# burchim/AVEC

Measured on AMD Instinct MI355X. Metric: AV utterances/sec fwd+bwd (audio T=400, video 100x88x88), higher is better.
Workload: dtype bf16

## Files before the change

### avec_amd/csrc/attention.h

```cpp
#pragma once
#include "common.h"
#include "avec_hip.h"

struct AttnArgs {
  const void *q, *k, *v; long long ld;
  const void* e; long long lde;
  const long long* lens; int len_div;
  int q_full;
  const float* mask; long long mask_bstride;
  void* o; long long ldo;
  float* lse;
  const void* dout;
  void *dq, *dk, *dv; long long lddq, ldd;
  float* de; long long ldde;
  void *pbuf, *dsbuf; long long ldt;
  void* dsrel; long long ldr;
  int B, H, T, d; float scale;
  int Tk;
};

template <typename T>
__device__ __forceinline__ bool key_keep(const AttnArgs& a, int b, int i, int j) {
  if (a.mask) return a.mask[(long long)b * a.mask_bstride + (long long)i * a.Tk + j] != 0.f;
  if (i >= a.q_full) return false;
  if (a.lens) return j < (int)(a.lens[b] / a.len_div);
  return true;
}


int attn_mfma_fwd(const AttnArgs& a, hipStream_t st);
int attn_mfma_bwd_rows(const AttnArgs& a, hipStream_t st);
```

### avec_amd/csrc/attention.hip

```cpp
#include "attention.h"
#include <stdio.h>

static constexpr int TQ = 32;
static constexpr int RPW = TQ / 4;
static constexpr int TK = 64;
static constexpr int QC = 32;
static constexpr int NCS = 3;

template <typename T, int VW>
__device__ __forceinline__ void load_vec(const T* p, float* v) {
  constexpr int NB = VW * (int)sizeof(T);
  if constexpr (NB < 4) { v[0] = ldf(p); }
  else {
    uint32_t w[NB / 4];
    if constexpr (NB == 16) { const chunk16 c = ldg16(p); w[0] = c.w[0]; w[1] = c.w[1]; w[2] = c.w[2]; w[3] = c.w[3]; }
    else {
#pragma unroll
      for (int k = 0; k < NB / 4; ++k) w[k] = ((const uint32_t*)p)[k];
    }
    if constexpr (sizeof(T) == 4) {
#pragma unroll
      for (int k = 0; k < NB / 4; ++k) v[k] = __uint_as_float(w[k]);
    } else {
#pragma unroll
// ... 94 lines not shown
        float p = (iv && jv) ? __expf(s - Li[rr]) * Il[rr] : 0.f;
        pval = p * (dp - dl[rr]) * a.scale;
        if (iv && jv) {
          const long long o = ((long long)bh * Tn + i) * a.ldt + j; stf((T*)a.pbuf + o, p); stf((T*)a.dsbuf + o, pval);
          if (a.dsrel) stf((T*)a.dsrel + ((long long)h * a.B * Tn + (long long)b * Tn + i) * a.ldr + (j + Tn - 1 - i), pval);
        }
      }
      Ps[w * 64 + lane] = pval;
      __syncthreads();
      if (!BWD) {
        for (int jj = 0; jj < TK; ++jj) {
          const float pj = Ps[w * 64 + jj];
#pragma unroll
          for (int u = 0; u < NCS; ++u) if (lane + 64 * u < d) acc[rr][u] += pj * Vs[jj * DP + lane + 64 * u];
        }
      } else {
        const float* ebase = Es + (TQ - 1 - ri) * DP;
        for (int jj = 0; jj < TK; ++jj) {
          const float dsj = Ps[w * 64 + jj];
#pragma unroll
          for (int u = 0; u < NCS; ++u) if (lane + 64 * u < d) acc[rr][u] += dsj * (Ks[jj * DP + lane + 64 * u] + ebase[jj * DP + lane + 64 * u]);
        }
      }
      __syncthreads();
    }
  }
#pragma unroll
  for (int rr = 0; rr < RPW; ++rr) {
    const int i = i0 + w * RPW + rr;
    if (i >= Tn) continue;
    if (!BWD) {
      const float inv = 1.f / l_run[rr];
      T* op = (T*)a.o + ((long long)b * Tn + i) * a.ldo + h * d;
#pragma unroll
      for (int u = 0; u < NCS; ++u) if (lane + 64 * u < d) stf(op + lane + 64 * u, acc[rr][u] * inv);
      if (lane == 0) { a.lse[((long long)bh * Tn + i) * 2] = m_run[rr]; a.lse[((long long)bh * Tn + i) * 2 + 1] = l_run[rr]; }
    } else {
      T* op = (T*)a.dq + ((long long)b * Tn + i) * a.lddq + h * d;
#pragma unroll
      for (int u = 0; u < NCS; ++u) if (lane + 64 * u < d) stf(op + lane + 64 * u, acc[rr][u]);
    }
  }
}

template <typename T, int DPAD>
__global__ __launch_bounds__(256) void attn_bwd_cols_kernel(AttnArgs a, int ktiles) {
  extern __shared__ __attribute__((aligned(16))) float sm[];
  const int d = a.d, DP = d | 1, Tn = a.T;
  float* Qs = sm; float* Gs = Qs + QC * DP; float* R0 = Gs + QC * DP; float* R1 = R0 + 64 * DP;
  const int lane = threadIdx.x & 63, w = threadIdx.x >> 6;
  const int bh = blockIdx.y, b = bh / a.H, h = bh % a.H;
  const bool rel = (int)blockIdx.x >= ktiles;
  const int c0 = (rel ? (int)blockIdx.x - ktiles : (int)blockIdx.x) * 64;
  const int col = c0 + lane;
  const T* qp = (const T*)a.q + (long long)b * Tn * a.ld + h * d;
  const T* gp = (const T*)a.dout + (long long)b * Tn * a.ldo + h * d;
  const T* P = (const T*)a.pbuf + (long long)bh * Tn * a.ldt; const T* S = (const T*)a.dsbuf + (long long)bh * Tn * a.ldt;
  float acc0[DPAD], acc1[DPAD];
#pragma unroll
  for (int c = 0; c < DPAD; ++c) { acc0[c] = 0.f; acc1[c] = 0.f; }
  for (int ic = 0; ic < Tn; ic += QC) {
    __syncthreads();
    load_rows<T>(Qs, DP, qp, a.ld, ic, QC, Tn, d);
    if (!rel) load_rows<T>(Gs, DP, gp, a.ldo, ic, QC, Tn, d);
    __syncthreads();
    for (int qi = w; qi < QC; qi += 4) {
      const int i = ic + qi;
      if (i >= Tn) break;
      const float* qrow = Qs + qi * DP;
      if (!rel) {
        float ds = 0.f, p = 0.f;
        if (col < Tn) { ds = ldf(S + (long long)i * a.ldt + col); p = ldf(P + (long long)i * a.ldt + col); }
        const float* grow = Gs + qi * DP;
#pragma unroll
        for (int c = 0; c < DPAD; ++c) if (c < d) { acc0[c] += ds * qrow[c]; acc1[c] += p * grow[c]; }
      } else {
        const int j = i - (Tn - 1) + col;
        const float ds = (col < 2 * Tn - 1 && j >= 0 && j < Tn) ? ldf(S + (long long)i * a.ldt + j) : 0.f;
#pragma unroll
        for (int c = 0; c < DPAD; ++c) if (c < d) acc0[c] += ds * qrow[c];
      }
    }
  }
  __syncthreads();
  for (int ww = 0; ww < 4; ++ww) {
    if (w == ww) {
#pragma unroll
      for (int c = 0; c < DPAD; ++c) if (c < d) {
        if (ww == 0) { R0[lane * DP + c] = acc0[c]; R1[lane * DP + c] = acc1[c]; }
        else { R0[lane * DP + c] += acc0[c]; R1[lane * DP + c] += acc1[c]; }
      }
    }
    __syncthreads();
  }
  for (int idx = threadIdx.x; idx < 64 * d; idx += 256) {
    const int r = idx / d, c = idx - r * d; const int cc = c0 + r;
    if (!rel) {
      if (cc < Tn) { stf((T*)a.dk + ((long long)b * Tn + cc) * a.ldd + h * d + c, R0[r * DP + c]); stf((T*)a.dv + ((long long)b * Tn + cc) * a.ldd + h * d + c, R1[r * DP + c]); }
    } else if (cc < 2 * Tn - 1) {
      atomicAdd(a.de + (long long)cc * a.ldde + h * d + c, R0[r * DP + c]);
    }
  }
}

static int fill_args(AttnArgs& a, const avec_attn_t* p) {
  a.q = p->q; a.k = p->k; a.v = p->v; a.ld = p->ld; a.e = p->e; a.lde = p->lde; a.lens = p->lens; a.len_div = p->len_div > 0 ? p->len_div : 1; a.q_full = p->q_full > 0 ? p->q_full : p->T;
  a.mask = p->mask; a.mask_bstride = p->mask_bstride; a.o = p->o; a.ldo = p->ldo; a.lse = p->lse; a.dout = p->dout;
  a.dq = p->dq; a.dk = p->dk; a.dv = p->dv; a.lddq = p->lddq; a.ldd = p->ldd; a.de = p->de; a.ldde = p->ldde; a.pbuf = p->pbuf; a.dsbuf = p->dsbuf; a.ldt = p->ldt; a.dsrel = p->dsrel; a.ldr = p->ldr;
  a.B = p->B; a.H = p->H; a.T = p->T; a.d = p->d; a.scale = p->scale; a.Tk = p->Tk > 0 ? p->Tk : p->T;
  AVEC_CHECK_ARG(a.q && a.k && a.v && a.e && a.o && a.lse, "attention: null pointer");
  AVEC_CHECK_ARG(a.B > 0 && a.H > 0 && a.T > 0 && a.d > 0 && a.d <= 64 * NCS && a.Tk >= a.T, "attention: bad dims B=%d H=%d T=%d Tk=%d d=%d (d <= %d, Tk >= T)", a.B, a.H, a.T, a.Tk, a.d, 64 * NCS);
  return 0;
}

extern "C" int avec_relpos_attention_fwd(int dtype, const avec_attn_t* p, hipStream_t st) {
  AttnArgs a; AVEC_CHECK_ARG(p, "attention_fwd: null args"); if (int r = fill_args(a, p)) return r;
  if (dtype == AVEC_BF16) { const int r = attn_mfma_fwd(a, st); if (r != 1) return r; }
  const int DP = a.d | 1; size_t lds = (size_t)(2 * TK + (TQ + TK - 1) + TQ) * DP * 4 + 4 * 64 * 4;
  dim3 grid((a.T + TQ - 1) / TQ, a.B * a.H);
  avec_note_kernel("attn_rows<%s,fwd>", dtype == AVEC_BF16 ? "bf16" : "f32");
  if (dtype == AVEC_BF16) { if (int r = avec_lds_optin(attn_rows_kernel<bf16, false>, lds)) return r; hipLaunchKernelGGL((attn_rows_kernel<bf16, false>), grid, dim3(256), lds, st, a); }
  else { if (int r = avec_lds_optin(attn_rows_kernel<float, false>, lds)) return r; hipLaunchKernelGGL((attn_rows_kernel<float, false>), grid, dim3(256), lds, st, a); }
  AVEC_LAUNCH_CHECK(); return 0;
}

template <typename T> static int launch_bwd(AttnArgs& a, hipStream_t st) {
  const int DP = a.d | 1;
  size_t lds1 = (size_t)(2 * TK + (TQ + TK - 1) + 2 * TQ) * DP * 4 + 4 * 64 * 4;
  dim3 grid1((a.T + TQ - 1) / TQ, a.B * a.H);
  bool rows_done = false;
  const bool cols = !(a.dsrel || a.Tk != a.T);
  AVEC_CHECK_ARG(!cols || a.d <= 96, "attention_bwd: the register-accumulating column pass serves d <= 96 (d=%d): pass dsrel and use avec_gemm_tn_batched", a.d);
  if (sizeof(T) == 2) { const int r = attn_mfma_bwd_rows(a, st); if (r == 0) rows_done = true; else if (r != 1) return r; }
  if (!rows_done) {
    if (int r = avec_lds_optin(attn_rows_kernel<T, true>, lds1)) return r;
    avec_note_kernel("attn_rows<%s,bwd>", sizeof(T) == 2 ? "bf16" : "f32");
    hipLaunchKernelGGL((attn_rows_kernel<T, true>), grid1, dim3(256), lds1, st, a);
  }
  if (!cols) return 0;
  size_t lds2 = (size_t)(2 * QC + 2 * 64) * DP * 4;
  const int ktiles = (a.T + 63) / 64, rtiles = (2 * a.T - 1 + 63) / 64;
  dim3 grid2(ktiles + rtiles, a.B * a.H);
#define LB(DPAD) do { char rows_[96]; snprintf(rows_, sizeof(rows_), "%s", avec_last_kernel()); avec_note_kernel("%s+cols<%d>", rows_, DPAD); \
    if (int r = avec_lds_optin(attn_bwd_cols_kernel<T, DPAD>, lds2)) return r; hipLaunchKernelGGL((attn_bwd_cols_kernel<T, DPAD>), grid2, dim3(256), lds2, st, a, ktiles); } while (0)
  if (a.d <= 48) LB(48); else if (a.d <= 64) LB(64); else LB(96);
#undef LB
  return 0;
}

extern "C" int avec_relpos_attention_bwd(int dtype, const avec_attn_t* p, hipStream_t st) {
  AttnArgs a; AVEC_CHECK_ARG(p, "attention_bwd: null args"); if (int r = fill_args(a, p)) return r;
  AVEC_CHECK_ARG(a.dout && a.dq && a.pbuf && a.dsbuf && a.ldt >= a.Tk && (a.dsrel ? a.ldr >= a.Tk + a.T - 1 : (a.Tk != a.T || (a.dk && a.dv && a.de))), "attention_bwd: null gradient / scratch pointer");
  int r = (dtype == AVEC_BF16) ? launch_bwd<bf16>(a, st) : launch_bwd<float>(a, st);
  if (r) return r;
  AVEC_LAUNCH_CHECK(); return 0;
}

struct AttnStream {
  const void *q, *k, *v; long long ld; const void* e; long long lde; void *kc, *vc;
  const long long* pos; const unsigned char* reset; const long long* clen; int div;
  void* o; long long ldo; int B, H, Tq, d, L; float scale;
};
template <typename T>
__global__ __launch_bounds__(256) void attn_stream_kernel(AttnStream a) {
  extern __shared__ __attribute__((aligned(16))) float sm[];
  const int d = a.d, DP = d | 1, Tq = a.Tq, L = a.L, cap = L + Tq;
  float* Ks = sm; float* Vs = Ks + TK * DP; float* Es = Vs + TK * DP; float* Qs = Es + (TQ + TK - 1) * DP; float* Ps = Qs + TQ * DP;
  const int lane = threadIdx.x & 63, w = threadIdx.x >> 6;
  const int bh = blockIdx.y, b = bh / a.H, h = bh % a.H;
  const int i0 = blockIdx.x * TQ;
  long long p0 = (a.reset && a.reset[b]) ? 0 : a.pos[b] / a.div; if (p0 < 0) p0 = 0;
  int n = Tq;
  if (a.clen) { const long long c = (a.clen[b] + a.div - 1) / a.div; n = c < 0 ? 0 : (c > Tq ? Tq : (int)c); }
  const long long ldc = (long long)a.H * d;
  const T* qp = (const T*)a.q + (long long)b * Tq * a.ld + h * d;
  const T* kp = (const T*)a.k + (long long)b * Tq * a.ld + h * d;
  const T* vp = (const T*)a.v + (long long)b * Tq * a.ld + h * d;
  T* kcb = (T*)a.kc + (long long)b * cap * ldc + h * d;
  T* vcb = (T*)a.vc + (long long)b * cap * ldc + h * d;
  const T* ep = (const T*)a.e + h * d;
  for (int r = w; r < TQ; r += 4) {
    const int i = i0 + r; const bool ok = i < Tq;
    for (int c = lane; c < d; c += 64) Qs[r * DP + c] = ok ? ldf(qp + (long long)i * a.ld + c) : 0.f;
    if (ok && i < n) {
      const long long crow = (p0 + i) % cap;
      for (int c = lane; c < d; c += 64) { kcb[crow * ldc + c] = kp[(long long)i * a.ld + c]; vcb[crow * ldc + c] = vp[(long long)i * a.ld + c]; }
    }
  }
  float m_run[RPW], l_run[RPW], acc[RPW][NCS];
#pragma unroll
  for (int rr = 0; rr < RPW; ++rr) { m_run[rr] = -INFINITY; l_run[rr] = 0.f; for (int u = 0; u < NCS; ++u) acc[rr][u] = 0.f; }
  const int i_last = min(i0 + TQ, Tq) - 1;
  const bool wave_live = i0 + w * RPW < Tq;
  for (int c0 = i0; c0 <= i_last + L; c0 += TK) {
    __syncthreads();
    for (int r = w; r < TK; r += 4) {
      const int c = c0 + r; bool ok = c <= i_last + L; const T *kr = kp, *vr = vp;
      if (c < L) { const long long p = p0 - L + c; ok = ok && p >= 0; const long long row = ok ? p % cap : 0; kr = kcb + row * ldc; vr = vcb + row * ldc; }
      else { const int ci = c - L; ok = ok && ci < Tq; const long long row = ok ? ci : 0; kr = kp + row * a.ld; vr = vp + row * a.ld; }
      for (int ch = lane; ch < d; ch += 64) { Ks[r * DP + ch] = ok ? ldf(kr + ch) : 0.f; Vs[r * DP + ch] = ok ? ldf(vr + ch) : 0.f; }
    }
    const int dmin = i0 + L - c0 - (TK - 1);
    for (int r = w; r < TQ + TK - 1; r += 4) {
      const int dl = dmin + r; const bool ok = dl >= 0 && dl <= L; const T* er = ep + (long long)(ok ? dl : 0) * a.lde;
      for (int ch = lane; ch < d; ch += 64) Es[r * DP + ch] = ok ? ldf(er + ch) : 0.f;
    }
    __syncthreads();
    if (wave_live) {
      const int c = c0 + lane;
#pragma unroll
      for (int rr = 0; rr < RPW; ++rr) {
        const int ri = w * RPW + rr, i = i0 + ri; const int dl = i + L - c;
        const bool keep = i < Tq && dl >= 0 && dl <= L && (c >= L || p0 - L + c >= 0);
        const float* qrow = Qs + ri * DP; const float* krow = Ks + lane * DP; const float* erow = Es + (ri + TK - 1 - lane) * DP;
        float s = 0.f;
        for (int ch = 0; ch < d; ++ch) s += qrow[ch] * (krow[ch] + erow[ch]);
        s *= a.scale;
        const float tmax = wave_max(keep ? s : -INFINITY);
        const float m_new = fmaxf(m_run[rr], tmax);
        float pval = 0.f;
        if (m_new != -INFINITY) {
          const float alpha = (m_run[rr] == -INFINITY) ? 0.f : __expf(m_run[rr] - m_new);
          pval = keep ? __expf(s - m_new) : 0.f;
          l_run[rr] = l_run[rr] * alpha + wave_sum(pval);
          for (int u = 0; u < NCS; ++u) acc[rr][u] *= alpha;
          m_run[rr] = m_new;
        }
        Ps[ri * 64 + lane] = pval;
      }
    }
    __syncthreads();
    if (wave_live) {
#pragma unroll
      for (int rr = 0; rr < RPW; ++rr) {
        const float* prow = Ps + (w * RPW + rr) * 64;
        for (int jj = 0; jj < TK; ++jj) {
          const float pj = prow[jj];
#pragma unroll
          for (int u = 0; u < NCS; ++u) if (lane + 64 * u < d) acc[rr][u] += pj * Vs[jj * DP + lane + 64 * u];
        }
      }
    }
  }
#pragma unroll
  for (int rr = 0; rr < RPW; ++rr) {
    const int i = i0 + w * RPW + rr;
    if (i >= Tq) continue;
    const float inv = 1.f / l_run[rr];
    T* op = (T*)a.o + ((long long)b * Tq + i) * a.ldo + h * d;
#pragma unroll
    for (int u = 0; u < NCS; ++u) if (lane + 64 * u < d) stf(op + lane + 64 * u, acc[rr][u] * inv);
  }
}

extern "C" long long avec_relpos_attention_stream_state_bytes(int dtype, int B, int H, int d, int L, int Tq) {
  if (B <= 0 || H <= 0 || d <= 0 || L < 0 || Tq <= 0) return 0;
  return (long long)B * (L + Tq) * H * d * (dtype == AVEC_BF16 ? 2 : 4);
}
extern "C" int avec_relpos_attention_stream(int dtype, const void* q, const void* k, const void* v, long long ld, const void* e, long long lde, void* kcache, void* vcache,
                                            long long cache_bytes, const long long* pos, const unsigned char* reset, const long long* chunk_len, int div, void* o, long long ldo,
                                            int B, int H, int Tq, int d, int L, float scale, hipStream_t st) {
  AVEC_CHECK_ARG(q && k && v && e && kcache && vcache && pos && o, "relpos_attention_stream: null pointer (q, k, v, e, kcache, vcache, pos and o are required)");
  AVEC_CHECK_ARG(B > 0 && H > 0 && Tq > 0 && L >= 0 && div > 0 && d > 0 && d <= 64 * NCS, "relpos_attention_stream: bad dims B=%d H=%d Tq=%d d=%d L=%d div=%d (d <= %d)", B, H, Tq, d, L, div, 64 * NCS);
  AVEC_CHECK_ARG(ld >= (long long)H * d && ldo >= (long long)H * d && lde >= (long long)H * d, "relpos_attention_stream: row strides ld=%lld ldo=%lld lde=%lld below H * d = %d", ld, ldo, lde, H * d);
  const long long need = avec_relpos_attention_stream_state_bytes(dtype, B, H, d, L, Tq);
  AVEC_CHECK_ARG(cache_bytes >= need, "relpos_attention_stream: key / value rings of %lld bytes each, %lld needed (avec_relpos_attention_stream_state_bytes)", cache_bytes, need);
  const uintptr_t em = dtype == AVEC_BF16 ? 1 : 3;
  AVEC_CHECK_ARG(!(((uintptr_t)q | (uintptr_t)k | (uintptr_t)v | (uintptr_t)e | (uintptr_t)kcache | (uintptr_t)vcache | (uintptr_t)o) & em) && !(((uintptr_t)pos | (uintptr_t)chunk_len) & 7),
                 "relpos_attention_stream: misaligned pointer (tensors: element size, pos / chunk_len: 8 bytes)");
  AVEC_CHECK_ARG(kcache != vcache, "relpos_attention_stream: kcache and vcache must be two buffers");
  AttnStream a{q, k, v, ld, e, lde, kcache, vcache, pos, reset, chunk_len, div, o, ldo, B, H, Tq, d, L, scale};
  const int DP = d | 1; const size_t lds = (size_t)(2 * TK + (TQ + TK - 1) + TQ) * DP * 4 + (size_t)TQ * 64 * 4;
  dim3 grid((Tq + TQ - 1) / TQ, B * H);
  avec_note_kernel("attn_stream<%s>", dtype == AVEC_BF16 ? "bf16" : "f32");
  if (dtype == AVEC_BF16) { if (int r = avec_lds_optin(attn_stream_kernel<bf16>, lds)) return r; hipLaunchKernelGGL((attn_stream_kernel<bf16>), grid, dim3(256), lds, st, a); }
  else { if (int r = avec_lds_optin(attn_stream_kernel<float>, lds)) return r; hipLaunchKernelGGL((attn_stream_kernel<float>), grid, dim3(256), lds, st, a); }
  AVEC_LAUNCH_CHECK(); return 0;
}
```

### avec_amd/csrc/attention_mfma.hip

```cpp
#include "attention.h"
#ifndef AVEC_ATTN_ABL
#define AVEC_ATTN_ABL 0
#endif

typedef __attribute__((ext_vector_type(8))) __bf16 bf16x8_t;
typedef __attribute__((ext_vector_type(16))) float f32x16;
typedef short v4s_t __attribute__((ext_vector_type(4)));

static constexpr int NTMAX = 12;
static constexpr int CTMAX = 3;

template <int PITCH> __device__ __forceinline__ int aswz(int row) {
  return PITCH == 128 ? ((((row >> 1) & 1) << 2) | ((row >> 2) & 3)) : (((row & 3) << 2) | ((row >> 2) & 3));
}
__device__ __forceinline__ f32x16 mma(const chunk16& a, const chunk16& b, f32x16 c) {
  return __builtin_amdgcn_mfma_f32_32x32x16_bf16(__builtin_bit_cast(bf16x8_t, a), __builtin_bit_cast(bf16x8_t, b), c, 0, 0, 0);
}
__device__ __forceinline__ chunk16 tr8(const char* p0, const char* p1) {
  typedef __attribute__((address_space(3))) v4s_t* lp_t;
  const v4s_t a = __builtin_amdgcn_ds_read_tr16_b64_v4i16((lp_t)p0), b = __builtin_amdgcn_ds_read_tr16_b64_v4i16((lp_t)p1);
  const uint2 ua = __builtin_bit_cast(uint2, a), ub = __builtin_bit_cast(uint2, b);
  chunk16 f; f.w[0] = ua.x; f.w[1] = ua.y; f.w[2] = ub.x; f.w[3] = ub.y; return f;
}
__device__ __forceinline__ uint32_t pack2(float lo, float hi) { return f32x2_to_bf16x2(lo, hi); }

template <int PITCH, int NTHR>
__device__ __forceinline__ void stage_rows(char* dst, const bf16* src, long long ld, int row0, int nrows, int limit, int d, int dpad) {
  const int CH = dpad >> 3;
  for (int idx = threadIdx.x; idx < nrows * CH; idx += NTHR) {
    const int r = idx / CH, c = idx - r * CH; const int gr = row0 + r;
    chunk16 v; v.w[0] = v.w[1] = v.w[2] = v.w[3] = 0u;
    if (gr >= 0 && gr < limit) {
      const bf16* p = src + (long long)gr * ld + c * 8;
      if (c * 8 + 8 <= d) v = ldg16(p);
      else {
        uint32_t h[8];
#pragma unroll
        for (int e = 0; e < 8; ++e) h[e] = (c * 8 + e < d) ? (uint32_t)p[e].v : 0u;
#pragma unroll
        for (int e = 0; e < 4; ++e) v.w[e] = h[2 * e] | (h[2 * e + 1] << 16);
      }
    }
    *(chunk16*)(dst + r * PITCH + ((c ^ aswz<PITCH>(r)) << 4)) = v;
  }
}

__device__ __forceinline__ void attn_glds16(const void* gsrc, unsigned lds_dst_uniform) {
  unsigned keep;
  asm volatile("s_mov_b32 %0, m0\n\ts_mov_b32 m0, %2\n\ts_nop 0\n\tglobal_load_lds_dwordx4 %1, off\n\ts_mov_b32 m0, %0" : "=&s"(keep) : "v"(gsrc), "s"(lds_dst_uniform) : "memory");
}
__device__ __attribute__((aligned(64))) unsigned char attn_zero16[64];

template <int PITCH, int NW>
__device__ __forceinline__ void stage_rows_dma(unsigned lds_img, char* img, const bf16* src, long long ld, int row0, int nrows, int limit, int d, int dpad,
                                               long long last_row, int rowbytes, int wave, int lane) {
  constexpr int SLOTS = PITCH / 16, RPI = 64 / SLOTS;
  constexpr int NV = PITCH == 128 ? 2 : 4;
  const int CH = dpad >> 3;
  const int rg = lane / SLOTS, pos = lane % SLOTS;
  const int ninstr = nrows / RPI;
  const unsigned ldb = (unsigned)ld * 2u;
  const bool can_past = dpad * 2 > rowbytes && last_row <= (long long)limit - 1;
  const int lastr = can_past ? (int)last_row : -1;
  unsigned short pe[8]; int pk = -1, pn = 0; unsigned pc = 0;
  if (can_past) {
    const int rt = lastr - row0;
    if (rt >= 0 && rt < nrows && (rt / RPI) % NW == wave && rt % RPI == rg) {
      int c = pos ^ aswz<PITCH>(rt);
      if (c < CH && c * 16 + 16 > rowbytes) {
        pk = rt / RPI; pc = (unsigned)c * 16u; pn = (rowbytes - c * 16) >> 1; pn = pn < 0 ? 0 : pn;
        const unsigned short* q = (const unsigned short*)((const char*)src + ((unsigned)lastr * ldb + pc));
#pragma unroll
        for (int e = 0; e < 8; ++e) pe[e] = e < pn ? q[e] : (unsigned short)0;
      }
    }
  }
  unsigned coff[NV]; bool cpast[NV];
#pragma unroll
  for (int v = 0; v < NV; ++v) {
    int c = pos ^ aswz<PITCH>(RPI * (wave + v * NW) + rg); c = c < CH ? c : 0;
    coff[v] = (unsigned)c * 16u; cpast[v] = c * 16 + 16 > rowbytes;
  }
  for (int k0 = wave; k0 < ninstr; k0 += NW * NV) {
#pragma unroll
    for (int v = 0; v < NV; ++v) {
      const int k = k0 + v * NW;
      if (k < ninstr) {
        int gr = row0 + k * RPI + rg; gr = gr < 0 ? 0 : (gr >= limit ? limit - 1 : gr);
        const char* p = (const char*)src + ((unsigned)gr * ldb + coff[v]);
        const bool past = gr == lastr && cpast[v];
        attn_glds16(past ? (const void*)attn_zero16 : (const void*)p, (unsigned)__builtin_amdgcn_readfirstlane((int)(lds_img + k * 1024)));
      }
    }
  }
  if (can_past && __builtin_amdgcn_readfirstlane(__any(pk >= 0) ? 1 : 0)) {
    asm volatile("s_waitcnt vmcnt(0)" ::: "memory");
    if (pk >= 0) {
      unsigned short* dst = (unsigned short*)(img + pk * 1024 + lane * 16);
#pragma unroll
      for (int e = 0; e < 8; ++e) if (e < pn) dst[e] = pe[e];
    }
  }
}
template <int PITCH, int NW>
__device__ __forceinline__ void zero_pad_channels(char* img, int nrows, int d, int dpad, int wave, int lane) {
  if (d == dpad) return;
  constexpr int SLOTS = PITCH / 16, RPI = 64 / SLOTS;
  const int rg = lane / SLOTS, pos = lane % SLOTS;
  const int ninstr = nrows / RPI;
  for (int k = wave; k < ninstr; k += NW) {
    const int r = k * RPI + rg;
    const int c = pos ^ aswz<PITCH>(r);
    unsigned short* dst = (unsigned short*)(img + k * 1024 + lane * 16);
#pragma unroll
    for (int e = 0; e < 8; ++e) if (c * 8 + e >= d && c * 8 + e < dpad) dst[e] = 0;
  }
}

struct MfmaGeom { int Tp, NT, NE, dpad, DKS, CT, alias; size_t offK, offV, offE, offQ, offS, total; };
static MfmaGeom mfma_geom(int T, int d, int pitch, bool bwd) {
  MfmaGeom g; g.Tp = (T + 31) / 32 * 32; g.NT = g.Tp / 32; g.NE = g.Tp + 64; g.dpad = (d + 15) / 16 * 16; g.DKS = g.dpad / 16; g.CT = (d + 31) / 32;
  for (g.alias = 0; g.alias < 2; ++g.alias) {
    g.offK = 0; g.offV = g.alias ? g.offK : g.offK + (size_t)g.Tp * pitch; g.offE = g.offV + (size_t)g.Tp * pitch; g.offQ = g.offE + (size_t)g.NE * pitch;
    g.offS = g.offQ + (size_t)64 * pitch * (bwd ? 2 : 1);
    g.total = g.offS + (size_t)2 * 8192;
    if (g.total <= 160 * 1024) break;
  }
  if (g.alias > 1) g.alias = 1;
  return g;
}

template <int PITCH, int NTM, int DKS>
__device__ __forceinline__ float scores(f32x16 (&S)[NTM], const char* Ks, const char* Es, const char* qrow, float* ring, const MfmaGeom& G, float scale,
                                        int w, int il, int hf, int Tn, int klen, bool row_masked) {
  const int dks = DKS ? DKS : G.DKS;
  const int swr = aswz<PITCH>(il);
#pragma unroll
  for (int jt = 0; jt < NTM; ++jt)
#pragma unroll
    for (int r = 0; r < 16; ++r) S[jt][r] = 0.f;
  auto rel_tile = [&](int et) {
    f32x16 R;
#pragma unroll
    for (int r = 0; r < 16; ++r) R[r] = 0.f;
    const char* erow = Es + (32 * et + 32 * (1 - w) + il) * PITCH;
#pragma unroll
    for (int kk = 0; kk < dks; ++kk) {
      const chunk16 fa = *(const chunk16*)(erow + (((2 * kk + hf) ^ swr) << 4));
      const chunk16 fb = *(const chunk16*)(qrow + (((2 * kk + hf) ^ swr) << 4));
      R = mma(fa, fb, R);
    }
    float* slot = ring + (et & 1) * 1024;
#pragma unroll
    for (int r = 0; r < 16; ++r) slot[((r & 3) + 8 * (r >> 2) + 4 * hf) * 32 + il] = R[r];
  };
  rel_tile(0);
#pragma unroll
  for (int jt = 0; jt < NTM; ++jt) {
    if (jt < G.NT) {
      const char* krow = Ks + (32 * jt + il) * PITCH;
#pragma unroll
      for (int kk = 0; kk < dks; ++kk) {
        const chunk16 fa = *(const chunk16*)(krow + (((2 * kk + hf) ^ swr) << 4));
        const chunk16 fb = *(const chunk16*)(qrow + (((2 * kk + hf) ^ swr) << 4));
        S[jt] = mma(fa, fb, S[jt]);
      }
      rel_tile(jt + 1);
      asm volatile("s_waitcnt lgkmcnt(0)" ::: "memory");
#pragma unroll
      for (int r = 0; r < 16; ++r) {
        const int jl = (r & 3) + 8 * (r >> 2) + 4 * hf;
        const int el = 32 * jt + jl + 31 - il;
        S[jt][r] += ring[(el & 63) * 32 + il];
      }
      asm volatile("" ::: "memory");
    }
  }
  float mx = -INFINITY;
#pragma unroll
  for (int jt = 0; jt < NTM; ++jt) {
    if (jt < G.NT) {
#pragma unroll
      for (int r = 0; r < 16; ++r) {
        const int j = 32 * jt + (r & 3) + 8 * (r >> 2) + 4 * hf;
        float v = S[jt][r] * scale;
        if (row_masked || j >= klen) v += -1e9f;
        v = j < Tn ? v : -INFINITY;
        S[jt][r] = v; mx = fmaxf(mx, v);
      }
    }
  }
  return mx;
}

template <int PITCH>
__device__ __forceinline__ void tr_offsets(int (&off)[CTMAX][2], int lane) {
  const int g4 = lane >> 4, t = lane & 15;
#pragma unroll
  for (int hh = 0; hh < 2; ++hh) {
    const int key = 8 * hh + 4 * (g4 >> 1) + (t >> 2);
#pragma unroll
    for (int ct = 0; ct < CTMAX; ++ct) {
      const int cb = 32 * ct + 16 * (g4 & 1);
      off[ct][hh] = key * PITCH + ((((cb >> 3) + ((t & 3) >> 1)) ^ aswz<PITCH>(key)) << 4) + (t & 1) * 8;
    }
  }
}

__device__ __forceinline__ void store_rows_T(const f32x16 (&O)[CTMAX], float mul, float* ring, const MfmaGeom& G, bf16* op, long long ldo, int nrow, int d, int lane) {
  const int hf = lane >> 5, il = lane & 31;
  bf16* ost = (bf16*)ring; const int OP = G.dpad + 4;
  asm volatile("s_waitcnt lgkmcnt(0)" ::: "memory");
#pragma unroll
  for (int ct = 0; ct < CTMAX; ++ct) {
    if (ct < G.CT) {
#pragma unroll
      for (int q = 0; q < 4; ++q) {
        const int c0 = 32 * ct + 8 * q + 4 * hf;
        uint2 u; u.x = pack2(O[ct][4 * q] * mul, O[ct][4 * q + 1] * mul); u.y = pack2(O[ct][4 * q + 2] * mul, O[ct][4 * q + 3] * mul);
        if (c0 < G.dpad) *(uint2*)(ost + il * OP + c0) = u;
      }
    }
  }
  asm volatile("s_waitcnt lgkmcnt(0)" ::: "memory");
  typedef uint32_t __attribute__((aligned(2))) u32_u;
  const int dh = d >> 1;
  for (int idx = lane; idx < nrow * dh; idx += 64) { const int r = idx / dh, c = (idx - r * dh) * 2; *(u32_u*)(op + (long long)r * ldo + c) = *(const uint32_t*)(ost + r * OP + c); }
  if (d & 1) for (int r = lane; r < nrow; r += 64) op[(long long)r * ldo + d - 1] = ost[r * OP + d - 1];
}

template <int PITCH, int NTM, bool ALIAS, int DKS>
__global__ __launch_bounds__(ALIAS ? 128 : 256) void attn_mfma_fwd_kernel(AttnArgs a, MfmaGeom G) {
  constexpr int NWS = ALIAS ? 2 : 4;
  extern __shared__ __attribute__((aligned(16))) char sm[];
  char* Ks = sm + G.offK; char* Vs = sm + G.offV; char* Es = sm + G.offE; char* Qs = sm + G.offQ;
  const int tid = threadIdx.x, lane = tid & 63, w = tid >> 6, hf = lane >> 5, il = lane & 31;
  float* ring = (float*)(sm + G.offS + w * 8192);
  const int bh = blockIdx.y, b = bh / a.H, h = bh - b * a.H;
  const int Tn = a.T, d = a.d, i0 = blockIdx.x * 64;
  const bf16* qp = (const bf16*)a.q + (long long)b * Tn * a.ld + h * d;
  const bf16* kp = (const bf16*)a.k + (long long)b * Tn * a.ld + h * d;
  const bf16* vp = (const bf16*)a.v + (long long)b * Tn * a.ld + h * d;
  const bf16* ep = (const bf16*)a.e + h * d;
  {
    typedef __attribute__((address_space(3))) void* lptr_t;
    const unsigned lds0 = (unsigned)(uintptr_t)(lptr_t)sm;
    const int wv = __builtin_amdgcn_readfirstlane(w);
    const long long lastq = (long long)(a.B - 1 - b) * Tn + Tn - 1;
    const int rb = (a.H - h) * d * 2;
    stage_rows_dma<PITCH, NWS>(lds0 + (unsigned)G.offK, Ks, kp, a.ld, 0, G.Tp, Tn, d, G.dpad, lastq, rb, wv, lane);
    if (!ALIAS) stage_rows_dma<PITCH, NWS>(lds0 + (unsigned)G.offV, Vs, vp, a.ld, 0, G.Tp, Tn, d, G.dpad, lastq, rb, wv, lane);
    stage_rows_dma<PITCH, NWS>(lds0 + (unsigned)G.offQ, Qs, qp, a.ld, i0, 64, Tn, d, G.dpad, lastq, rb, wv, lane);
    stage_rows_dma<PITCH, NWS>(lds0 + (unsigned)G.offE, Es, ep, a.lde, (Tn - 1) - (i0 + 63), G.NE, 2 * Tn - 1, d, G.dpad, 2 * Tn - 2, rb, wv, lane);
    asm volatile("s_waitcnt vmcnt(0)" ::: "memory");
    zero_pad_channels<PITCH, NWS>(Qs, 64, d, G.dpad, wv, lane);
  }
  __syncthreads();
  if (NWS > 2 && w >= 2) return;
#if AVEC_ATTN_ABL == 1
  if (sm[tid * 16] == 123) a.lse[0] = 1.f;
  return;
#endif

  const int i = i0 + 32 * w + il;
  const char* qrow = Qs + (32 * w + il) * PITCH;
  const int klen = a.lens ? (int)(a.lens[b] / a.len_div) : Tn;
  const bool row_masked = i >= a.q_full;

  f32x16 S[NTM];
  float mx = scores<PITCH, NTM, DKS>(S, Ks, Es, qrow, ring, G, a.scale, w, il, hf, Tn, klen, row_masked);
  mx = fmaxf(mx, __shfl_xor(mx, 32, 64));
  float lsum = 0.f;
#pragma unroll
  for (int jt = 0; jt < NTM; ++jt) {
    if (jt < G.NT) {
#pragma unroll
      for (int r = 0; r < 16; ++r) { const float p = __expf(S[jt][r] - mx); S[jt][r] = p; lsum += p; }
    }
  }
  lsum += __shfl_xor(lsum, 32, 64);
  if (hf == 0 && i < Tn) { a.lse[((long long)bh * Tn + i) * 2] = mx; a.lse[((long long)bh * Tn + i) * 2 + 1] = lsum; }
#if AVEC_ATTN_ABL == 2
  return;
#endif

  if (ALIAS) { __syncthreads(); stage_rows<PITCH, 128>(Vs, vp, a.ld, 0, G.Tp, Tn, d, G.dpad); __syncthreads(); }
  f32x16 O[CTMAX];
#pragma unroll
  for (int ct = 0; ct < CTMAX; ++ct)
#pragma unroll
    for (int r = 0; r < 16; ++r) O[ct][r] = 0.f;
  int offv[CTMAX][2]; tr_offsets<PITCH>(offv, lane);
#pragma unroll
  for (int jt = 0; jt < NTM; ++jt) {
    if (jt < G.NT) {
#pragma unroll
      for (int s = 0; s < 2; ++s) {
        chunk16 pb;
#pragma unroll
        for (int e = 0; e < 4; ++e) pb.w[e] = pack2(S[jt][8 * s + 2 * e], S[jt][8 * s + 2 * e + 1]);
        const char* vb = Vs + (32 * jt + 16 * s) * PITCH;
#pragma unroll
        for (int ct = 0; ct < CTMAX; ++ct) if (ct < G.CT) O[ct] = mma(tr8(vb + offv[ct][0], vb + offv[ct][1]), pb, O[ct]);
      }
    }
  }
  bf16* op = (bf16*)a.o + ((long long)b * Tn + i0 + 32 * w) * a.ldo + h * d;
  store_rows_T(O, 1.f / lsum, ring, G, op, a.ldo, min(32, Tn - (i0 + 32 * w)), d, lane);
}

template <int PITCH, int NTM, bool ALIAS, int DKS>
__global__ __launch_bounds__(ALIAS ? 128 : 256) void attn_mfma_bwd_kernel(AttnArgs a, MfmaGeom G) {
  constexpr int NWS = ALIAS ? 2 : 4;
  extern __shared__ __attribute__((aligned(16))) char sm[];
  char* Ks = sm + G.offK; char* Vs = sm + G.offV; char* Es = sm + G.offE; char* Qs = sm + G.offQ; char* Gs = Qs + 64 * PITCH;
  const int tid = threadIdx.x, lane = tid & 63, w = tid >> 6, hf = lane >> 5, il = lane & 31;
  float* ring = (float*)(sm + G.offS + w * 8192);
  const int bh = blockIdx.y, b = bh / a.H, h = bh - b * a.H;
  const int Tn = a.T, d = a.d, i0 = blockIdx.x * 64;
  const bf16* qp = (const bf16*)a.q + (long long)b * Tn * a.ld + h * d;
  const bf16* kp = (const bf16*)a.k + (long long)b * Tn * a.ld + h * d;
  const bf16* vp = (const bf16*)a.v + (long long)b * Tn * a.ld + h * d;
  const bf16* ep = (const bf16*)a.e + h * d;
  const bf16* gp = (const bf16*)a.dout + (long long)b * Tn * a.ldo + h * d;
  {
    typedef __attribute__((address_space(3))) void* lptr_t;
    const unsigned lds0 = (unsigned)(uintptr_t)(lptr_t)sm;
    const int wv = __builtin_amdgcn_readfirstlane(w);
    const long long lastq = (long long)(a.B - 1 - b) * Tn + Tn - 1;
    const int rb = (a.H - h) * d * 2;
    stage_rows_dma<PITCH, NWS>(lds0 + (unsigned)G.offK, Ks, kp, a.ld, 0, G.Tp, Tn, d, G.dpad, lastq, rb, wv, lane);
    if (!ALIAS) stage_rows_dma<PITCH, NWS>(lds0 + (unsigned)G.offV, Vs, vp, a.ld, 0, G.Tp, Tn, d, G.dpad, lastq, rb, wv, lane);
    stage_rows_dma<PITCH, NWS>(lds0 + (unsigned)G.offQ, Qs, qp, a.ld, i0, 64, Tn, d, G.dpad, lastq, rb, wv, lane);
    stage_rows_dma<PITCH, NWS>(lds0 + (unsigned)G.offQ + 64 * PITCH, Gs, gp, a.ldo, i0, 64, Tn, d, G.dpad, lastq, rb, wv, lane);
    stage_rows_dma<PITCH, NWS>(lds0 + (unsigned)G.offE, Es, ep, a.lde, (Tn - 1) - (i0 + 63), G.NE, 2 * Tn - 1, d, G.dpad, 2 * Tn - 2, rb, wv, lane);
    asm volatile("s_waitcnt vmcnt(0)" ::: "memory");
    zero_pad_channels<PITCH, NWS>(Qs, 64, d, G.dpad, wv, lane);
    zero_pad_channels<PITCH, NWS>(Gs, 64, d, G.dpad, wv, lane);
  }
  __syncthreads();
  if (NWS > 2 && w >= 2) return;
#if AVEC_ATTN_ABL == 1
  if (sm[tid * 16] == 123) a.lse[0] = 1.f;
  return;
#endif

  const int i = i0 + 32 * w + il;
  const int swr = aswz<PITCH>(il);
  const char* qrow = Qs + (32 * w + il) * PITCH; const char* grow = Gs + (32 * w + il) * PITCH;
  const int klen = a.lens ? (int)(a.lens[b] / a.len_div) : Tn;
  const bool row_masked = i >= a.q_full, iv = i < Tn;
  float delta = 0.f, m_i = 0.f, il_i = 0.f;
  if (iv) {
    const bf16* orow = (const bf16*)a.o + ((long long)b * Tn + i) * a.ldo + h * d;
    const int c0 = hf * ((d + 1) >> 1), c1 = hf ? d : ((d + 1) >> 1);
    for (int c = c0; c < c1; ++c) {
      const int ch = c >> 3; const bf16* gq = (const bf16*)(grow + ((ch ^ swr) << 4)) + (c & 7);
      delta += bf16_to_f32(gq->v) * bf16_to_f32(orow[c].v);
    }
    m_i = a.lse[((long long)bh * Tn + i) * 2]; il_i = 1.f / a.lse[((long long)bh * Tn + i) * 2 + 1];
  }
  delta += __shfl_xor(delta, 32, 64);

  f32x16 S[NTM];
  scores<PITCH, NTM, DKS>(S, Ks, Es, qrow, ring, G, a.scale, w, il, hf, Tn, klen, row_masked);
#if AVEC_ATTN_ABL == 2
  if (S[0][0] + S[1][3] + delta == 1234.5f) a.lse[0] = 1.f;
  return;
#endif
  if (ALIAS) { __syncthreads(); stage_rows<PITCH, 128>(Vs, vp, a.ld, 0, G.Tp, Tn, d, G.dpad); __syncthreads(); }
  bf16* prow = (bf16*)a.pbuf + ((long long)bh * Tn + i) * a.ldt;
  bf16* srow = (bf16*)a.dsbuf + ((long long)bh * Tn + i) * a.ldt;
  bf16* rrow = a.dsrel ? (bf16*)a.dsrel + ((long long)h * a.B * Tn + (long long)b * Tn + i) * a.ldr + (Tn - 1 - i) : nullptr;
  const bool st8 = (a.ldt & 3) == 0 && ((((size_t)a.pbuf) | ((size_t)a.dsbuf)) & 7) == 0;
#pragma unroll
  for (int jt = 0; jt < NTM; ++jt) {
    if (jt < G.NT) {
      f32x16 dP;
#pragma unroll
      for (int r = 0; r < 16; ++r) dP[r] = 0.f;
      const char* vrow = Vs + (32 * jt + il) * PITCH;
#pragma unroll
      for (int kk = 0; kk < (DKS ? DKS : G.DKS); ++kk) {
        const chunk16 fa = *(const chunk16*)(vrow + (((2 * kk + hf) ^ swr) << 4));
        const chunk16 fb = *(const chunk16*)(grow + (((2 * kk + hf) ^ swr) << 4));
        dP = mma(fa, fb, dP);
      }
#pragma unroll
      for (int q = 0; q < 4; ++q) {
        const int j0 = 32 * jt + 8 * q + 4 * hf;
        float pv[4], dv[4];
#pragma unroll
        for (int e = 0; e < 4; ++e) {
          const int r = 4 * q + e; const bool ok = iv && (j0 + e) < Tn;
          const float p = ok ? __expf(S[jt][r] - m_i) * il_i : 0.f;
          pv[e] = p; dv[e] = p * (dP[r] - delta) * a.scale; S[jt][r] = dv[e];
        }
        if (iv && j0 < Tn) {
          if (st8 && j0 + 3 < Tn) {
            uint2 up, ud; up.x = pack2(pv[0], pv[1]); up.y = pack2(pv[2], pv[3]); ud.x = pack2(dv[0], dv[1]); ud.y = pack2(dv[2], dv[3]);
            *(uint2*)(prow + j0) = up; *(uint2*)(srow + j0) = ud;
          } else {
#pragma unroll
            for (int e = 0; e < 4; ++e) if (j0 + e < Tn) { prow[j0 + e].v = f32_to_bf16(pv[e]); srow[j0 + e].v = f32_to_bf16(dv[e]); }
          }
          if (rrow) {
            typedef uint2 __attribute__((aligned(2))) u64_u;
            if (j0 + 3 < Tn) { uint2 ud; ud.x = pack2(dv[0], dv[1]); ud.y = pack2(dv[2], dv[3]); *(u64_u*)(rrow + j0) = ud; }
            else {
#pragma unroll
              for (int e = 0; e < 4; ++e) if (j0 + e < Tn) rrow[j0 + e].v = f32_to_bf16(dv[e]);
            }
          }
        }
      }
    }
  }
#if AVEC_ATTN_ABL == 3
  return;
#endif
  if (ALIAS) { __syncthreads(); stage_rows<PITCH, 128>(Ks, kp, a.ld, 0, G.Tp, Tn, d, G.dpad); __syncthreads(); }
  f32x16 DQ[CTMAX];
#pragma unroll
  for (int ct = 0; ct < CTMAX; ++ct)
#pragma unroll
    for (int r = 0; r < 16; ++r) DQ[ct][r] = 0.f;
  int offt[CTMAX][2]; tr_offsets<PITCH>(offt, lane);
#pragma unroll
  for (int jt = 0; jt < NTM; ++jt) {
    if (jt < G.NT) {
#pragma unroll
      for (int s = 0; s < 2; ++s) {
        chunk16 pb;
#pragma unroll
        for (int e = 0; e < 4; ++e) pb.w[e] = pack2(S[jt][8 * s + 2 * e], S[jt][8 * s + 2 * e + 1]);
        const char* kb = Ks + (32 * jt + 16 * s) * PITCH;
#pragma unroll
        for (int ct = 0; ct < CTMAX; ++ct) if (ct < G.CT) DQ[ct] = mma(tr8(kb + offt[ct][0], kb + offt[ct][1]), pb, DQ[ct]);
      }
    }
  }
  asm volatile("s_waitcnt lgkmcnt(0)" ::: "memory");
#pragma unroll
  for (int r = 0; r < 16; ++r) ring[1024 + ((r & 3) + 8 * (r >> 2) + 4 * hf) * 32 + il] = 0.f;
#pragma unroll
  for (int et = 0; et <= NTM; ++et) {
    if (et <= G.NT) {
      float* slot = ring + (et & 1) * 1024;
#pragma unroll
      for (int r = 0; r < 16; ++r) {
        float v = 0.f;
        if (et < NTM) v = (et < G.NT) ? S[et < NTM ? et : 0][r] : 0.f;
        slot[((r & 3) + 8 * (r >> 2) + 4 * hf) * 32 + il] = v;
      }
      asm volatile("s_waitcnt lgkmcnt(0)" ::: "memory");
      float rs[16];
#pragma unroll
      for (int r = 0; r < 16; ++r) {
        const int j = 32 * et + (r & 3) + 8 * (r >> 2) + 4 * hf - 31 + il;
        rs[r] = ring[(j & 63) * 32 + il];
      }
      asm volatile("" ::: "memory");
#pragma unroll
      for (int s = 0; s < 2; ++s) {
        chunk16 pb;
#pragma unroll
        for (int e = 0; e < 4; ++e) pb.w[e] = pack2(rs[8 * s + 2 * e], rs[8 * s + 2 * e + 1]);
        const char* eb = Es + (32 * et + 32 * (1 - w) + 16 * s) * PITCH;
#pragma unroll
        for (int ct = 0; ct < CTMAX; ++ct) if (ct < G.CT) DQ[ct] = mma(tr8(eb + offt[ct][0], eb + offt[ct][1]), pb, DQ[ct]);
      }
    }
  }
  bf16* dqp = (bf16*)a.dq + ((long long)b * Tn + i0 + 32 * w) * a.lddq + h * d;
  store_rows_T(DQ, 1.f, ring, G, dqp, a.lddq, min(32, Tn - (i0 + 32 * w)), d, lane);
}

static const bool g_mfma_off = getenv("AVEC_NO_MFMA_ATTN") != nullptr;
static bool rows_too_short(long long ld, int d) { return ld + d < (d + 15) / 16 * 16; }

int attn_mfma_fwd(const AttnArgs& a, hipStream_t st) {
  if (g_mfma_off || a.mask || a.d > 96 || a.T > 32 * NTMAX || a.Tk != a.T || rows_too_short(a.ld, a.d) || rows_too_short(a.lde, a.d)) return 1;
  const int pitch = a.d <= 64 ? 128 : 256;
  const MfmaGeom G = mfma_geom(a.T, a.d, pitch, false);
  if (G.total > 160 * 1024) return 1;
  dim3 grid((a.T + 63) / 64, a.B * a.H);
#define AVEC_LAUNCH_ATTN(TAG, NAME, P, N, A, K) do { avec_note_kernel(TAG "<%d,%d,%d,%d>", P, N, (int)A, K); if (int r = avec_lds_optin(NAME<P, N, A, K>, G.total)) return r; \
    hipLaunchKernelGGL((NAME<P, N, A, K>), grid, dim3(G.alias ? 128 : 256), G.total, st, a, G); } while (0)
#define AVEC_PICK_DKS(TAG, NAME, N, A) do { \
    if (pitch == 128) { if (G.DKS == 4) AVEC_LAUNCH_ATTN(TAG, NAME, 128, N, A, 4); else if (G.DKS == 3) AVEC_LAUNCH_ATTN(TAG, NAME, 128, N, A, 3); else AVEC_LAUNCH_ATTN(TAG, NAME, 128, N, A, 0); } \
    else { if (G.DKS == 6) AVEC_LAUNCH_ATTN(TAG, NAME, 256, N, A, 6); else AVEC_LAUNCH_ATTN(TAG, NAME, 256, N, A, 0); } } while (0)
#define AVEC_PICK_ATTN(TAG, NAME) do { \
    if (a.T <= 224 && !G.alias) AVEC_PICK_DKS(TAG, NAME, 7, false); \
    else if (!G.alias) AVEC_PICK_DKS(TAG, NAME, 12, false); \
    else AVEC_PICK_DKS(TAG, NAME, 12, true); } while (0)
  AVEC_PICK_ATTN("attn_mfma_fwd", attn_mfma_fwd_kernel);
  AVEC_LAUNCH_CHECK(); return 0;
}

int attn_mfma_bwd_rows(const AttnArgs& a, hipStream_t st) {
  if (g_mfma_off || a.mask || a.d > 96 || a.T > 32 * NTMAX || a.Tk != a.T || !a.pbuf || !a.dsbuf || !a.dq || !a.dout || rows_too_short(a.ld, a.d) || rows_too_short(a.lde, a.d) ||
      rows_too_short(a.ldo, a.d)) return 1;
  const int pitch = a.d <= 64 ? 128 : 256;
  const MfmaGeom G = mfma_geom(a.T, a.d, pitch, true);
  if (G.total > 160 * 1024) return 1;
  dim3 grid((a.T + 63) / 64, a.B * a.H);
  AVEC_PICK_ATTN("attn_mfma_bwd", attn_mfma_bwd_kernel);
#undef AVEC_PICK_ATTN
#undef AVEC_PICK_DKS
#undef AVEC_LAUNCH_ATTN
  AVEC_LAUNCH_CHECK(); return 0;
}
```

### avec_amd/csrc/gemm.hip

```cpp
#include "gemm_dev.h"

template <typename T, int BM, int BN, int MODE, bool SRC_F32, bool A16>
__global__ __launch_bounds__(256, 2) void gemm_nt_kernel(GemmArgs g) {
  constexpr int VEC = Elt<T>::VEC;
  constexpr int KE = BKB / (int)sizeof(T);
  constexpr int NCA = BM * 8 / 256, NCB = BN * 8 / 256;
  constexpr int MT = BM / 64, NT = BN / 64;
  constexpr int TILE = (BM + BN) * LDS_ROW;
  extern __shared__ __attribute__((aligned(16))) char smem[];
  const int tid = threadIdx.x, lane = tid & 63, wave = tid >> 6;
  const int wm = wave >> 1, wn = wave & 1;
  const long long m0 = (long long)blockIdx.x * BM; const int n0 = blockIdx.y * BN;
  const int kc = (tid & 7) * VEC;
  const int r0 = tid >> 3;

  RowInfo ra[NCA]; RowInfo rb[NCB];
  RowSrc ws; ws.ptr = g.W; ws.ld = g.ldw; ws.step = 0; ws.rows_out = ws.rows_in = 1;
#pragma unroll
  for (int i = 0; i < NCA; ++i) ra[i] = row_info<MODE>(g.a, m0 + r0 + i * 32, g.M);
#pragma unroll
  for (int i = 0; i < NCB; ++i) rb[i] = row_info<MODE_PLAIN>(ws, n0 + r0 + i * 32, g.N);

  f32x16 acc[MT][NT];
#pragma unroll
// ... 678 lines not shown
    long long row[MT], rrow[MT]; bool valid[MT];
    const long long Mc = perm ? pMc : g.M;
    const bool use_res = g.e.res != nullptr && (!g.e.res_cls0 || cls == 0);
#pragma unroll
    for (int i = 0; i < MT; ++i) {
      long long mc = m0 + wm * (BM / 2) + i * 32 + (lane & 31);
      valid[i] = mc < Mc; if (!valid[i]) mc = Mc - 1;
      row[i] = mc;
      if (perm) { long long img; int ih, iw; perm2_pixel(g.a, cls, mc, img, ih, iw); row[i] = (img * g.a.H + ih) * (long long)g.a.W + iw; }
      rrow[i] = g.e.res_cls0 ? mc : row[i];
    }
    conv_epilogue_tr<BM, BN, MT, NT>(g, acc, smem, row, valid, use_res ? (const bf16*)g.e.res : nullptr, rrow, m0 + BM <= Mc, n0, tid, lane, wm, wn);
  } else nt_epilogue<T, BM, BN, MT, NT>(g, acc, smem, m0, n0, tid, lane, wm, wn, cls);
}

typedef __attribute__((ext_vector_type(8))) int i32x8;

template <int BM, int BN, int STAGES>
__global__ __launch_bounds__(256, 2) void gemm_nt_fp8_kernel(GemmArgs g, const float* __restrict__ amax_a, const float* __restrict__ amax_w) {
  typedef bf16 T;
  constexpr int RB = 128, KE = 128;
  constexpr int NCA = BM * 8 / 256, NCB = BN * 8 / 256;
  constexpr int MT = BM / 64, NT = BN / 64;
  constexpr int TILE = (BM + BN) * RB;
  extern __shared__ __attribute__((aligned(16))) char smem[];
  const int tid = threadIdx.x, lane = tid & 63, wave = tid >> 6;
  const int wm = wave >> 1, wn = wave & 1;
  const long long m0 = (long long)blockIdx.x * BM; const int n0 = blockIdx.y * BN;
  typedef __attribute__((address_space(1))) const void* gptr_t;
  typedef __attribute__((address_space(3))) void* lptr_t;
  long long aoff[NCA], boff[NCB]; int ka[NCA], kb[NCB];
#pragma unroll
  for (int i = 0; i < NCA; ++i) { const int row = (tid >> 3) + i * 32; aoff[i] = (m0 + row < g.M) ? (m0 + row) * g.a.ld : -1; ka[i] = ((tid & 7) ^ glds_swz<RB>(row)) * 16; }
#pragma unroll
  for (int i = 0; i < NCB; ++i) { const int row = (tid >> 3) + i * 32; boff[i] = (n0 + row < g.N) ? (long long)(n0 + row) * g.ldw : -1; kb[i] = ((tid & 7) ^ glds_swz<RB>(row)) * 16; }
  auto issue = [&](int kt, int buf) {
    char* As = smem + buf * TILE; char* Bs = As + BM * RB;
#pragma unroll
    for (int i = 0; i < NCA; ++i) {
      const int k = kt * KE + ka[i];
      const void* src = (aoff[i] >= 0 && k < g.K) ? (const void*)((const char*)g.a.ptr + aoff[i] + k) : (const void*)avec_zero16;
      __builtin_amdgcn_global_load_lds((gptr_t)src, (lptr_t)(As + (i * 256 + wave * 64) * 16), 16, 0, 0);
    }
#pragma unroll
    for (int i = 0; i < NCB; ++i) {
      const int k = kt * KE + kb[i];
      const void* src = (boff[i] >= 0 && k < g.K) ? (const void*)((const char*)g.W + boff[i] + k) : (const void*)avec_zero16;
      __builtin_amdgcn_global_load_lds((gptr_t)src, (lptr_t)(Bs + (i * 256 + wave * 64) * 16), 16, 0, 0);
    }
  };
  int offa[MT], swa[MT], offb[NT], swb[NT];
#pragma unroll
  for (int i = 0; i < MT; ++i) { const int row = wm * (BM / 2) + i * 32 + (lane & 31); offa[i] = row * RB; swa[i] = glds_swz<RB>(row); }
#pragma unroll
  for (int j = 0; j < NT; ++j) { const int row = wn * (BN / 2) + j * 32 + (lane & 31); offb[j] = row * RB; swb[j] = glds_swz<RB>(row); }
  const int gsel = lane >> 5;
  f32x16 acc[MT][NT];
#pragma unroll
  for (int i = 0; i < MT; ++i)
#pragma unroll
    for (int j = 0; j < NT; ++j)
#pragma unroll
      for (int r = 0; r < 16; ++r) acc[i][j][r] = 0.f;
  const int KT = (g.K + KE - 1) / KE;
  constexpr int LPT = NCA + NCB;
#define AVEC_WAIT_VM(n) asm volatile("s_waitcnt vmcnt(%0)" ::"n"(n) : "memory")
#pragma unroll
  for (int st = 0; st < STAGES - 1; ++st) if (st < KT) issue(st, st);
  for (int kt = 0; kt < KT; ++kt) {
    const int newer = min(STAGES - 2, KT - 1 - kt);
    if (STAGES <= 2 || newer <= 0) AVEC_WAIT_VM(0);
    else if (newer == 1) AVEC_WAIT_VM(LPT);
    else AVEC_WAIT_VM(2 * LPT);
    __builtin_amdgcn_s_barrier();
    asm volatile("" ::: "memory");
    if (kt + STAGES - 1 < KT) issue(kt + STAGES - 1, (kt + STAGES - 1) % STAGES);
    const char* As = smem + (kt % STAGES) * TILE; const char* Bs = As + BM * RB;
#pragma unroll
    for (int s2 = 0; s2 < 2; ++s2) {
      chunk16 fa[MT][2], fb[NT][2];
#pragma unroll
      for (int i = 0; i < MT; ++i)
#pragma unroll
        for (int h = 0; h < 2; ++h) fa[i][h] = *(const chunk16*)(As + offa[i] + (((4 * s2 + 2 * gsel + h) ^ swa[i]) << 4));
#pragma unroll
      for (int j = 0; j < NT; ++j)
#pragma unroll
        for (int h = 0; h < 2; ++h) fb[j][h] = *(const chunk16*)(Bs + offb[j] + (((4 * s2 + 2 * gsel + h) ^ swb[j]) << 4));
      asm volatile("" ::: "memory");
#pragma unroll
      for (int i = 0; i < MT; ++i) {
        const i32x8 a = {(int)fa[i][0].w[0], (int)fa[i][0].w[1], (int)fa[i][0].w[2], (int)fa[i][0].w[3], (int)fa[i][1].w[0], (int)fa[i][1].w[1], (int)fa[i][1].w[2], (int)fa[i][1].w[3]};
#pragma unroll
        for (int j = 0; j < NT; ++j) {
          const i32x8 b = {(int)fb[j][0].w[0], (int)fb[j][0].w[1], (int)fb[j][0].w[2], (int)fb[j][0].w[3], (int)fb[j][1].w[0], (int)fb[j][1].w[1], (int)fb[j][1].w[2], (int)fb[j][1].w[3]};
          acc[i][j] = __builtin_amdgcn_mfma_scale_f32_32x32x64_f8f6f4(a, b, acc[i][j], 0, 0, 0, 127, 0, 127);
        }
      }
    }
  }
#undef AVEC_WAIT_VM
  const float sc = (fmaxf(*amax_a, 1e-20f) * (1.0f / 448.0f)) * (fmaxf(*amax_w, 1e-20f) * (1.0f / 448.0f));
#pragma unroll
  for (int i = 0; i < MT; ++i)
#pragma unroll
    for (int j = 0; j < NT; ++j)
#pragma unroll
      for (int r = 0; r < 16; ++r) acc[i][j][r] *= sc;
  __syncthreads();
  nt_epilogue<T, BM, BN, MT, NT>(g, acc, smem, m0, n0, tid, lane, wm, wn);
}

struct TnArgs { const void* P; long long ldp; RowSrc q; float* O; void* Oact; long long ldo; long long M; int I, J, Iq, Jq; int m_per_block; float* pcs;
                int split, nb_inner, xcd_map, q_ohw, q_mg, q_nwrap; long long sPo, sPi, sQo, sQi, sOo, sOi; };

__device__ __forceinline__ int tn_swz(int col) { return (((col >> 2) ^ (col >> 3) ^ (col >> 4)) & 1) << 4; }

template <typename T>
__device__ __forceinline__ void store_transposed(char* S, int col0, int p, const chunk16& c0, const chunk16& c1) {
  constexpr int VEC = Elt<T>::VEC;
  if (sizeof(T) == 4) {
#pragma unroll
    for (int e = 0; e < VEC; ++e) *(uint32_t*)(S + (col0 + e) * LDS_ROW + ((p ^ tn_swz(col0 + e)) << 2)) = c0.w[e];
  } else {
#pragma unroll
    for (int e = 0; e < VEC; ++e) {
      const uint32_t w = (e & 1) ? __builtin_amdgcn_perm(c1.w[e >> 1], c0.w[e >> 1], 0x07060302u) : __builtin_amdgcn_perm(c1.w[e >> 1], c0.w[e >> 1], 0x05040100u);
      *(uint32_t*)(S + (col0 + e) * LDS_ROW + ((p ^ tn_swz(col0 + e)) << 2)) = w;
    }
  }
}

template <typename T, int BM, int BN, int MT, int NT>
__device__ __forceinline__ void mma_tile_swz(const char* As, const char* Bs, int wm, int wn, int lane, f32x16 (&acc)[MT][NT]) {
  int offa[MT], offb[NT], lowa[MT], lowb[NT];
#pragma unroll
  for (int i = 0; i < MT; ++i) { const int row = wm * (BM / 2) + i * 32 + (lane & 31); offa[i] = row * LDS_ROW; lowa[i] = ((lane >> 5) * 16) ^ (tn_swz(row) << 2); }
#pragma unroll
  for (int j = 0; j < NT; ++j) { const int row = wn * (BN / 2) + j * 32 + (lane & 31); offb[j] = row * LDS_ROW; lowb[j] = ((lane >> 5) * 16) ^ (tn_swz(row) << 2); }
#pragma unroll
  for (int kk = 0; kk < 4; ++kk) {
    chunk16 fa[MT], fb[NT];
#pragma unroll
    for (int i = 0; i < MT; ++i) fa[i] = *(const chunk16*)(As + offa[i] + (lowa[i] ^ (kk * 32)));
#pragma unroll
    for (int j = 0; j < NT; ++j) fb[j] = *(const chunk16*)(Bs + offb[j] + (lowb[j] ^ (kk * 32)));
#pragma unroll
    for (int i = 0; i < MT; ++i)
#pragma unroll
      for (int j = 0; j < NT; ++j) Mma<T>::run(fa[i], fb[j], acc[i][j]);
  }
}

template <typename T, int BI, int BJ, int MODE, bool Q_F32, bool A16>
__device__ __forceinline__ void gemm_tn_body(TnArgs g, const int bx, const int by, const int bz) {
  constexpr int VEC = Elt<T>::VEC;
  constexpr int RPT = sizeof(T) == 2 ? 2 : 1;
  constexpr int KE = 32 * RPT;
  constexpr int CPR_I = BI / VEC, CPR_J = BJ / VEC;
  constexpr int NTI = 32 * CPR_I / 256, NTJ = 32 * CPR_J / 256;
  constexpr int MT = BI / 64, NT = BJ / 64;
  constexpr int TILE = (BI + BJ) * LDS_ROW;
  constexpr bool Q_CONV = (MODE == MODE_CONV_FWD);
  extern __shared__ __attribute__((aligned(16))) char smem[];
  const int tid = threadIdx.x, lane = tid & 63, wave = tid >> 6;
  const int wm = wave >> 1, wn = wave & 1;
  const int i0 = bx * BI, j0 = by * BJ;
  const int zb = bz / g.split, zs = bz - zb * g.split;
  const long long bo = zb / g.nb_inner, bi = zb - bo * g.nb_inner;
  g.P = (const T*)g.P + bo * g.sPo + bi * g.sPi;
  g.q.ptr = (Q_F32 && sizeof(T) == 2) ? (const void*)((const float*)g.q.ptr + bo * g.sQo + bi * g.sQi) : (const void*)((const T*)g.q.ptr + bo * g.sQo + bi * g.sQi);
  g.O += bo * g.sOo + bi * g.sOi;
  T* Oact = g.Oact ? (T*)g.Oact + bo * g.sOo + bi * g.sOi : nullptr;
  const long long mb = (long long)zs * g.m_per_block;
  long long me = mb + g.m_per_block; if (me > g.M) me = g.M;

  f32x16 acc[MT][NT];
#pragma unroll
  for (int i = 0; i < MT; ++i)
#pragma unroll
    for (int j = 0; j < NT; ++j)
#pragma unroll
      for (int r = 0; r < 16; ++r) acc[i][j][r] = 0.f;

  auto task_p = [&](int u) { const int hi = (tid >> 6) + 4 * u; return (tid & 15) + 16 * (hi & 1); };
  auto task_c = [&](int u) { const int hi = (tid >> 6) + 4 * u; return ((tid >> 4) & 3) + 4 * (hi >> 1); };
  int qkh[NTJ], qkw[NTJ], qc[NTJ], qoh[NTJ][RPT], qow[NTJ][RPT]; long long qimg[NTJ][RPT];
  if (Q_CONV) {
#pragma unroll
    for (int u = 0; u < NTJ; ++u) {
      const int j = j0 + task_c(u) * VEC; const int tap = j / g.q.C; qc[u] = j - tap * g.q.C; qkh[u] = tap / g.q.KW; qkw[u] = tap - qkh[u] * g.q.KW;
#pragma unroll
      for (int r = 0; r < RPT; ++r) {
        const long long m = mb + task_p(u) * RPT + r; qow[u][r] = (int)(m % g.q.OW); const long long t = m / g.q.OW; qoh[u][r] = (int)(t % g.q.OH); qimg[u][r] = t / g.q.OH;
      }
    }
  }
  Pend pp[NTI][RPT], pq[NTJ][RPT];
  auto issue = [&](long long mt0) {
#pragma unroll
    for (int u = 0; u < NTI; ++u) {
      const int col = i0 + task_c(u) * VEC;
#pragma unroll
      for (int r = 0; r < RPT; ++r) { const long long m = mt0 + task_p(u) * RPT + r; pp[u][r] = issue_load<T, false, A16>(g.P, m < me ? m * g.ldp + col : -1, col, g.Iq); }
    }
#pragma unroll
    for (int u = 0; u < NTJ; ++u) {
      const int col = j0 + task_c(u) * VEC;
#pragma unroll
      for (int r = 0; r < RPT; ++r) {
        const long long m = mt0 + task_p(u) * RPT + r;
        if (Q_CONV) {
          RowInfo ri; ri.valid = m < me; ri.base = qimg[u][r] * (long long)g.q.H * g.q.W * g.q.C;
          ri.a = qoh[u][r] * g.q.stride - g.q.pad; ri.b = qow[u][r] * g.q.stride - g.q.pad;
          pq[u][r] = issue_load<T, false, A16>(g.q.ptr, conv_offset<MODE_CONV_FWD>(g.q, ri, qkh[u], qkw[u], qc[u]), col, g.J);
          qow[u][r] += KE;
          while (qow[u][r] >= g.q.OW) { qow[u][r] -= g.q.OW; if (++qoh[u][r] >= g.q.OH) { qoh[u][r] = 0; ++qimg[u][r]; } }
        } else {
          long long row = m;
          if (g.q.step > 1) row = (m / g.q.rows_out) * (long long)g.q.rows_in + (m % g.q.rows_out) * (long long)g.q.step;
          pq[u][r] = issue_load<T, Q_F32, A16>(g.q.ptr, m < me ? row * g.q.ld + col : -1, col, g.Jq);
        }
      }
    }
  };
  auto stage = [&](int buf) {
    char* Ps = smem + buf * TILE; char* Qs = Ps + BI * LDS_ROW;
#pragma unroll
    for (int u = 0; u < NTI; ++u) store_transposed<T>(Ps, task_c(u) * VEC, task_p(u), finish_load<T, false>(pp[u][0]), finish_load<T, false>(pp[u][RPT - 1]));
#pragma unroll
    for (int u = 0; u < NTJ; ++u) store_transposed<T>(Qs, task_c(u) * VEC, task_p(u), finish_load<T, Q_F32 && !Q_CONV>(pq[u][0]), finish_load<T, Q_F32 && !Q_CONV>(pq[u][RPT - 1]));
  };
  if (mb < me) {
    issue(mb);
    stage(0);
    __syncthreads();
    int cur = 0;
    for (long long mt0 = mb; mt0 < me; mt0 += KE, cur ^= 1) {
      const bool more = mt0 + KE < me;
      if (more) issue(mt0 + KE);
      mma_tile_swz<T, BI, BJ, MT, NT>(smem + cur * TILE, smem + cur * TILE + BI * LDS_ROW, wm, wn, lane, acc);
      if (more) stage(cur ^ 1);
      __syncthreads();
    }
  }
#pragma unroll
  for (int j = 0; j < NT; ++j) {
    const int col = j0 + wn * (BJ / 2) + j * 32 + (lane & 31);
    if (col >= g.J) continue;
#pragma unroll
    for (int i = 0; i < MT; ++i)
#pragma unroll
      for (int r = 0; r < 16; ++r) {
        const int row = i0 + wm * (BI / 2) + i * 32 + (r & 3) + 8 * (r >> 2) + 4 * (lane >> 5);
        if (row < g.I) { if (Oact) stf(Oact + (long long)row * g.ldo + col, acc[i][j][r]); else atomicAdd(g.O + (long long)row * g.ldo + col, acc[i][j][r]); }
      }
  }
}

template <typename T, int BI, int BJ, int MODE, bool Q_F32, bool A16>
__global__ __launch_bounds__(256, 2) void gemm_tn_kernel(TnArgs g) { gemm_tn_body<T, BI, BJ, MODE, Q_F32, A16>(g, blockIdx.x, blockIdx.y, blockIdx.z); }

#define AVEC_TN_MULTI_MAX 3
struct TnMulti { TnArgs g[AVEC_TN_MULTI_MAX]; int first[AVEC_TN_MULTI_MAX + 1], gx[AVEC_TN_MULTI_MAX], gy[AVEC_TN_MULTI_MAX], n; };
__global__ __launch_bounds__(256, 2) void gemm_tn_multi_kernel(TnMulti m) {
  const int w = blockIdx.x;
  int p = 0; if (m.n > 1 && w >= m.first[1]) p = 1; if (m.n > 2 && w >= m.first[2]) p = 2;
  int l = w - m.first[p]; const int bx = l % m.gx[p]; l /= m.gx[p];
  gemm_tn_body<bf16, 64, 64, MODE_PLAIN, false, false>(m.g[p], bx, l % m.gy[p], l / m.gy[p]);
}

typedef short v4s_t __attribute__((ext_vector_type(4)));
__device__ __forceinline__ chunk16 tr_read8(const char* p0, const char* p1) {
  typedef __attribute__((address_space(3))) v4s_t* lp_t;
  const v4s_t a = __builtin_amdgcn_ds_read_tr16_b64_v4i16((lp_t)p0), b = __builtin_amdgcn_ds_read_tr16_b64_v4i16((lp_t)p1);
  const uint2 ua = __builtin_bit_cast(uint2, a), ub = __builtin_bit_cast(uint2, b);
  chunk16 f; f.w[0] = ua.x; f.w[1] = ua.y; f.w[2] = ub.x; f.w[3] = ub.y; return f;
}
template <int BC> __device__ __forceinline__ int tr_swz(int row) { return BC == 128 ? 4 * (row & 3) : 4 * ((row >> 1) & 1); }

template <int BI, int BJ, int MODE, int STAGES, bool Q32 = false, int KT = 64>
__device__ __forceinline__ void tn_tr_body(const TnArgs& g, const int bx, const int by, const int bz) {
  typedef bf16 T;
  constexpr int CPI = BI / 8, CPJ = BJ / 8;
  constexpr int RI = 256 / CPI, RJ = 256 / CPJ;
  constexpr int NLI = KT / RI, NLJ = KT / RJ;
  constexpr int MTI = BI / 64, MTJ = BJ / 64;
  constexpr int PBYTES = KT * BI * 2, QBYTES = KT * BJ * 2, TILE = PBYTES + QBYTES;
  constexpr bool Q_CONV = (MODE == MODE_CONV_FWD);
  extern __shared__ __attribute__((aligned(16))) char smem[];
  const int tid = threadIdx.x, lane = tid & 63, wave = tid >> 6;
  const int wi = wave >> 1, wj = wave & 1;
  const int i0 = bx * BI, j0 = by * BJ;
  const int zb = bz / g.split, zs = bz - zb * g.split;
  const long long bo = zb / g.nb_inner, bi = zb - bo * g.nb_inner;
  const T* Pp = (const T*)g.P + bo * g.sPo + bi * g.sPi;
  const T* Qp = (const T*)g.q.ptr + bo * g.sQo + bi * g.sQi;
  float* Op = g.O + bo * g.sOo + bi * g.sOi;
  const long long mb = (long long)zs * g.m_per_block;
  long long me = mb + g.m_per_block; if (me > g.M) me = g.M;

  f32x16 acc[MTI][MTJ];
#pragma unroll
  for (int i = 0; i < MTI; ++i)
#pragma unroll
    for (int j = 0; j < MTJ; ++j)
#pragma unroll
      for (int r = 0; r < 16; ++r) acc[i][j][r] = 0.f;

  const int prow0 = tid / CPI, pcol = i0 + (((tid % CPI) ^ tr_swz<BI>(prow0)) << 3);
  const int qrow0 = tid / CPJ, qcol = j0 + (((tid % CPJ) ^ tr_swz<BJ>(qrow0)) << 3);
  const bool pok = pcol < g.Iq, qok = qcol < (Q_CONV ? g.J : g.Jq);
  int qkh = 0, qkw = 0, qc = 0, qpx[NLJ]; long long qimg[NLJ];
  const int q_hwc = Q_CONV ? g.q.H * g.q.W * g.q.C : 0;
  if (Q_CONV) {
    const int tap = qcol / g.q.C; qc = qcol - tap * g.q.C; qkh = tap / g.q.KW; qkw = tap - qkh * g.q.KW;
#pragma unroll
    for (int u = 0; u < NLJ; ++u) {
      const long long m = mb + qrow0 + u * RJ; const long long im = m / g.q_ohw; qpx[u] = (int)(m - im * g.q_ohw); qimg[u] = im * (long long)q_hwc;
    }
  }
  typedef __attribute__((address_space(1))) const void* gptr_t;
  typedef __attribute__((address_space(3))) void* lptr_t;
  const unsigned lds0 = (unsigned)(uintptr_t)(lptr_t)smem;
  auto tn_dma = [&](const void* src, unsigned off) {
    if ((!Q_CONV || AVEC_TN_CONV_ASM) && !(AVEC_TN_BUILTIN_DMA)) glds16_v64(src, (unsigned)__builtin_amdgcn_readfirstlane((int)(lds0 + off)));
    else __builtin_amdgcn_global_load_lds((gptr_t)src, (lptr_t)(smem + off), 16, 0, 0);
  };
  unsigned poff[NLI], qoff[NLJ];
  bool lean = false;
  if constexpr (!Q_CONV) {
    lean = g.q.step <= 1 && !(AVEC_TN_BUILTIN_DMA);
#pragma unroll
    for (int u = 0; u < NLI; ++u) poff[u] = (unsigned)(((long long)(prow0 + u * RI) * g.ldp + (pok ? pcol : i0)) * 2);
#pragma unroll
    for (int u = 0; u < NLJ; ++u) qoff[u] = (unsigned)(((long long)(qrow0 + u * RJ) * g.q.ld + (qok ? qcol : j0)) * 2);
  }
  const int wave_u = __builtin_amdgcn_readfirstlane(wave);
  auto issue = [&](long long mt0, int buf) {
    if constexpr (!Q_CONV) {
      if (lean && mt0 + KT <= me) {
        const unsigned l0 = lds0 + (unsigned)(buf * TILE) + (unsigned)wave_u * 1024u;
        glds16_group<NLI>(poff, (const char*)Pp + mt0 * g.ldp * 2, l0);
        glds16_group<NLJ>(qoff, (const char*)Qp + mt0 * g.q.ld * 2, l0 + PBYTES);
        return;
      }
    }
#pragma unroll
    for (int u = 0; u < NLI; ++u) {
      const long long m = mt0 + prow0 + u * RI;
      const void* src = (pok && m < me) ? (const void*)(Pp + m * g.ldp + pcol) : (const void*)avec_zero16;
      tn_dma(src, (unsigned)(buf * TILE + (u * 256 + wave * 64) * 16));
    }
#pragma unroll
    for (int u = 0; u < NLJ; ++u) {
      const long long m = mt0 + qrow0 + u * RJ;
      const void* src = (const void*)avec_zero16;
      if (Q_CONV) {
        const int oh = (int)(((unsigned)qpx[u] * (unsigned)g.q_mg) >> 20), ow = qpx[u] - oh * g.q.OW;
        const int ih = oh * g.q.stride - g.q.pad + qkh, iw = ow * g.q.stride - g.q.pad + qkw;
        const bool ok = qok && m < me && (unsigned)ih < (unsigned)g.q.H && (unsigned)iw < (unsigned)g.q.W;
        const T* sp = Q32 ? Qp + ((int)qimg[u] + (ih * g.q.W + iw) * g.q.C + qc) : Qp + qimg[u] + (ih * g.q.W + iw) * g.q.C + qc;
        src = ok ? (const void*)sp : src;
        qpx[u] += KT;
        for (int r = 0; r < g.q_nwrap; ++r) { const bool w = qpx[u] >= g.q_ohw; qpx[u] -= w ? g.q_ohw : 0; qimg[u] += w ? q_hwc : 0; }
      } else {
        long long row = m;
        if (g.q.step > 1) row = (m / g.q.rows_out) * (long long)g.q.rows_in + (m % g.q.rows_out) * (long long)g.q.step;
        src = (qok && m < me) ? (const void*)(Qp + row * g.q.ld + qcol) : src;
      }
      tn_dma(src, (unsigned)(buf * TILE + PBYTES + (u * 256 + wave * 64) * 16));
    }
  };
  const int g4 = lane >> 4, t = lane & 15;
  int offa[MTI][2], offb[MTJ][2];
#pragma unroll
  for (int h = 0; h < 2; ++h) {
    const int row = 8 * (g4 >> 1) + 4 * h + (t >> 2);
#pragma unroll
    for (int i = 0; i < MTI; ++i) { const int cb = wi * (BI / 2) + i * 32 + 16 * (g4 & 1); offa[i][h] = row * (BI * 2) + ((((cb >> 3) + ((t & 3) >> 1)) ^ tr_swz<BI>(row)) << 4) + (t & 1) * 8; }
#pragma unroll
    for (int j = 0; j < MTJ; ++j) { const int cb = wj * (BJ / 2) + j * 32 + 16 * (g4 & 1); offb[j][h] = PBYTES + row * (BJ * 2) + ((((cb >> 3) + ((t & 3) >> 1)) ^ tr_swz<BJ>(row)) << 4) + (t & 1) * 8; }
  }
  constexpr int CS_RF = 64 / (CPI * 4), CS_N = (KT / 4) / (4 * CS_RF);
  const bool do_cs = g.pcs != nullptr && by == 0;
  const int cs_pc = lane % CPI, cs_r4 = (lane / CPI) & 3, cs_rs = lane / (CPI * 4);
  float cs[8] = {0.f, 0.f, 0.f, 0.f, 0.f, 0.f, 0.f, 0.f};
  constexpr int LPT = NLI + NLJ;
#define AVEC_WAIT_VM(n) asm volatile("s_waitcnt vmcnt(%0)" ::"n"(n) : "memory")
  const int KTN = (int)((me - mb + KT - 1) / KT);
#pragma unroll
  for (int st = 0; st < STAGES - 1; ++st) if (st < KTN) issue(mb + (long long)st * KT, st);
  for (int kt = 0; kt < KTN; ++kt) {
    const int newer = min(STAGES - 2, KTN - 1 - kt);
    if (STAGES <= 2 || newer <= 0) AVEC_WAIT_VM(0);
    else if (newer == 1) AVEC_WAIT_VM(LPT);
    else AVEC_WAIT_VM(2 * LPT);
    __builtin_amdgcn_s_barrier();
    asm volatile("" ::: "memory");
    if (kt + STAGES - 1 < KTN) issue(mb + (long long)(kt + STAGES - 1) * KT, (kt + STAGES - 1) % STAGES);
    const char* S = smem + (kt % STAGES) * TILE;
    if (do_cs) {
#pragma unroll
      for (int n = 0; n < CS_N; ++n) {
        const int m = cs_r4 + 4 * (wave * CS_RF + cs_rs + 4 * CS_RF * n);
        const chunk16 c = *(const chunk16*)(S + m * (BI * 2) + (cs_pc << 4));
#pragma unroll
        for (int e = 0; e < 4; ++e) { cs[2 * e] += __uint_as_float(c.w[e] << 16); cs[2 * e + 1] += __uint_as_float(c.w[e] & 0xffff0000u); }
      }
    }
#pragma unroll
    for (int kk = 0; kk < KT / 16; ++kk) {
      chunk16 fa[MTI], fb[MTJ];
#pragma unroll
      for (int i = 0; i < MTI; ++i) fa[i] = tr_read8(S + offa[i][0] + kk * 16 * BI * 2, S + offa[i][1] + kk * 16 * BI * 2);
#pragma unroll
      for (int j = 0; j < MTJ; ++j) fb[j] = tr_read8(S + offb[j][0] + kk * 16 * BJ * 2, S + offb[j][1] + kk * 16 * BJ * 2);
#pragma unroll
      for (int i = 0; i < MTI; ++i)
#pragma unroll
        for (int j = 0; j < MTJ; ++j) Mma<T>::run(fa[i], fb[j], acc[i][j]);
    }
  }
#undef AVEC_WAIT_VM
// ... 130 lines not shown
  if constexpr (sizeof(T) == 2 && MODE != MODE_PLAIN) { if (a16) return launch_nt_generic<T, BM, BN, MODE, false, true>(g, grid, st); }
  return launch_nt_generic<T, BM, BN, MODE, false, false>(g, grid, st);
}

template <typename T, int BM, int BN>
static int launch_nt_mode(const GemmArgs& g_in, int mode, int src_f32, hipStream_t st) {
  GemmArgs g = g_in;
  dim3 grid((unsigned)((g.M + BM - 1) / BM), (unsigned)((g.N + BN - 1) / BN));
  constexpr int VEC = Elt<T>::VEC;
  const bool f32src = src_f32 && sizeof(T) == 2;
  const bool a16 = avec_aligned16(g.a.ptr) && avec_aligned16(g.W) && g.K % VEC == 0 && g.ldw % VEC == 0 &&
                   (mode != MODE_PLAIN || (g.a.ld % (f32src ? 4 : VEC) == 0));
  const bool plain_any = sizeof(T) == 2 && mode == MODE_PLAIN && !f32src && (g.K % 8 == 0 || g.K % 8 == 4) && g.K >= 8 && g.ldw >= g.K && g.a.ld >= g.K && g.a.step <= 1;
  g.ktail = (plain_any && g.K % 8 == 4) ? 4 : 0;
  if (g.perm2 && mode == MODE_CONV_BWD && g.fast_conv && a16 && !f32src) {
    g.pTs[0] = 0; for (int c = 0; c < 4; ++c) g.pTs[c + 1] = g.pTs[c] + (int)((perm2_count(g.a, c, g.pImgs) + BM - 1) / BM);
    grid.x = (unsigned)g.pTs[4];
  } else {
    if (g.e.res_cls0) { avec_set_error("gemm_nt: res_cls0: this launch cannot run in parity-class order (alignment)"); return -1; }
    g.perm2 = 0;
  }
  if constexpr (sizeof(T) == 2 && BN == 64 && BM == 64) {
    const long long arows = g.a.step > 1 ? (g.M / (g.a.rows_out > 0 ? g.a.rows_out : 1) + 1) * (long long)g.a.rows_in : g.M;
    if (mode == MODE_PLAIN && !f32src && g.a.step <= 1 && (g.K % 8 == 0 || g.ktail) && g.K >= 8 && g.ldw >= g.K && g.a.ld >= g.K &&
        arows * g.a.ld * 2 < (1ll << 32) && (long long)g.N * g.ldw * 2 < (1ll << 32)) {
      const bool tr = plain_tr_ok(g);
      if ((long long)grid.x * grid.y > 512 && !g.ktail && g.K <= 384) return tr ? launch_nt_plain<BM, BN, 2, true>(g, grid, st) : launch_nt_plain<BM, BN, 2, false>(g, grid, st);
      return tr ? launch_nt_plain<BM, BN, 4, true>(g, grid, st) : launch_nt_plain<BM, BN, 4, false>(g, grid, st);
    }
  }
  if constexpr (sizeof(T) == 2 && BM == 128 && (BN == 128 || BN == 64)) {
    static const bool no_clean = getenv("AVEC_NO_LEAN_CONV") != nullptr;
    if (mode != MODE_PLAIN && g.fast_conv && a16 && !f32src && !no_clean && g.a.C % 32 == 0 && (long long)g.N * g.ldw * 2 < (1ll << 32)) {
      const bool fwd = mode == MODE_CONV_FWD;
      if (epi_tr_ok(g)) return fwd ? launch_nt_conv_lean<BN, MODE_CONV_FWD, true>(g, grid, st) : launch_nt_conv_lean<BN, MODE_CONV_BWD, true>(g, grid, st);
      if (g.e.res_mask) { avec_set_error("gemm_nt: res_mask needs the register-direct epilogue"); return -1; }
      return fwd ? launch_nt_conv_lean<BN, MODE_CONV_FWD, false>(g, grid, st) : launch_nt_conv_lean<BN, MODE_CONV_BWD, false>(g, grid, st);
    }
  }
  if (g.e.res_mask) { avec_set_error("gemm_nt: res_mask needs the register-direct epilogue (no kernel with it takes this product)"); return -1; }
  static const bool rb_env_set = getenv("AVEC_NT_RB") != nullptr;
  static const int rb_env = rb_env_set ? atoi(getenv("AVEC_NT_RB")) : 128;
  const long long ntiles = (long long)grid.x * grid.y;
  const bool rb64 = sizeof(T) == 2 && (rb_env_set ? rb_env == 64 : ntiles >= 1536);
  const bool dma = (a16 || plain_any) && !f32src;
  if (mode == MODE_PLAIN) return launch_nt_general<T, BM, BN, MODE_PLAIN>(g, grid, dma, rb64, f32src, a16, st);
  if (mode == MODE_CONV_FWD) return launch_nt_general<T, BM, BN, MODE_CONV_FWD>(g, grid, dma, rb64, f32src, a16, st);
  return launch_nt_general<T, BM, BN, MODE_CONV_BWD>(g, grid, dma, rb64, f32src, a16, st);
}

static int launch_conv_shift(const GemmArgs& g_in, int mode, hipStream_t st) {
  static const bool off = getenv("AVEC_NO_CONV_SHIFT") != nullptr;
  const RowSrc& a = g_in.a;
  if (off || mode == MODE_PLAIN || a.KH != 3 || a.KW != 3 || a.stride != 1 || a.pad != 1 || a.H != a.OH || a.W != a.OW || a.W > 31 || a.C % 32 != 0) return 1;
  if (!avec_aligned16(a.ptr) || !avec_aligned16(g_in.W) || g_in.ldw % 8 != 0 || g_in.M * a.C >= (1ll << 31) || (long long)g_in.N * g_in.ldw >= (1ll << 31) || g_in.N < 64) return 1;
  GemmArgs g = g_in; g.perm2 = 0; g.pTs[0] = 1;
  static const int bm_env = getenv("AVEC_SHIFT_BM") ? atoi(getenv("AVEC_SHIFT_BM")) : 0;
  const long long t128 = ((g.M + 127) / 128) * ((g.N + 127) / 128), t256 = ((g.M + 255) / 256) * ((g.N + 127) / 128);
  const double e128 = (double)t128 / (double)(((t128 + 767) / 768) * 768), e256 = 1.08 * (double)t256 / (double)(((t256 + 511) / 512) * 512);
  const bool tr_ok = epi_tr_ok(g) && !g.e.res_cls0;
  const bool fwd = mode == MODE_CONV_FWD;
  if (g.N >= 128 && (bm_env == 256 || (bm_env == 0 && e256 > e128) || (g.e.res_mask && tr_ok))) {
    if (tr_ok) return fwd ? launch_shift<256, 128, MODE_CONV_FWD, true>(g, st) : launch_shift<256, 128, MODE_CONV_BWD, true>(g, st);
    return fwd ? launch_shift<256, 128, MODE_CONV_FWD, false>(g, st) : launch_shift<256, 128, MODE_CONV_BWD, false>(g, st);
  }
  if (g.e.res_mask) { avec_set_error("gemm_nt: res_mask needs the register-direct epilogue (N >= 128, bf16 output and residual in 16-byte pieces)"); return -1; }
  if (g.N >= 128) return fwd ? launch_shift<128, 128, MODE_CONV_FWD, false>(g, st) : launch_shift<128, 128, MODE_CONV_BWD, false>(g, st);
  return fwd ? launch_shift<128, 64, MODE_CONV_FWD, false>(g, st) : launch_shift<128, 64, MODE_CONV_BWD, false>(g, st);
}

template <typename T>
static int launch_nt(const GemmArgs& g, int mode, int src_f32, hipStream_t st) {
  long long t128 = ((g.M + 127) / 128) * ((g.N + 127) / 128);
  if (g.N > 64 && t128 >= 384) return launch_nt_mode<T, 128, 128>(g, mode, src_f32, st);
  const bool lean = sizeof(T) == 2 && mode == MODE_PLAIN && !src_f32 && g.K % 8 == 0 && ((g.M + 63) / 64) * ((g.N + 63) / 64) <= 4096;
  if (!lean && ((g.M + 127) / 128) * ((g.N + 63) / 64) >= 384) return launch_nt_mode<T, 128, 64>(g, mode, src_f32, st);
  return launch_nt_mode<T, 64, 64>(g, mode, src_f32, st);
}

extern "C" int avec_gemm_nt(int dtype, const void* A, const avec_rows_t* a_rows, int a_mode, int a_f32,
                            const void* W, long long ldw, long long M, int N, int K,
                            const avec_epilogue_t* ep, hipStream_t stream) {
  AVEC_CHECK_ARG(dtype == AVEC_F32 || dtype == AVEC_BF16, "gemm_nt: bad dtype %d", dtype);
  AVEC_CHECK_ARG(A && W && ep && ep->out && a_rows, "gemm_nt: null pointer");
  AVEC_CHECK_ARG(M > 0 && N > 0 && K > 0, "gemm_nt: bad dims M=%lld N=%d K=%d", M, N, K);
  AVEC_CHECK_ARG(a_mode >= 0 && a_mode <= 2, "gemm_nt: bad a_mode %d", a_mode);
  const int vec = dtype == AVEC_BF16 ? 8 : 4;
  AVEC_CHECK_ARG(K >= vec && (dtype == AVEC_F32 || (K % 2 == 0 && ldw % 2 == 0)), "gemm_nt: K=%d / ldw=%lld: need K >= %d and (bf16) even K, ldw (dword-aligned chunks)", K, ldw, vec);
  AVEC_CHECK_ARG(a_mode != AVEC_ROWS_PLAIN || dtype == AVEC_F32 || a_rows->ld % 2 == 0, "gemm_nt: lda=%lld must be even", a_rows->ld);
  AVEC_CHECK_ARG(!(a_f32 && dtype == AVEC_BF16) || K % 4 == 0, "gemm_nt: fp32-source staging needs K %% 4 == 0 (K=%d)", K);
  AVEC_CHECK_ARG(a_mode == AVEC_ROWS_PLAIN || (a_rows->C % vec == 0 && K == a_rows->KH * a_rows->KW * a_rows->C),
                 "gemm_nt: conv C=%d must be a multiple of %d and K = KH*KW*C", a_rows->C, vec);
  GemmArgs g; g.a = make_src(A, a_rows); g.W = W; g.ldw = ldw; g.M = M; g.N = N; g.K = K;
  g.fast_conv = 0; g.perm2 = 0; g.pImgs = 0; g.ktail = 0; for (int c = 0; c < 5; ++c) g.pTs[c] = 0;
  if (a_mode != AVEC_ROWS_PLAIN) {
    const int KE = dtype == AVEC_BF16 ? 64 : 32;
    const long long imgs = a_mode == MODE_CONV_FWD ? (M + (long long)a_rows->OH * a_rows->OW - 1) / ((long long)a_rows->OH * a_rows->OW) : (M + (long long)a_rows->H * a_rows->W - 1) / ((long long)a_rows->H * a_rows->W);
    const long long src_elems = imgs * (a_mode == MODE_CONV_FWD ? (long long)a_rows->H * a_rows->W : (long long)a_rows->OH * a_rows->OW) * a_rows->C;
    g.fast_conv = a_rows->C % KE == 0 && a_rows->KH * a_rows->KW <= 32 && src_elems + (long long)(a_rows->W + a_rows->OW + 2) * a_rows->C * 4 < (1ll << 31) &&
                  (a_mode == MODE_CONV_FWD || a_rows->stride == 1 || a_rows->stride == 2);
    static const bool no_perm = getenv("AVEC_NO_PERM2") != nullptr;
    if (!no_perm && dtype == AVEC_BF16 && g.fast_conv && a_mode == MODE_CONV_BWD && a_rows->stride == 2 && M == imgs * (long long)a_rows->H * a_rows->W) {
      g.perm2 = 1; g.pImgs = imgs;
    }
  }
  Epi& e = g.e;
  e = make_epi(ep);
  e.bnb_y = ep->bnb_y; e.ldby = ep->ldby; e.bnb_ss = ep->bnb_ss; e.bnb_mask = ep->bnb_mask; e.res_cls0 = ep->res_cls0; e.res_mask = ep->res_mask;
  AVEC_CHECK_ARG(!e.res_mask || (dtype == AVEC_BF16 && !a_f32 && a_mode != AVEC_ROWS_PLAIN && e.res && e.res_act && !e.res_cls0 && e.ldres % 8 == 0),
                 "gemm_nt: res_mask needs a bf16 convolution product with a bf16 residual whose rows are whole 8-element pieces");
  AVEC_CHECK_ARG(!e.res_cls0 || (g.perm2 && e.res), "gemm_nt: res_cls0 needs a bf16 stride-2 backward-data product that runs in parity-class order");
  AVEC_CHECK_ARG(!e.bnb_y || (e.stats && N % 4 == 0 && !(e.ldo & 3) && !(e.ldby & 3) && !(e.ldres & 3) && !(e.ldz & 3) && !(e.ldpre & 3) && (!e.bnb_mask || e.bnb_ss) && (e.bnb_mask || e.dact == 2 || e.dact == 0)),
                 "gemm_nt: the BatchNorm-backward fusion needs stats, N %% 4 == 0 and row strides that are multiples of 4");
  AVEC_CHECK_ARG(!(e.drop_p > 0.f) || e.rng, "gemm_nt: dropout without rng state");
  int r = 1;
  if (dtype == AVEC_BF16 && !a_f32 && a_mode != AVEC_ROWS_PLAIN) r = launch_conv_shift(g, a_mode, stream);
  if (r == 1 && dtype == AVEC_BF16 && !a_f32 && a_mode != AVEC_ROWS_PLAIN) r = avec_launch_conv_s2(g, a_mode, stream);
  if (r == 1) r = (dtype == AVEC_BF16) ? launch_nt<bf16>(g, a_mode, a_f32, stream) : launch_nt<float>(g, a_mode, a_f32, stream);
  if (r) return r;
  AVEC_LAUNCH_CHECK();
  return 0;
}


template <int BM, int BN, int STG>
static int launch_nt_fp8(const GemmArgs& g, const float* amax_a, const float* amax_w, hipStream_t st) {
  const dim3 grid((unsigned)((g.M + BM - 1) / BM), (unsigned)((g.N + BN - 1) / BN));
  const size_t lds = max_lds((size_t)STG * (BM + BN) * 128, epi_lds(BN));
  const auto kernel = gemm_nt_fp8_kernel<BM, BN, STG>;
  if (int r = avec_lds_optin(kernel, lds)) return r;
  hipLaunchKernelGGL(kernel, grid, dim3(256), lds, st, g, amax_a, amax_w);
  return 0;
}
extern "C" int avec_gemm_nt_fp8(const void* A, long long lda, const void* W, long long ldw, long long M, int N, int K,
                                const float* amax_a, const float* amax_w, const avec_epilogue_t* ep, hipStream_t stream) {
  AVEC_CHECK_ARG(A && W && ep && ep->out && amax_a && amax_w, "gemm_nt_fp8: null pointer");
  AVEC_CHECK_ARG(M > 0 && N > 0 && K > 0 && K % 16 == 0 && lda % 16 == 0 && ldw % 16 == 0 && avec_aligned16(A) && avec_aligned16(W),
                 "gemm_nt_fp8: M=%lld N=%d K=%d lda=%lld ldw=%lld: K and the row strides must be multiples of 16 bytes, operands 16-byte aligned", M, N, K, lda, ldw);
  GemmArgs g; memset(&g, 0, sizeof(g));
  g.a.ptr = A; g.a.ld = lda; g.W = W; g.ldw = ldw; g.M = M; g.N = N; g.K = K;
  g.e = make_epi(ep);
  AVEC_CHECK_ARG(!(g.e.drop_p > 0.f) || g.e.rng, "gemm_nt_fp8: dropout without rng state");
  const long long t128 = ((M + 127) / 128) * ((N + 127) / 128);
  int r;
  if (N > 64 && t128 >= 384) r = launch_nt_fp8<128, 128, 2>(g, amax_a, amax_w, stream);
  else if (((M + 127) / 128) * ((N + 63) / 64) >= 384) r = launch_nt_fp8<128, 64, 2>(g, amax_a, amax_w, stream);
  else r = launch_nt_fp8<64, 64, 4>(g, amax_a, amax_w, stream);
  if (r) return r;
  AVEC_LAUNCH_CHECK();
  return 0;
}

static thread_local TnMulti* tn_collect = nullptr;
template <typename T, int BI, int BJ, int MODE, bool F32SRC, bool A16>
static int launch_tn_generic(const TnArgs& g, dim3 grid, hipStream_t st) {
  return avec_launch(gemm_tn_kernel<T, BI, BJ, MODE, F32SRC, A16>, grid, dim3(256), (size_t)2 * (BI + BJ) * LDS_ROW, st, {g},
                     "gemm_tn_kernel<%s,%d,%d,%d,%d,%d>", elt_name<T>(), BI, BJ, MODE, (int)F32SRC, (int)A16);
}
template <int BI, int BJ, int MODE, bool Q32, int KT>
static int launch_tn_tr(TnArgs g, dim3 grid, hipStream_t st) {
  g.q_nwrap = (KT + g.q_ohw - 1) / g.q_ohw;
  return avec_launch(gemm_tn_tr_kernel<BI, BJ, MODE, 2, Q32, KT>, grid, dim3(256), (size_t)2 * KT * (BI + BJ) * 2, st, {g},
                     "gemm_tn_tr_kernel<%d,%d,%d,2,%d,%d>", BI, BJ, MODE, (int)Q32, KT);
}
template <int BI, int BJ, int KT>
static int launch_tn_tr_mode(const TnArgs& g, int mode, dim3 grid, hipStream_t st) {
  if (mode == MODE_PLAIN) return launch_tn_tr<BI, BJ, MODE_PLAIN, false, KT>(g, grid, st);
  const long long q_elems = ((g.M + (long long)g.q.OH * g.q.OW - 1) / ((long long)g.q.OH * g.q.OW) + 1) * g.q.H * g.q.W * g.q.C;
  return q_elems < (1ll << 31) ? launch_tn_tr<BI, BJ, MODE_CONV_FWD, true, KT>(g, grid, st) : launch_tn_tr<BI, BJ, MODE_CONV_FWD, false, KT>(g, grid, st);
}

template <typename T, int BI, int BJ>
static int launch_tn_tile(TnArgs g, int mode, int q_f32, int nbatch, hipStream_t st) {
  constexpr int KE = BKB / (int)sizeof(T);
  int tiles = ((g.I + BI - 1) / BI) * ((g.J + BJ - 1) / BJ) * nbatch;
  long long ksteps = (g.M + KE - 1) / KE;
  static const long long wg_env = getenv("AVEC_TN_WGS") ? atoll(getenv("AVEC_TN_WGS")) : 0;
  const long long wg_target = wg_env > 0 ? wg_env : (mode != MODE_PLAIN ? 896 : 512);
  long long split = (wg_target + tiles - 1) / tiles; if (split > ksteps / 4) split = ksteps / 4; if (split < 1 || g.Oact) split = 1;
  long long per = ((ksteps + split - 1) / split) * KE;
  split = (g.M + per - 1) / per;
  g.m_per_block = (int)per; g.split = (int)split;
  dim3 grid((g.I + BI - 1) / BI, (g.J + BJ - 1) / BJ, (unsigned)(split * nbatch));
  constexpr int VEC = Elt<T>::VEC;
  const bool f32src = q_f32 && sizeof(T) == 2;
  const bool a16 = nbatch == 1 && avec_aligned16(g.P) && avec_aligned16(g.q.ptr) && g.Iq % VEC == 0 && g.Jq % VEC == 0 && g.ldp % VEC == 0 &&
                   (mode != MODE_PLAIN || (g.q.ld % (f32src ? 4 : VEC) == 0));
  if (sizeof(T) == 2 && a16 && !f32src && !g.Oact && (mode == MODE_PLAIN || g.q_mg != 0)) {
    static const int kt_env = getenv("AVEC_TN_KT") ? atoi(getenv("AVEC_TN_KT")) : 32;
    return kt_env == 64 ? launch_tn_tr_mode<BI, BJ, 64>(g, mode, grid, st) : launch_tn_tr_mode<BI, BJ, 32>(g, mode, grid, st);
  }
  if (g.pcs) {
    if (int r = colsum_launch(sizeof(T) == 2 ? AVEC_BF16 : AVEC_F32, g.P, g.ldp, g.pcs, g.M, g.I, true, st)) return r;
  }
  if (tn_collect && sizeof(T) == 2 && BI == 64 && BJ == 64 && mode == MODE_PLAIN && !f32src && !a16 && !g.pcs && tn_collect->n < AVEC_TN_MULTI_MAX) {
    TnMulti& m = *tn_collect; const int k = m.n++;
    m.g[k] = g; m.gx[k] = (int)grid.x; m.gy[k] = (int)grid.y; m.first[k + 1] = m.first[k] + (int)(grid.x * grid.y * grid.z);
    return 0;
  }
  if (mode == MODE_PLAIN) {
    if constexpr (sizeof(T) == 2) {
      if (f32src) return a16 ? launch_tn_generic<T, BI, BJ, MODE_PLAIN, true, true>(g, grid, st) : launch_tn_generic<T, BI, BJ, MODE_PLAIN, true, false>(g, grid, st);
    }
    return a16 ? launch_tn_generic<T, BI, BJ, MODE_PLAIN, false, true>(g, grid, st) : launch_tn_generic<T, BI, BJ, MODE_PLAIN, false, false>(g, grid, st);
  }
  return a16 ? launch_tn_generic<T, BI, BJ, MODE_CONV_FWD, false, true>(g, grid, st) : launch_tn_generic<T, BI, BJ, MODE_CONV_FWD, false, false>(g, grid, st);
}

static int gemm_tn_impl(int dtype, const void* P, long long ldp, const void* Q, const avec_rows_t* q_rows, int q_mode, int q_f32,
                        float* O, void* Oact, long long ldo, long long M, int I, int J, int nb_outer, int nb_inner, const long long* strides, float* p_colsum, hipStream_t stream) {
  AVEC_CHECK_ARG(dtype == AVEC_F32 || dtype == AVEC_BF16, "gemm_tn: bad dtype %d", dtype);
  AVEC_CHECK_ARG(P && Q && (O || Oact) && q_rows, "gemm_tn: null pointer");
  AVEC_CHECK_ARG(M > 0 && I > 0 && J > 0 && nb_outer > 0 && nb_inner > 0, "gemm_tn: bad dims");
  AVEC_CHECK_ARG(q_mode == MODE_PLAIN || q_mode == MODE_CONV_FWD, "gemm_tn: bad q_mode %d", q_mode);
  const int vec = dtype == AVEC_BF16 ? 8 : 4;
  const int Jq = (q_mode == MODE_PLAIN && q_rows->ld >= (J + vec - 1) / vec * vec) ? (J + vec - 1) / vec * vec : J;
  const int Iq = (ldp >= (I + vec - 1) / vec * vec) ? (I + vec - 1) / vec * vec : I;
  AVEC_CHECK_ARG(Iq >= vec && Jq >= vec && (dtype == AVEC_F32 || (Iq % 2 == 0 && Jq % 2 == 0 && ldp % 2 == 0)), "gemm_tn: I=%d, J=%d: need >= %d and (bf16) even I, J, ldp", I, J, vec);
  AVEC_CHECK_ARG(q_mode != MODE_PLAIN || dtype == AVEC_F32 || q_rows->ld % 2 == 0, "gemm_tn: ldq must be even");
  AVEC_CHECK_ARG(q_mode == MODE_PLAIN || q_rows->C % vec == 0, "gemm_tn: conv C=%d must be a multiple of %d", q_rows->C, vec);
  AVEC_CHECK_ARG(!(q_f32 && dtype == AVEC_BF16) || Jq % 4 == 0, "gemm_tn: fp32-source staging needs J %% 4 == 0");
  TnArgs g; g.P = P; g.ldp = ldp; g.q = make_src(Q, q_rows); g.O = O; g.Oact = Oact; g.ldo = ldo; g.M = M; g.I = I; g.J = J; g.Iq = Iq; g.Jq = Jq; g.m_per_block = 0; g.pcs = p_colsum;
  g.split = 1; g.nb_inner = nb_inner;
  g.q_ohw = 1; g.q_mg = 0; g.q_nwrap = 0;
  if (q_mode != MODE_PLAIN && q_rows->OW > 0 && q_rows->OH > 0 && (long long)q_rows->OH * q_rows->OW <= 4096) {
    const int ohw = q_rows->OH * q_rows->OW; const unsigned mg = ((1u << 20) + (unsigned)q_rows->OW - 1u) / (unsigned)q_rows->OW;
    bool exact = true; for (int px = 0; px < ohw && exact; ++px) exact = (int)(((unsigned)px * mg) >> 20) == px / q_rows->OW;
    g.q_ohw = ohw; g.q_mg = exact ? (int)mg : 0;
  }
  g.xcd_map = 1;
  g.sPo = strides ? strides[0] : 0; g.sPi = strides ? strides[1] : 0; g.sQo = strides ? strides[2] : 0; g.sQi = strides ? strides[3] : 0;
  g.sOo = strides ? strides[4] : 0; g.sOi = strides ? strides[5] : 0;
  if (dtype == AVEC_BF16 && strides) for (int i = 0; i < 2; ++i) AVEC_CHECK_ARG(strides[i] % 2 == 0, "gemm_tn: bf16 batch strides of P must be even");
  const int nbatch = nb_outer * nb_inner;
  bool big = (I >= 128 && J >= 128) && ((long long)((I + 127) / 128) * ((J + 127) / 128) * nbatch >= 48 || M >= 32768);
  int r;
  const bool wide = !big && I <= 64 && J >= 128 && M >= 32768 && dtype == AVEC_BF16 && !q_f32 && nbatch == 1 && avec_aligned16(P) && avec_aligned16(Q) && Iq % 8 == 0 && Jq % 8 == 0 &&
                    ldp % 8 == 0 && (q_mode != MODE_PLAIN || q_rows->ld % 8 == 0);
  if (dtype == AVEC_BF16) r = big ? launch_tn_tile<bf16, 128, 128>(g, q_mode, q_f32, nbatch, stream) : wide ? launch_tn_tile<bf16, 64, 128>(g, q_mode, q_f32, nbatch, stream)
                                                                                                    : launch_tn_tile<bf16, 64, 64>(g, q_mode, q_f32, nbatch, stream);
  else r = big ? launch_tn_tile<float, 128, 128>(g, q_mode, q_f32, nbatch, stream) : launch_tn_tile<float, 64, 64>(g, q_mode, q_f32, nbatch, stream);
  if (r) return r;
  AVEC_LAUNCH_CHECK();
  return 0;
}

extern "C" int avec_gemm_tn(int dtype, const void* P, long long ldp, const void* Q, const avec_rows_t* q_rows, int q_mode, int q_f32,
                            float* O, long long ldo, long long M, int I, int J, hipStream_t stream) {
  return gemm_tn_impl(dtype, P, ldp, Q, q_rows, q_mode, q_f32, O, nullptr, ldo, M, I, J, 1, 1, nullptr, nullptr, stream);
}
extern "C" int avec_gemm_tn_bias(int dtype, const void* P, long long ldp, const void* Q, const avec_rows_t* q_rows, int q_mode, int q_f32,
                                 float* O, long long ldo, float* p_colsum, long long M, int I, int J, hipStream_t stream) {
  AVEC_CHECK_ARG(!p_colsum || (I % 4 == 0 && ldp % 4 == 0), "gemm_tn_bias: column sums need I %% 4 == 0 and ldp %% 4 == 0");
  return gemm_tn_impl(dtype, P, ldp, Q, q_rows, q_mode, q_f32, O, nullptr, ldo, M, I, J, 1, 1, nullptr, p_colsum, stream);
}

extern "C" int avec_gemm_tn_batched(int dtype, const void* P, long long ldp, const void* Q, long long ldq, float* O, long long ldo, long long M, int I, int J,
                                    int nb_outer, int nb_inner, const long long* strides6, hipStream_t stream) {
  avec_rows_t rows = {}; rows.ld = ldq;
  AVEC_CHECK_ARG(strides6, "gemm_tn_batched: null strides");
  return gemm_tn_impl(dtype, P, ldp, Q, &rows, MODE_PLAIN, 0, O, nullptr, ldo, M, I, J, nb_outer, nb_inner, strides6, nullptr, stream);
}
extern "C" int avec_gemm_tn_batched_store(int dtype, const void* P, long long ldp, const void* Q, long long ldq, void* O_act, long long ldo, long long M, int I, int J,
                                          int nb_outer, int nb_inner, const long long* strides6, hipStream_t stream) {
  avec_rows_t rows = {}; rows.ld = ldq;
  AVEC_CHECK_ARG(strides6 && O_act, "gemm_tn_batched_store: null pointer");
  return gemm_tn_impl(dtype, P, ldp, Q, &rows, MODE_PLAIN, 0, nullptr, O_act, ldo, M, I, J, nb_outer, nb_inner, strides6, nullptr, stream);
}

extern "C" int avec_gemm_tn_batched_multi(int dtype, const avec_tn_batched_t* items, int n, hipStream_t stream) {
  AVEC_CHECK_ARG(items && n >= 1 && n <= AVEC_TN_MULTI_MAX, "gemm_tn_batched_multi: need 1..%d problems (got %d)", AVEC_TN_MULTI_MAX, n);
  TnMulti m; m.n = 0; m.first[0] = 0;
  tn_collect = &m;
  int rc = 0;
  for (int k = 0; k < n && rc == 0; ++k) {
    const avec_tn_batched_t& t = items[k];
    avec_rows_t rows = {}; rows.ld = t.ldq;
    if (!t.strides6 || (!t.O && !t.O_act)) { avec_set_error("gemm_tn_batched_multi: problem %d: null pointer", k); rc = -1; break; }
    rc = gemm_tn_impl(dtype, t.P, t.ldp, t.Q, &rows, MODE_PLAIN, 0, t.O_act ? nullptr : t.O, t.O_act, t.ldo, t.M, t.I, t.J, t.nb_outer, t.nb_inner, t.strides6, nullptr, stream);
  }
  tn_collect = nullptr;
  if (rc) return rc;
  if (m.n > 0) {
    if (int r = avec_launch(gemm_tn_multi_kernel, dim3((unsigned)m.first[m.n]), dim3(256), (size_t)2 * (64 + 64) * LDS_ROW, stream, {m}, "gemm_tn_multi_kernel<%d>", m.n)) return r;
    AVEC_LAUNCH_CHECK();
  }
  return 0;
}

static bool tn_item_ok(int dtype, const avec_tn_item_t& t) {
  if (dtype != AVEC_BF16 || !t.P || !t.Q || !t.O || t.M <= 0 || t.I <= 0 || t.J <= 0) return false;
  if (t.ldp < t.I || t.ldq < t.J) return false;
  if (t.p_colsum && (t.I % 4 || t.ldp % 4)) return false;
  return t.M < (1ll << 31) && t.ldp < (1ll << 31) && t.ldq < (1ll << 31) && t.ldo < (1ll << 31);
}
template <int BT>
static int launch_tn_grouped(const TnGroup& grp, hipStream_t st) {
  constexpr int STG = 2, KT = 64;
  return avec_launch(gemm_tn_tr_grouped_kernel<BT, STG, KT>, dim3((unsigned)grp.total), dim3(256), (size_t)STG * KT * (BT + BT) * 2, st, {grp},
                     "gemm_tn_tr_grouped_kernel<%d,%d,%d>", BT, STG, KT);
}
extern "C" int avec_gemm_tn_grouped_ok(int dtype, const avec_tn_item_t* item) { return item && tn_item_ok(dtype, *item) ? 1 : 0; }

extern "C" int avec_gemm_tn_grouped(int dtype, const avec_tn_item_t* items, int n, hipStream_t stream) {
  AVEC_CHECK_ARG(items && n > 0 && n <= AVEC_TN_GROUP_MAX, "gemm_tn_grouped: need 1..%d items (got %d)", AVEC_TN_GROUP_MAX, n);
  for (int k = 0; k < n; ++k) AVEC_CHECK_ARG(tn_item_ok(dtype, items[k]), "gemm_tn_grouped: item %d is not eligible (bf16 operands, row strides >= widths, bias sums need I %% 4 == 0)", k);
  long long t128 = 0;
  for (int k = 0; k < n; ++k) t128 += (long long)((items[k].I + 127) / 128) * ((items[k].J + 127) / 128);
  const int BT = t128 >= 96 ? 128 : 64;
  const long long wg_target = 512;
  long long per = 256;
  for (long long cand = 8192; cand >= 256; cand -= 64) {
    long long wgs = 0;
    for (int k = 0; k < n; ++k) wgs += (long long)((items[k].I + BT - 1) / BT) * ((items[k].J + BT - 1) / BT) * ((items[k].M + cand - 1) / cand);
    if (wgs >= wg_target) { per = cand; break; }
  }
  TnGroup grp; grp.n = n;
  int first = 0;
  for (int k = 0; k < n; ++k) {
    const avec_tn_item_t& s = items[k]; TnItem& t = grp.it[k];
    t.P = s.P; t.Q = s.Q; t.O = s.O; t.pcs = s.p_colsum; t.ldp = (int)s.ldp; t.ldq = (int)s.ldq; t.ldo = (int)s.ldo; t.M = (int)s.M; t.I = s.I; t.J = s.J;
    t.Iq = (s.I + 7) / 8 * 8; t.Jq = (s.J + 7) / 8 * 8;
    t.rows_out = s.q_rows_out > 0 ? s.q_rows_out : 1; t.rows_in = s.q_rows_in > 0 ? s.q_rows_in : 1; t.step = s.q_step;
    long long mp = per; if (mp > s.M) mp = (s.M + 63) / 64 * 64;
    t.m_per_block = (int)mp; t.split = (int)((s.M + mp - 1) / mp);
    t.gx = (s.I + BT - 1) / BT; t.gy = (s.J + BT - 1) / BT; t.first = first;
    first += t.gx * t.gy * t.split;
  }
  grp.total = first;
  grp.xcd_map = 1;
  if (int r = BT == 128 ? launch_tn_grouped<128>(grp, stream) : launch_tn_grouped<64>(grp, stream)) return r;
  AVEC_LAUNCH_CHECK();
  return 0;
}
```

### avec_amd/ops.py

```python
import collections
import ctypes
import os

import torch

from . import fp8
from . import runtime as rt
from .lib import (ACT_GELU, ACT_NONE, ACT_RELU, ACT_SWISH, BF16, LN_GROUP_MAX, ROWS_CONV_BWD, ROWS_CONV_FWD, ROWS_PLAIN, ROWS_STEM3D, TN_GROUP_MAX, WGRAD_GROUP_MAX, Attn, Epilogue, LnItem, Rows, TnBatched, TnItem,
                  WgradItem, lib)

_byref = ctypes.byref


class KernelTimer:
    NAMES = {(0, ROWS_CONV_FWD): "gemm_nt<conv_fwd>", (0, ROWS_CONV_BWD): "gemm_nt<conv_bwd_data>", (0, ROWS_STEM3D): "gemm_nt<stem3d>",
             (0, ROWS_PLAIN): "gemm_nt<plain>", (1, ROWS_CONV_FWD): "gemm_tn<conv_wgrad>", (1, ROWS_STEM3D): "gemm_tn<stem3d_wgrad>",
             (1, ROWS_PLAIN): "gemm_tn<plain>", (2, 0): "conv3x3_slab<fwd>", (2, 1): "conv3x3_slab<bwd_data>", (2, 2): "conv3x3_slab<wgrad>"}

    def __init__(self):
        self.enabled = False
        self.records = []

    def reset(self, enabled):
        self.enabled, self.records = enabled, []

    def start(self):
        e = torch.cuda.Event(enable_timing=True)
        e.record()
        return e

    def stop(self, e0, key, flops, abytes=0.0):
        e1 = torch.cuda.Event(enable_timing=True)
        e1.record()
        name = lib.raw("avec_last_kernel")()
        self.records.append((key, flops, e0, e1, name.decode() if name else "", float(abytes)))

    def bracket_overhead_us(self, n=200):
        evs = []
        for _ in range(n):
            a, b = torch.cuda.Event(enable_timing=True), torch.cuda.Event(enable_timing=True)
            a.record(); b.record()
            evs.append((a, b))
        torch.cuda.synchronize()
        d = sorted(a.elapsed_time(b) * 1e3 for a, b in evs)
        return d[len(d) // 2]

    def summary(self, peak_tflops, steps=1):
        if not self.records:
            return None
        torch.cuda.synchronize()
        ovh = self.bracket_overhead_us() * 1e-6
        agg, rows = {}, {}
        for key, flops, e0, e1, name, ab in self.records:
            dt = max(e0.elapsed_time(e1) * 1e-3 - ovh, 1e-7)
            a = agg.setdefault(key, [0.0, 0.0, 0])
            a[0] += dt; a[1] += flops; a[2] += 1
            r = rows.setdefault(name or self.NAMES.get(key, str(key)), [0.0, 0.0, 0, 0.0])
            r[0] += dt; r[1] += flops; r[2] += 1; r[3] += ab

        def row(name, v):
            return {"kernel": name, "launches_per_step": round(v[2] / steps, 1), "avg_us": round(1e6 * v[0] / v[2], 2), "ms_per_step": round(1e3 * v[0] / steps, 3),
                    "alg_gflop_per_launch": round(v[1] / v[2] / 1e9, 3), "alg_bytes_per_launch": round(v[3] / v[2]), "tflops": round(v[1] / v[0] / 1e12, 1),
                    "frac": round(v[1] / v[0] / 1e12 / peak_tflops, 4)}
        ordered = sorted(rows.items(), key=lambda kv: -kv[1][0])
        top_name, top = ordered[0]
        t_all = sum(v[0] for v in rows.values()); f_all = sum(v[1] for v in rows.values())
        achieved = top[1] / top[0] / 1e12
        return {"bound": "mfma", "kernel": top_name, "achieved": round(achieved, 2), "peak": peak_tflops, "unit": "TFLOP/s",
                "frac": round(achieved / peak_tflops, 5), "traffic": None, "launches": round(top[2] / steps, 1), "avg_launch_ms": round(1e3 * top[0] / top[2], 5),
                "alg_gflop_per_launch": round(top[1] / top[2] / 1e9, 3), "alg_bytes_per_launch": round(top[3] / top[2]),
                "event_bracket_overhead_us": round(ovh * 1e6, 2),
                "rows": [row(n, v) for n, v in ordered[:8]],
                "gemm_family_total": {"ms_per_step": round(1e3 * t_all / steps, 3), "tflops": round(f_all / t_all / 1e12, 1), "frac": round(f_all / t_all / 1e12 / peak_tflops, 4)},
                "families": {self.NAMES.get(k, str(k)): {"ms_total": round(1e3 * v[0] / steps, 3), "tflops": round(v[1] / v[0] / 1e12, 2), "launches": round(v[2] / steps, 1)}
                             for k, v in sorted(agg.items(), key=lambda kv: -kv[1][0])}}


KERNEL_TIMER = KernelTimer()


def _p(t):
    return None if t is None else t.data_ptr()


STAMPS = {"on": os.environ.get("AVEC_STAMPS", "0") == "1", "buf": None, "names": []}


def stamp(name):
    if not STAMPS["on"]:
        return
    if STAMPS["buf"] is None:
        STAMPS["buf"] = torch.zeros(256, dtype=torch.int64, device="cuda")
    if name not in STAMPS["names"]:
        STAMPS["names"].append(name)
    lib.stamp(STAMPS["buf"].data_ptr(), STAMPS["names"].index(name), rt.stream())


class StampFn(torch.autograd.Function):

    @staticmethod
    def forward(ctx, x, name):
        ctx.name = name
        stamp(name + ":f")
        return x.view_as(x)

    @staticmethod
    def backward(ctx, g):
        stamp(ctx.name + ":b")
        return g, None


def mark(x, name):
    return StampFn.apply(x, name) if (STAMPS["on"] and torch.is_tensor(x) and x.requires_grad) else (stamp(name + ":f") or x)


def grad_of(p):
    if p.grad is None:
        p.grad = torch.zeros_like(p)
    return p.grad


def empty(shape, dtype, ref):
    if dtype == torch.bfloat16 and len(shape) == 2 and shape[1] % 8:
        n = shape[0] * shape[1]
        return torch.empty(n + 8, dtype=dtype, device=ref.device)[:n].view(shape)
    return torch.empty(shape, dtype=dtype, device=ref.device)


TN_MULTI = True
ATTN_ODD_VALU = False


def _chunk_readable(t, ld, width, rows):
    if width % 8 == 0 and ld % 8 == 0 and t.data_ptr() % 16 == 0:
        return True
    if ld >= (width + 7) // 8 * 8:
        return True
    st = t.untyped_storage()
    end = (t.storage_offset() + (rows - 1) * ld + (width + 7) // 8 * 8) * t.element_size()
    return end <= st.nbytes()


def rows_plain(ld, rows_out=1, rows_in=1, step=0):
    r = Rows()
    r.ld, r.rows_out, r.rows_in, r.step = ld, rows_out, rows_in, step
    return r


def rows_conv(H, W, C, KH, KW, stride, pad, OH, OW):
    r = Rows()
    r.H, r.W, r.C, r.KH, r.KW, r.stride, r.pad, r.OH, r.OW = H, W, C, KH, KW, stride, pad, OH, OW
    return r


def gemm_nt_fp8(A, ent, out, M, N, K, *, bias=None, act=ACT_NONE, out_pre=None, drop_p=0.0, sid=0, res=None, alpha=1.0, out_f32=False, ldo=None):
    Kp = ent.Kp
    q = torch.empty((M, Kp), dtype=torch.uint8, device=A.device)
    lib.fp8_quantize(rt.dt(), A.data_ptr(), K, q.data_ptr(), Kp, M, K, ent.a_amax, 1, rt.stream())
    ep = Epilogue()
    ep.out, ep.ldo, ep.out_f32 = out.data_ptr(), (N if ldo is None else ldo), int(out_f32)
    if out_pre is not None:
        ep.out_pre, ep.ldpre = out_pre.data_ptr(), N
    ep.bias, ep.act, ep.alpha = _p(bias), act, alpha
    if drop_p > 0.0:
        ep.drop_p, ep.rng, ep.rng_stream = drop_p, rt.rng_state(out.device).data_ptr(), sid
    if res is not None:
        ep.res, ep.ldres, ep.res_act = res.data_ptr(), N, 0
    ev = KERNEL_TIMER.start() if KERNEL_TIMER.enabled else None
    lib.gemm_nt_fp8(q.data_ptr(), Kp, ent.wq, Kp, M, N, Kp, ent.a_amax, ent.w_amax, _byref(ep), rt.stream())
    if ev is not None:
        KERNEL_TIMER.stop(ev, (0, 0), 2.0 * M * N * K)
    return out


def gemm_nt(A, W, out, M, N, K, *, rows=None, mode=ROWS_PLAIN, a_f32=False, ldw=None, bias=None, act=ACT_NONE, out_pre=None,
            drop_p=0.0, sid=0, res=None, res_act=False, alpha=1.0, dact_z=None, dact=0, colsum=None, stats=None, out_f32=False,
            ldo=None, ldres=None, dtype=None, flops=None, bnb=None, res_cls0=False, abytes=None, res_mask=None):
    ep = Epilogue()
    ep.out, ep.ldo, ep.out_f32 = out.data_ptr(), (N if ldo is None else ldo), int(out_f32)
    if out_pre is not None:
        ep.out_pre, ep.ldpre = out_pre.data_ptr(), N
    ep.bias = _p(bias)
    ep.act = act
    if drop_p > 0.0:
        ep.drop_p, ep.rng, ep.rng_stream = drop_p, rt.rng_state(out.device).data_ptr(), sid
    if res is not None:
        ep.res, ep.ldres, ep.res_act, ep.res_cls0 = res.data_ptr(), (N if ldres is None else ldres), int(res_act), int(res_cls0)
        if res_mask is not None:
            ep.res_mask = res_mask.data_ptr()
    ep.alpha = alpha
    if dact_z is not None:
        ep.dact_z, ep.ldz, ep.dact = dact_z.data_ptr(), N, dact
    ep.colsum, ep.stats = _p(colsum), _p(stats)
    if bnb is not None:
        ep.bnb_y, ep.ldby, ep.stats = bnb.y.data_ptr(), N, bnb.stats.data_ptr()
        if bnb.mask_z is not None:
            ep.dact_z, ep.ldz, ep.dact, ep.bnb_mask = bnb.mask_z.data_ptr(), N, 2, 0
        else:
            ep.bnb_ss, ep.bnb_mask = bnb.ss.data_ptr(), 1
    if rows is None:
        rows = rows_plain(K)
    ev = KERNEL_TIMER.start() if KERNEL_TIMER.enabled else None
    lib.gemm_nt(rt.dt() if dtype is None else dtype, A.data_ptr(), _byref(rows), mode, int(a_f32), W.data_ptr(),
                K if ldw is None else ldw, M, N, K, _byref(ep), rt.stream())
    if ev is not None:
        esz = A.element_size()
        KERNEL_TIMER.stop(ev, (0, mode), 2.0 * M * N * K if flops is None else flops,
                          ((M * K + N * K) * esz + M * N * (4 if out_f32 else esz)) if abytes is None else abytes)
    return out


DEFER_WGRAD = os.environ.get("AVEC_DEFER_WGRAD", "1") != "0"


_QueueKind = collections.namedtuple("_QueueKind", "item group_max launcher dtype timer_key abytes flush_when_full")


def _wgrad3x3_bytes(it):
    return 2.0 * 2 * it.images * it.H * it.W * it.C + 4.0 * 9 * it.C * it.C


_QUEUE_KINDS = {
    "tn": _QueueKind(TnItem, TN_GROUP_MAX, "gemm_tn_grouped", lambda: BF16, (1, ROWS_PLAIN), lambda it: 2.0 * it.M * (it.I + it.J) + 4.0 * it.I * it.J, True),
    "ln": _QueueKind(LnItem, LN_GROUP_MAX, "layernorm_param_grads_grouped", rt.dt, None, None, True),
    "cw": _QueueKind(WgradItem, WGRAD_GROUP_MAX, "wgrad3x3_c128_grouped", None, (2, 2), _wgrad3x3_bytes, False),
    "cw64": _QueueKind(WgradItem, WGRAD_GROUP_MAX, "wgrad3x3_c64_grouped", None, (2, 2), _wgrad3x3_bytes, False),
}


class _PendingGrads:
    __slots__ = ("stream", "items", "flops", "keep")

    def __init__(self, stream):
        self.stream = stream
        self.clear()

    def clear(self):
        self.items, self.flops, self.keep = {k: [] for k in _QUEUE_KINDS}, dict.fromkeys(_QUEUE_KINDS, 0.0), []

    def push(self, kind, item, keep, flops=0.0):
        self.items[kind].append(item)
        self.keep += keep
        self.flops[kind] += flops
        if _QUEUE_KINDS[kind].flush_when_full and len(self.items[kind]) >= _QUEUE_KINDS[kind].group_max:
            self.flush((kind,))

    def flush(self, kinds=None):
        cur = torch.cuda.current_stream()
        if cur.cuda_stream != self.stream.cuda_stream:
            for t in self.keep:
                t.record_stream(cur)
        for kind in (_QUEUE_KINDS if kinds is None else kinds):
            k, items = _QUEUE_KINDS[kind], self.items[kind]
            if not items:
                continue
            ev = KERNEL_TIMER.start() if (k.timer_key is not None and KERNEL_TIMER.enabled) else None
            for i in range(0, len(items), k.group_max):
                chunk = items[i:i + k.group_max]
                getattr(lib, k.launcher)(*(() if k.dtype is None else (k.dtype(),)), (k.item * len(chunk))(*chunk), len(chunk), rt.stream())
            if ev is not None:
                KERNEL_TIMER.stop(ev, k.timer_key, self.flops[kind], sum(k.abytes(it) for it in items))
            self.items[kind], self.flops[kind] = [], 0.0
        if not any(self.items.values()):
            self.keep = []


class _BackwardPass:
    __slots__ = ("task", "queues", "prep", "ln2", "pos", "bn_ready")

    def __init__(self, task):
        self.task = task
        self.queues = {}
        self.prep = {}
        self.ln2 = {}
        self.pos = {}
        self.bn_ready = {}

    def pending(self):
        st = torch.cuda.current_stream()
        q = self.queues.get(st.cuda_stream)
        if q is None:
            q = self.queues[st.cuda_stream] = _PendingGrads(st)
        return q
# ... 376 lines not shown


_POS_CACHE = {}
_POS_EPOCH = [0]


class _PosGroupEntry:
    __slots__ = ("e_all", "pe", "L", "D", "Tp", "capture")


def invalidate_pos_cache():
    _POS_CACHE.clear()
    _POS_EPOCH[0] += 1


def _pos_group_entry(wp, Tp, D, device):
    if rt.compute_dtype() != "bf16":
        return None, 0
    grp = rt.fused_group(wp)
    if grp is None or len(grp.weights) < 2 or fp8.enabled():
        return None, 0
    idx = next((k for k, w in enumerate(grp.weights) if w is wp), None)
    if idx is None:
        return None, 0
    arena = wp._avec_shadow.arena
    key = (id(grp), Tp, str(device))
    ent = _POS_CACHE.get(key)
    ver = (getattr(arena, "refresh_count", 0), torch.cuda.current_stream().cuda_stream)
    if ent is None or ent[0] != ver:
        L = len(grp.weights)
        e = _PosGroupEntry()
        e.L, e.D, e.Tp, e.pe = L, D, Tp, rel_pos_table(Tp, D, device)
        e.capture = _POS_EPOCH[0] if torch.cuda.is_current_stream_capturing() else None
        e.e_all = empty((2 * Tp - 1, L * D), rt.act_dtype(), e.pe)
        gemm_nt(e.pe, grp.fwd, e.e_all, 2 * Tp - 1, L * D, D, bias=grp.bias)
        _POS_CACHE[key] = ent = (ver, e, grp)
        if len(_POS_CACHE) > 64:
            for k in list(_POS_CACHE)[:32]:
                _POS_CACHE.pop(k, None)
    elif ent[1].capture is not None and torch.cuda.is_current_stream_capturing():
        assert ent[1].capture == _POS_EPOCH[0], "E built inside one captured graph must not be served to a later capture"
    return ent[1], idx


def _pos_group_backward(entry, wp):
    acc = _pass().pos[entry]
    acc[1] -= 1
    if acc[1] > 0:
        return
    de_all = _pass().pos.pop(entry)[0]
    grp = rt.fused_group(wp)
    R, W = 2 * entry.Tp - 1, entry.L * entry.D
    dea = empty((R, W), rt.act_dtype(), de_all)
    lib.cast_rows(rt.dt(), de_all.data_ptr(), W, dea.data_ptr(), W, R, W, rt.stream())
    gemm_tn(dea, entry.pe, grp.wgrad, R, W, entry.D, p_colsum=grp.bgrad, side=True)


class AttentionModuleFn(torch.autograd.Function):
    @staticmethod
    def forward(ctx, x, lens, mask, ln_w, ln_b, wq, bq, wk, bk, wv, bv, wo, bo, wp, bp, H, patch, eps, drop_p, sid, residual):
        rt.require_gpu(x)
        B, T, D = x.shape
        M, d, adt = B * T, D // H, rt.act_dtype()
        grp = rt.fused_group(wq)
        grp_ok = grp is not None and grp.weights[1] is wk and grp.weights[2] is wv and bq is not None
        x2 = _f32c(x.reshape(-1, D))
        if ln_w is not None:
            h, mean, rstd = layernorm_fwd(x2, ln_w, ln_b, M, D, False, eps)
        else:
            mean = rstd = None
            h = empty((M, D), adt, x2)
            lib.cast_rows(rt.dt(), x2.data_ptr(), D, h.data_ptr(), D, M, D, rt.stream())
        if patch > 1:
            Tp = (T + patch - 1) // patch
            hp = empty((B * Tp, D), adt, x2)
            lib.patch_pool_fwd(rt.dt(), h.data_ptr(), hp.data_ptr(), B, T, D, patch, rt.stream())
        else:
            Tp, hp = T, h
        Mp = B * Tp
        if mask is not None:
            mask = mask.reshape(mask.shape[0], T, T) if patch == 1 else _pool_mask(mask, T, patch)
            mask = mask.float().contiguous()
        if grp_ok:
            qkv = empty((Mp, 3 * D), adt, x2)
            ent = fp8.entry(wq, D)
            if ent is not None and ent.N == 3 * D:
                gemm_nt_fp8(hp, ent, qkv, Mp, 3 * D, D, bias=grp.bias)
            else:
                gemm_nt(hp, grp.fwd, qkv, Mp, 3 * D, D, bias=grp.bias)
        else:
            qkv = empty((Mp, 3 * D), adt, x2)
            for i, (w, b) in enumerate(((wq, bq), (wk, bk), (wv, bv))):
                sh = rt.shadow(w)
                gemm_nt(hp, sh.fwd, qkv[:, i * D:], Mp, D, D, bias=b, ldo=3 * D)
        pg, pgi = _pos_group_entry(wp, Tp, D, x.device)
        if pg is not None:
            pe, e = pg.pe, pg.e_all[:, pgi * D:(pgi + 1) * D]
        else:
            pe = rel_pos_table(Tp, D, x.device)
            e = linear_fwd(pe, wp, bp, 2 * Tp - 1, in_f32=False, out_f32=False)
        o = empty((Mp, D), adt, x2)
        lse = empty((B * H, Tp, 2), torch.float32, x2)
        q_full = T // patch if (patch > 1 and mask is None) else 0
        a = _attn_args(qkv, e, lens, patch, mask, o, lse, B, H, Tp, d, D, q_full)
        lib.relpos_attention_fwd(rt.dt(), _byref(a), rt.stream())
        res = x2 if residual else None
        if patch > 1:
            oo = linear_fwd(o, wo, bo, Mp, in_f32=False, out_f32=False)
            base = x2 if residual else torch.zeros_like(x2)
            y = empty((M, D), torch.float32, x2)
            rng = rt.rng_state(x.device).data_ptr() if drop_p > 0 else None
            lib.patch_unpool_add(rt.dt(), oo.data_ptr(), base.data_ptr(), y.data_ptr(), drop_p, rng, sid, B, T, D, patch, rt.stream())
        else:
            y = linear_fwd(o, wo, bo, M, in_f32=False, out_f32=True, drop_p=drop_p, sid=sid, res=res, alpha=1.0)
        ctx.saved = (x2, mean, rstd, h, hp, qkv, pe, e, o, lse, lens, mask, ln_w, ln_b, wq, bq, wk, bk, wv, bv, wo, bo, wp, bp,
                     H, patch, drop_p, sid, residual, B, T, Tp, D)
        ctx.pos_group = (pg, pgi)
        ctx.prep_req = _prep_request(x)
        return _tag_prep(y.view(B, T, D), 1.0, drop_p, sid) if patch == 1 else y.view(B, T, D)

    @staticmethod
    def backward(ctx, dy):
        (x2, mean, rstd, h, hp, qkv, pe, e, o, lse, lens, mask, ln_w, ln_b, wq, bq, wk, bk, wv, bv, wo, bo, wp, bp,
         H, patch, drop_p, sid, residual, B, T, Tp, D) = ctx.saved
        M, Mp, d, adt = B * T, B * Tp, D // H, rt.act_dtype()
        dy = _f32c(dy.reshape(M, D))
        if patch > 1:
            doo = empty((Mp, D), adt, dy)
            rng = rt.rng_state(dy.device).data_ptr() if drop_p > 0 else None
            lib.patch_unpool_bwd(rt.dt(), dy.data_ptr(), doo.data_ptr(), drop_p, rng, sid, B, T, D, patch, rt.stream())
        else:
            doo = _take_prep(dy, M, D, 1.0, drop_p, sid)
            if doo is None:
                doo = grad_prep(dy, M, D, drop_p=drop_p, sid=sid)
        linear_bwd_weight(doo, o, wo, Mp, bias=bo)
        do = torch.empty(Mp * D + 8, dtype=adt, device=dy.device)[:Mp * D].view(Mp, D)
        do = linear_bwd_input(doo, wo, Mp, out_f32=False, out=do)
        dqkv = empty((Mp, 3 * D), adt, dy)
        pg, pgi = ctx.pos_group
        if pg is not None:
            acc = _pass().pos.get(pg)
            if acc is None:
                acc = _pass().pos[pg] = [rt.zeros_scratch((2 * Tp - 1) * pg.L * D, dy.device).view(2 * Tp - 1, pg.L * D), pg.L]
            de = acc[0][:, pgi * D:(pgi + 1) * D]
        else:
            de = rt.zeros_scratch((2 * Tp - 1) * D, dy.device).view(2 * Tp - 1, D)
        a = _attn_args(qkv, e, lens, patch, mask, o, lse, B, H, Tp, d, D, T // patch if (patch > 1 and mask is None) else 0)
        a.dout = do.data_ptr()
        esz = dqkv.element_size()
        a.dq, a.lddq = dqkv.data_ptr(), 3 * D
        a.dk, a.dv, a.ldd = dqkv.data_ptr() + D * esz, dqkv.data_ptr() + 2 * D * esz, 3 * D
        a.de, a.ldde = de.data_ptr(), de.stride(0)
        Tld, Rld = (Tp + 7) // 8 * 8, (2 * Tp - 1 + 7) // 8 * 8
        scratch = empty((2, B * H, Tp, Tld), adt, dy)
        a.pbuf, a.dsbuf, a.ldt = scratch.data_ptr(), scratch.data_ptr() + scratch[0].numel() * esz, Tld
        use_mfma = d % 2 == 0 or not ATTN_ODD_VALU
        if use_mfma:
            n_rel = H * B * Tp * Rld
            if adt == torch.bfloat16:
                dsrel = rt.zeros_scratch((n_rel + 1) // 2, dy.device).view(torch.bfloat16)[:n_rel].view(H, B * Tp, Rld)
            else:
                dsrel = rt.zeros_scratch(n_rel, dy.device).view(H, B * Tp, Rld)
            a.dsrel, a.ldr = dsrel.data_ptr(), Rld
        lib.relpos_attention_bwd(rt.dt(), _byref(a), rt.stream())
        if use_mfma:
            L6 = ctypes.c_longlong * 6
            sK, sV, sE = L6(H * Tp * Tld, Tp * Tld, Tp * 3 * D, d, Tp * 3 * D, d), L6(H * Tp * Tld, Tp * Tld, Tp * D, d, Tp * 3 * D, d), L6(0, B * Tp * Rld, 0, d, 0, d)
            if TN_MULTI:
                it = (TnBatched * 3)()
                it[0].P, it[0].ldp, it[0].Q, it[0].ldq, it[0].O_act, it[0].ldo = a.dsbuf, Tld, qkv.data_ptr(), 3 * D, dqkv.data_ptr() + D * esz, 3 * D
                it[0].M, it[0].I, it[0].J, it[0].nb_outer, it[0].nb_inner, it[0].strides6 = Tp, Tp, d, B, H, sK
                it[1].P, it[1].ldp, it[1].Q, it[1].ldq, it[1].O_act, it[1].ldo = a.pbuf, Tld, do.data_ptr(), D, dqkv.data_ptr() + 2 * D * esz, 3 * D
                it[1].M, it[1].I, it[1].J, it[1].nb_outer, it[1].nb_inner, it[1].strides6 = Tp, Tp, d, B, H, sV
                it[2].P, it[2].ldp, it[2].Q, it[2].ldq, it[2].O, it[2].ldo = dsrel.data_ptr(), Rld, qkv.data_ptr(), 3 * D, de.data_ptr(), de.stride(0)
                it[2].M, it[2].I, it[2].J, it[2].nb_outer, it[2].nb_inner, it[2].strides6 = B * Tp, 2 * Tp - 1, d, 1, H, sE
                lib.gemm_tn_batched_multi(rt.dt(), it, 3, rt.stream())
            else:
                lib.gemm_tn_batched_store(rt.dt(), a.dsbuf, Tld, qkv.data_ptr(), 3 * D, dqkv.data_ptr() + D * esz, 3 * D, Tp, Tp, d, B, H, sK, rt.stream())
                lib.gemm_tn_batched_store(rt.dt(), a.pbuf, Tld, do.data_ptr(), D, dqkv.data_ptr() + 2 * D * esz, 3 * D, Tp, Tp, d, B, H, sV, rt.stream())
                lib.gemm_tn_batched(rt.dt(), dsrel.data_ptr(), Rld, qkv.data_ptr(), 3 * D, de.data_ptr(), de.stride(0), B * Tp, 2 * Tp - 1, d, 1, H, sE, rt.stream())
        dhp = None
        grp = rt.fused_group(wq)
        if grp is not None and grp.weights[1] is wk and grp.weights[2] is wv and bq is not None:
            gemm_tn(dqkv, hp, grp.wgrad, Mp, 3 * D, D, p_colsum=grp.bgrad, side=True)
            dhp = empty((Mp, D), adt, dy)
            gemm_nt(dqkv, grp.bwd, dhp, Mp, D, 3 * D)
        else:
            for i, (w, b) in enumerate(((wq, bq), (wk, bk), (wv, bv))):
                g = dqkv[:, i * D:]
                linear_bwd_weight(g, hp, w, Mp, ldp=3 * D, bias=b)
                dhp = linear_bwd_input(g, w, Mp, out_f32=False, lda=3 * D, res=dhp, res_act=True, out=dhp)
        if pg is not None:
            _pos_group_backward(pg, wp)
        else:
            dea = empty((2 * Tp - 1, D), adt, dy)
            lib.cast_rows(rt.dt(), de.data_ptr(), D, dea.data_ptr(), D, 2 * Tp - 1, D, rt.stream())
            linear_bwd_weight(dea, pe, wp, 2 * Tp - 1, bias=bp)
        if patch > 1:
            dh = empty((M, D), adt, dy)
            lib.patch_pool_bwd(rt.dt(), dhp.data_ptr(), dh.data_ptr(), B, T, D, patch, rt.stream())
        else:
            dh = dhp
        if ln_w is not None:
            dx = layernorm_bwd(dh, False, x2, mean, rstd, ln_w, ln_b, M, D, dres=dy if residual else None, prep=ctx.prep_req)
        else:
            dx = dy.clone() if residual else torch.zeros_like(dy)
            lib.to_f32_rows(rt.dt(), dh.data_ptr(), D, dx.data_ptr(), D, M, D, 1, rt.stream())
        return (dx.view(B, T, D),) + (None,) * 20


class RelPosCoreFn(torch.autograd.Function):

    @staticmethod
    def forward(ctx, qkv, e, lens, len_div, mask, B, H, T, d, scale):
        rt.require_gpu(qkv)
        D, adt = H * d, rt.act_dtype()
        assert qkv.dtype == adt and e.dtype == adt and qkv.is_contiguous() and e.is_contiguous() and qkv.shape == (B * T, 3 * D) and e.shape == (2 * T - 1, D)
        assert d % 2 == 0, "the batched-GEMM backward needs an even head width (pad the operands)"
        if mask is not None:
            mask = mask.reshape(mask.shape[0], T, T).float().contiguous()
        o = empty((B * T, D), adt, qkv)
        lse = empty((B * H, T, 2), torch.float32, qkv)
        a = _attn_args(qkv, e, lens, len_div, mask, o, lse, B, H, T, d, D)
        a.scale = scale
        lib.relpos_attention_fwd(rt.dt(), _byref(a), rt.stream())
        ctx.saved = (qkv, e, o, lse, lens, len_div, mask, B, H, T, d, scale)
        return o

    @staticmethod
    def backward(ctx, do):
        qkv, e, o, lse, lens, len_div, mask, B, H, T, d, scale = ctx.saved
        D, adt = H * d, rt.act_dtype()
        do = do.to(adt).contiguous()
        dqkv = empty((B * T, 3 * D), adt, do)
        de = torch.zeros((2 * T - 1, D), dtype=torch.float32, device=do.device)
        a = _attn_args(qkv, e, lens, len_div, mask, o, lse, B, H, T, d, D)
        a.scale = scale
        a.dout = do.data_ptr()
        esz = dqkv.element_size()
        a.dq, a.lddq = dqkv.data_ptr(), 3 * D
        a.dk, a.dv, a.ldd = dqkv.data_ptr() + D * esz, dqkv.data_ptr() + 2 * D * esz, 3 * D
        a.de, a.ldde = de.data_ptr(), D
        Tld, Rld = (T + 7) // 8 * 8, (2 * T - 1 + 7) // 8 * 8
        scratch = empty((2, B * H, T, Tld), adt, do)
        a.pbuf, a.dsbuf, a.ldt = scratch.data_ptr(), scratch.data_ptr() + scratch[0].numel() * esz, Tld
        dsrel = torch.zeros((H, B * T, Rld), dtype=adt, device=do.device)
        a.dsrel, a.ldr = dsrel.data_ptr(), Rld
        lib.relpos_attention_bwd(rt.dt(), _byref(a), rt.stream())
        L6 = ctypes.c_longlong * 6
        lib.gemm_tn_batched_store(rt.dt(), a.dsbuf, Tld, qkv.data_ptr(), 3 * D, dqkv.data_ptr() + D * esz, 3 * D, T, T, d, B, H,
                                  L6(H * T * Tld, T * Tld, T * 3 * D, d, T * 3 * D, d), rt.stream())
        lib.gemm_tn_batched_store(rt.dt(), a.pbuf, Tld, do.data_ptr(), D, dqkv.data_ptr() + 2 * D * esz, 3 * D, T, T, d, B, H,
                                  L6(H * T * Tld, T * Tld, T * D, d, T * 3 * D, d), rt.stream())
        lib.gemm_tn_batched(rt.dt(), dsrel.data_ptr(), Rld, qkv.data_ptr(), 3 * D, de.data_ptr(), D, B * T, 2 * T - 1, d, 1, H,
                            L6(0, B * T * Rld, 0, d, 0, d), rt.stream())
        return dqkv, de.to(adt), None, None, None, None, None, None, None, None


def relpos_core_infer(q, k, v, e, lens, mask, B, H, T, Tk, d, scale, want_probs=False):
    rt.require_gpu(q)
    D, adt = H * d, rt.act_dtype()
    for t in (q, k, v, e):
        assert t.dtype == adt and t.is_contiguous()
    assert q.shape == (B * T, D) and k.shape == (B * Tk, D) and v.shape == (B * Tk, D) and e.shape == (Tk + T - 1, D)
    if mask is not None:
        mask = mask.reshape(mask.shape[0], T, Tk).float().contiguous()
    o = empty((B * T, D), adt, q)
    lse = empty((B * H, T, 2), torch.float32, q)
    a = Attn()
    a.q, a.k, a.v, a.ld = q.data_ptr(), k.data_ptr(), v.data_ptr(), D
    a.e, a.lde = e.data_ptr(), D
    a.lens, a.len_div = _p(lens), 1
    if mask is not None:
        a.mask, a.mask_bstride = mask.data_ptr(), (T * Tk if mask.shape[0] > 1 else 0)
    a.o, a.ldo, a.lse = o.data_ptr(), D, lse.data_ptr()
    a.B, a.H, a.T, a.d, a.scale, a.Tk = B, H, T, d, scale, Tk
    lib.relpos_attention_fwd(rt.dt(), _byref(a), rt.stream())
    if not want_probs:
        return o, None
    Tld = (Tk + 7) // 8 * 8
    scratch = empty((2, B * H, T, Tld), adt, q)
    dq = empty((B * T, D), adt, q)
    zero = torch.zeros((B * T, D), dtype=adt, device=q.device)
    dsrel = torch.zeros((H, B * T, (Tk + T - 1 + 7) // 8 * 8), dtype=adt, device=q.device)
    a.dout, a.dq, a.lddq = zero.data_ptr(), dq.data_ptr(), D
    a.pbuf, a.dsbuf, a.ldt = scratch.data_ptr(), scratch.data_ptr() + scratch[0].numel() * scratch.element_size(), Tld
    a.dsrel, a.ldr = dsrel.data_ptr(), dsrel.shape[2]
    lib.relpos_attention_bwd(rt.dt(), _byref(a), rt.stream())
    return o, scratch[0].view(B, H, T, Tld)[..., :Tk].float()


def _pool_mask(mask, T, P):
    pad = (P - T % P) % P
    m = torch.nn.functional.pad(mask.reshape(mask.shape[0], 1, T, T).float(), (0, pad, 0, pad), value=0.0)
    Tp = (T + pad) // P
    return m.reshape(m.shape[0], Tp, P, Tp, P).amin(dim=(2, 4))


class BNState:

    NREP = 64

    def __init__(self, C, ref):
        self.stats = rt.zeros_scratch(self.NREP * 2 * C, ref.device)
        self.red = None
        self.ss = torch.empty(4 * C, dtype=torch.float32, device=ref.device)
        self.C = C


RELU_BITMASK = True
def bn_finalize(bn, st, count, training):
    C = st.C
    cptr = None
    sptr, nrep = st.stats.data_ptr(), st.NREP
    if training and rt.sync_batchnorm():
        st.red = rt.sync_bn_stats(st.stats, st.NREP, C, count, key=(id(bn), "f"))
        sptr, nrep, cptr = st.red.data_ptr(), 1, st.red.data_ptr() + 2 * C * 4
# ... 1065 lines not shown
```

### include/avec_hip.h

```cpp
#ifndef AVEC_HIP_H
#define AVEC_HIP_H
#include <stdint.h>
#ifdef __HIPCC__
#include <hip/hip_runtime.h>
#else
typedef struct ihipStream_t* hipStream_t;
#endif
#ifdef __cplusplus
extern "C" {
#endif

#define AVEC_F32 0
#define AVEC_BF16 1
#define AVEC_ABI_VERSION 4
#define AVEC_STAT_REPLICAS 64

int avec_version(void);
int avec_struct_size(int which);
const char* avec_last_error(void);
const char* avec_last_kernel(void);
int avec_set_reduce_workspace(void* base, long long bytes);
int avec_set_reduce_workspace_stream(void* base, long long bytes, hipStream_t stream);

enum { AVEC_ROWS_PLAIN = 0, AVEC_ROWS_CONV_FWD = 1, AVEC_ROWS_CONV_BWD = 2 };
typedef struct avec_rows {
  long long ld;
  int rows_out, rows_in, step;
  int H, W, C, KH, KW, stride, pad, OH, OW;
  int T3;
} avec_rows_t;

typedef struct avec_epilogue {
  void* out; long long ldo; int out_f32;
  void* out_pre; long long ldpre;
  const float* bias;
  int act;
  float drop_p; const unsigned long long* rng; unsigned rng_stream;
  const void* res; long long ldres; float alpha; int res_act;
  const void* dact_z; long long ldz; int dact;
  float* colsum;
  float* stats;
  const void* bnb_y; long long ldby; const float* bnb_ss; int bnb_mask;
  int res_cls0;
  const unsigned char* res_mask;
} avec_epilogue_t;

int avec_gemm_nt(int dtype, const void* A, const avec_rows_t* a_rows, int a_mode, int a_f32,
                 const void* W, long long ldw, long long M, int N, int K,
                 const avec_epilogue_t* ep, hipStream_t stream);

typedef struct { const float* src; void* dst; long long n; int slot; int K, Kp; int reserved; } avec_fp8_item_t;
int avec_fp8_quantize(int src_dtype, const void* x, long long ldx, void* q, long long ldq, long long M, int K, float* amax, int compute_amax, hipStream_t stream);
int avec_fp8_weights_refresh(const avec_fp8_item_t* table, int n_items, int blocks_per_item, float* amax, hipStream_t stream);
int avec_gemm_nt_fp8(const void* A, long long lda, const void* W, long long ldw, long long M, int N, int K,
                     const float* amax_a, const float* amax_w, const avec_epilogue_t* ep, hipStream_t stream);


int avec_gemm_tn(int dtype, const void* P, long long ldp, const void* Q, const avec_rows_t* q_rows, int q_mode, int q_f32,
                 float* O, long long ldo, long long M, int I, int J, hipStream_t stream);
int avec_gemm_tn_bias(int dtype, const void* P, long long ldp, const void* Q, const avec_rows_t* q_rows, int q_mode, int q_f32,
                      float* O, long long ldo, float* p_colsum, long long M, int I, int J, hipStream_t stream);
#define AVEC_TN_GROUP_MAX 32
typedef struct avec_tn_item {
  const void* P; const void* Q; float* O; float* p_colsum;
  long long ldp, ldq, ldo, M;
  int I, J;
  int q_rows_out, q_rows_in, q_step;
  int reserved;
} avec_tn_item_t;
int avec_gemm_tn_grouped_ok(int dtype, const avec_tn_item_t* item);
int avec_gemm_tn_grouped(int dtype, const avec_tn_item_t* items, int n, hipStream_t stream);
int avec_gemm_tn_batched(int dtype, const void* P, long long ldp, const void* Q, long long ldq, float* O, long long ldo, long long M, int I, int J,
                         int nb_outer, int nb_inner, const long long* strides6, hipStream_t stream);
int avec_gemm_tn_batched_store(int dtype, const void* P, long long ldp, const void* Q, long long ldq, void* O_act, long long ldo, long long M, int I, int J,
                               int nb_outer, int nb_inner, const long long* strides6, hipStream_t stream);

typedef struct {
  const void* P; long long ldp; const void* Q; long long ldq;
  float* O; void* O_act; long long ldo;
  long long M; int I, J, nb_outer, nb_inner;
  const long long* strides6;
} avec_tn_batched_t;
int avec_gemm_tn_batched_multi(int dtype, const avec_tn_batched_t* items, int n, hipStream_t stream);

#define AVEC_PEER_MAX_WORLD 8
int avec_peer_exchange_sum(const float* in, float* out, int n, void* const* pages, long long page_stride_granules, int rank, int world,
                           unsigned* epoch, int* err_flag, int timeout_ms, hipStream_t stream);
int avec_peer_exchange_sum_fused(const float* in, int n_replicas, int n_in, int has_tail, float tail, float* dgamma, float* dbeta, int C, float* out,
                                 void* const* pages, long long page_stride_granules, int rank, int world, unsigned* epoch, int* err_flag, int timeout_ms,
                                 hipStream_t stream);
int avec_enable_peer_access(int peer_device);
int avec_peer_buffer_alloc(void** ptr, long long bytes, void* ipc_handle_64b);
int avec_peer_buffer_open(const void* ipc_handle_64b, void** ptr);
int avec_peer_buffer_close(void* ptr);
int avec_peer_buffer_free(void* ptr);

int avec_layernorm_fwd(int dtype, const float* x, const float* gamma, const float* beta, void* y, int y_f32,
                       float* mean, float* rstd, long long M, int D, float eps, hipStream_t stream);
int avec_layernorm_bwd(int dtype, const void* dy, int dy_f32, const float* x, const float* mean, const float* rstd, const float* gamma,
                       float* dx, const float* dres, float* dgamma, float* dbeta, long long M, int D, hipStream_t stream);
int avec_layernorm_bwd_prep(int dtype, const void* dy, int dy_f32, const float* x, const float* mean, const float* rstd, const float* gamma,
                            float* dx, const float* dres, void* prep, float prep_alpha, float prep_drop_p, const unsigned long long* rng, unsigned rng_stream,
                            long long M, int D, hipStream_t stream);
int avec_layernorm_fwd2(int dtype, const float* x, const float* gamma1, const float* beta1, float eps1, float* y1, float* mean1, float* rstd1,
                        const float* gamma2, const float* beta2, float eps2, void* h2, float* mean2, float* rstd2, long long M, int D, hipStream_t stream);
int avec_layernorm_bwd2(int dtype, const void* dy2, const float* x2, const float* mean2, const float* rstd2, const float* gamma2, const float* dres2, float* dx2,
                        const float* x1, const float* mean1, const float* rstd1, const float* gamma1, float* dx1,
                        void* prep, float prep_alpha, float prep_drop_p, const unsigned long long* rng, unsigned rng_stream, long long M, int D, hipStream_t stream);
#define AVEC_LN_GROUP_MAX 40
typedef struct avec_ln_item {
  const void* dy; const float* x; const float* mean; const float* rstd; float* dgamma; float* dbeta;
  long long M; int D; int dy_f32;
} avec_ln_item_t;
int avec_layernorm_param_grads_grouped(int dtype, const avec_ln_item_t* items, int n, hipStream_t stream);
int avec_grad_prep(int dtype, const float* dout, long long ld, void* dacc, float alpha, float drop_p, const unsigned long long* rng,
                   unsigned rng_stream, float* dbias, long long M, int N, hipStream_t stream);
int avec_colsum(int dtype, const void* x, long long ld, float* out, long long M, int N, hipStream_t stream);
int avec_strided_rows_add(float* dx, const float* src, int B, int T, int To, int D, int step, hipStream_t stream);
int avec_bn_stats(int dtype, const void* y, float* stats, long long M, int C, hipStream_t stream);
int avec_bn_collapse(const float* stats, int n_replicas, float count, float* out, int C, hipStream_t stream);
int avec_bn_affine_grads(const float* dstats, float* dgamma, float* dbeta, int C, hipStream_t stream);
int avec_bn_finalize(const float* stats, int n_replicas, const float* count_ptr, float count, const float* gamma, const float* beta, float* running_mean,
                     float* running_var, long long* num_batches_tracked, float momentum, float eps, float* ss, int C, int training, hipStream_t stream);
int avec_stamp(unsigned long long* out, int slot, hipStream_t stream);
int avec_bn_bwd_finalize(const float* stats, int n_replicas, const float* ss, float* dstats, int C, hipStream_t stream);
int avec_bn_apply_fwd(int dtype, const void* y, const float* ss, const void* residual, int act, void* out, long long M, int C, hipStream_t stream);
int avec_bn_bwd_reduce(int dtype, const void* dout, const void* y, const void* out, const float* ss, int act, float* dstats, long long M, int C, hipStream_t stream);
int avec_bn_bwd_apply(int dtype, const void* dout, const void* y, const void* out, const float* ss, const float* gamma, const float* dstats,
                      const float* count_ptr, float count, int act, void* dy, void* dres, float* dgamma, float* dbeta, long long M, int C, hipStream_t stream);
int avec_bn_apply_fwd_mask(int dtype, const void* y, const float* ss, const void* residual, const float* residual_ss, void* out, unsigned char* mask, long long M, int C,
                           hipStream_t stream);
int avec_bn_bwd_reduce_mask(int dtype, const void* dout, const void* y, const unsigned char* mask, const float* ss, float* dstats, long long M, int C, hipStream_t stream);
int avec_bn_bwd_apply_mask(int dtype, const void* dout, const void* y, const unsigned char* mask, const float* ss, const float* gamma, const float* dstats,
                           const float* count_ptr, float count, void* dy, void* dres, float* dgamma, float* dbeta, long long M, int C, hipStream_t stream);
int avec_softmax_fwd(int dtype, const float* logits, void* probs, long long M, int V, hipStream_t stream);
int avec_softmax_bwd(int dtype, const void* dprobs, const float* logits, float* dlogits, const float* dadd, long long M, int V, hipStream_t stream);
int avec_cast_rows(int dtype, const float* src, long long ld_src, void* dst, long long ld_dst, long long M, int N, hipStream_t stream);
int avec_to_f32_rows(int dtype, const void* src, long long ld_src, float* dst, long long ld_dst, long long M, int N, int accum, hipStream_t stream);
int avec_act_f32(int act, const float* x, const float* dy, float* out, long long rows, int C, int backward, hipStream_t stream);
int avec_dropout_f32(const float* x, float* y, float p, const unsigned long long* rng, unsigned rng_stream, long long n, hipStream_t stream);
int avec_maxpool_hw_fwd(int dtype, const void* x, void* out, unsigned char* idx, long long frames, int H, int W, int C, int KH, int KW, int SH, int SW,
                        int pad0_h, int pad0_w, int pad1_h, int pad1_w, hipStream_t stream);
int avec_maxpool_hw_bwd(int dtype, const void* dy, const unsigned char* idx, void* dx, long long frames, int H, int W, int C, int KH, int KW, int SH, int SW,
                        int pad0_h, int pad0_w, int pad1_h, int pad1_w, hipStream_t stream);
int avec_upsample_rows(int dtype, const void* src, void* dst, long long B, int T, int D, int P, int backward, hipStream_t stream);
int avec_patch_pool_fwd(int dtype, const void* x, void* y, int B, int T, int D, int P, hipStream_t stream);
int avec_patch_pool_bwd(int dtype, const void* dy, void* dx, int B, int T, int D, int P, hipStream_t stream);
int avec_patch_unpool_add(int dtype, const void* o, const float* res, float* out, float drop_p, const unsigned long long* rng, unsigned rng_stream,
                          int B, int T, int D, int P, hipStream_t stream);
int avec_patch_unpool_bwd(int dtype, const float* dout, void* dob, float drop_p, const unsigned long long* rng, unsigned rng_stream,
                          int B, int T, int D, int P, hipStream_t stream);
int avec_avgpool_fwd(int dtype, const void* x, void* y, long long N, int HW, int C, hipStream_t stream);
int avec_avgpool_bwd(int dtype, const void* dy, void* dx, long long N, int HW, int C, hipStream_t stream);

int avec_glu_dwconv_fwd(int dtype, const void* u, const float* w, const float* bias, void* out, float* stats,
                        int B, int T, int C, int K, int stride, int pad_left, hipStream_t stream);
int avec_glu_dwconv_fwd_bn(int dtype, const void* u, const float* w, const float* bias, void* out, float* stats, int B, int T, int C, int K, int stride, int pad_left,
                           const float* gamma, const float* beta, float* running_mean, float* running_var, long long* num_batches_tracked, float momentum, float eps,
                           float* ss, hipStream_t stream);
int avec_dwconv_glu_bwd(int dtype, const void* dc, const void* u, const float* w, void* du, float* dw, float* dbias,
                        int B, int T, int C, int K, int stride, int pad_left, hipStream_t stream);
int avec_dwconv_glu_bwd_bn(int dtype, const void* da, const void* c, const float* ss, const float* gamma, const float* dstats, float count, const void* u, const float* w,
                           void* du, float* dw, float* dbias, float* dgamma, float* dbeta, int B, int T, int C, int K, int pad_left, hipStream_t stream);

typedef struct avec_attn {
  const void *q, *k, *v; long long ld;
  const void* e; long long lde;
  const long long* lens; int len_div;
  int q_full;
  const float* mask; long long mask_bstride;
  void* o; long long ldo; float* lse;
  const void* dout;
  void *dq, *dk, *dv; long long lddq, ldd;
  float* de; long long ldde;
  void *pbuf, *dsbuf; long long ldt;
  void* dsrel; long long ldr;
  int B, H, T, d; float scale;
  int Tk;
} avec_attn_t;
int avec_relpos_attention_fwd(int dtype, const avec_attn_t* args, hipStream_t stream);
int avec_relpos_attention_bwd(int dtype, const avec_attn_t* args, hipStream_t stream);

long long avec_glu_dwconv_stream_state_bytes(int dtype, int B, int C, int K);
int avec_glu_dwconv_stream(int dtype, const void* u, const float* w, const float* bias, const float* ss, void* out, void* state, long long state_bytes,
                           const long long* pos, const unsigned char* reset, const long long* chunk_len, int div, int B, int Tq, int C, int K, int stride, hipStream_t stream);
long long avec_relpos_attention_stream_state_bytes(int dtype, int B, int H, int d, int L, int Tq);
int avec_relpos_attention_stream(int dtype, const void* q, const void* k, const void* v, long long ld, const void* e, long long lde, void* kcache, void* vcache,
                                 long long cache_bytes, const long long* pos, const unsigned char* reset, const long long* chunk_len, int div, void* o, long long ldo,
                                 int B, int H, int Tq, int d, int L, float scale, hipStream_t stream);
int avec_stream_advance(long long* pos, unsigned char* reset, const long long* chunk_len, long long full, int B, hipStream_t stream);

int avec_mel_frames(const float* audio, const float* window, float* frames, int B, long long L, int n_fft, int win, int hop, hipStream_t stream);
int avec_mel_power_log(const float* spec, const float* fb, float* out, int B, int F, int n_bins, int n_mels, hipStream_t stream);
int avec_specaugment(float* mel, const long long* lens, int B, int n_mels, int F, int mF, int Fparam, int mT, float pS,
                     const unsigned long long* rng, unsigned rng_stream, hipStream_t stream);
int avec_debug_rng_uniform(const unsigned long long* rng, unsigned rng_stream, const long long* ids, int n, float* out, hipStream_t stream);
int avec_audio_stem_conv_fwd(int dtype, const float* mel, const float* w, const float* bias, void* y, float* stats, int B, int n_mels, int F, int C, hipStream_t stream);
int avec_audio_stem_act_fwd(int dtype, const void* y, const float* ss, void* a, int B, int n_mels, int F, int C, hipStream_t stream);
int avec_audio_stem_bwd(int dtype, const void* da, const void* y, const float* mel, const float* ss, const float* gamma, float* dstats,
                        const float* count_ptr, float count, int phase, float* dw, float* dbias, float* dgamma, float* dbeta,
                        int B, int n_mels, int F, int C, hipStream_t stream);
int avec_stem_im2col(int dtype, const float* video, void* A, long long clips, int T, int H, int W, int ldk, hipStream_t stream);
int avec_stem3d_supported(long long clips, int T, int H, int W);
int avec_stem3d_fwd(const float* video, const void* w_shadow, int ldw, const float* bias, void* y, float* stats, long long clips, int T, int H, int W, hipStream_t stream);
int avec_stem3d_wgrad(const float* video, const void* dy, float* dw, long long clips, int T, int H, int W, hipStream_t stream);
int avec_stem3p_supported(long long clips, int T, int H, int W);
int avec_stem3p_fwd(const void* video_bf16, const void* w_shadow, const float* bias, const float* gamma, void* zp, unsigned char* idx, float* stats,
                    long long clips, int T, int H, int W, hipStream_t stream);
int avec_stem3p_reduce(void* dpool, const void* zp, const float* ss, float* dstats, long long frames, int PH, int PW, hipStream_t stream);
int avec_stem3p_wgrad_supported(long long clips, int T, int H, int W);
int avec_stem3p_wgrad(const void* video_bf16, const void* w_shadow, const float* bias, const void* dpool_masked, const unsigned char* idx, const float* ss,
                      const float* gamma, const float* dstats, const float* count_ptr, float count, float* dw, float* dgamma, float* dbeta,
                      long long clips, int T, int H, int W, hipStream_t stream);
int avec_stem3p_dz(const void* video_bf16, const void* w_shadow, const float* bias, const void* dpool_masked, const unsigned char* idx, const float* ss,
                   const float* gamma, const float* dstats, const float* count_ptr, float count, void* dz, float* dgamma, float* dbeta,
                   long long clips, int T, int H, int W, hipStream_t stream);
int avec_stem_pool_fwd(int dtype, const void* y, const float* ss, void* out, unsigned char* idx, void* ymax, long long frames, int H, int W, int C, hipStream_t stream);
int avec_stem_pool_bwd_reduce_pooled(int dtype, const void* dpool, const unsigned char* idx, const void* ymax, const float* ss, float* dstats,
                                     long long frames, int H, int W, int C, hipStream_t stream);
int avec_stem_pool_bwd(int dtype, const void* dpool, const unsigned char* idx, const void* y, const float* ss, const float* gamma, float* dstats,
                       const float* count_ptr, float count, int phase, void* dy, float* dgamma, float* dbeta, long long frames, int H, int W, int C, hipStream_t stream);

int avec_conv3x3_c64_supported(int H, int W, int Cin, int Cout, int KH, int KW, int stride);
int avec_conv3x3_c64(const void* x, const void* w, void* y, const void* res, float* stats, long long images, int H, int W, int flip, hipStream_t stream);
int avec_conv3x3_c64_res_masked(const void* x, const void* w, void* y, const void* res, const unsigned char* res_mask, long long images, int H, int W, int flip, hipStream_t stream);
int avec_wgrad3x3_c64(const void* x, const void* dy, float* dw, long long images, int H, int W, hipStream_t stream);
int avec_wgrad3x3_c128_supported(int H, int W, int Cin, int Cout, int KH, int KW, int stride);
int avec_wgrad3x3_c128(const void* x, const void* dy, float* dw, long long images, int C, int H, int W, hipStream_t stream);
#define AVEC_WGRAD_GROUP_MAX 16
typedef struct { const void* x; const void* dy; float* dw; long long images; int C, H, W, reserved; } avec_wgrad3x3_item_t;
int avec_wgrad3x3_c128_grouped(const avec_wgrad3x3_item_t* items, int n, hipStream_t stream);
int avec_wgrad3x3_c64_grouped(const avec_wgrad3x3_item_t* items, int n, hipStream_t stream);

int avec_video_input(const unsigned char* clips, const long long* clip_off, const int* geom, const int* masks, int max_masks, int channels, const float* lut, float mean, float stdv,
                     int mean_frame, float* out, float* frame_ws, int B, int Tout, int OH, int OW, hipStream_t stream);
int avec_video_tta_batch(const float* x, float* y, int B, long long rows, int W, int n, unsigned flip_mask, hipStream_t stream);

long long avec_ctc_workspace_floats(int B, int T, int Lmax);
int avec_ctc_loss(const float* logits, const long long* in_lens, const long long* targets, const long long* tgt_lens, float* nll, float* mean_out,
                  float* grad, float* workspace, int B, int T, int V, int Lmax, int blank, int zero_infinity, hipStream_t stream);
int avec_ctc_loss_multi_fits(int T, int V, int Lmax);
int avec_ctc_loss_multi(int n_heads, const float* const* logits, const long long* const* in_lens, const int* T, float* const* nll, float* const* mean_out, float* const* grad,
                        const long long* targets, const long long* tgt_lens, const float* weights, float* total, int B, int V, int Lmax, int blank, int zero_infinity, hipStream_t stream);
int avec_scale_by_scalar(const float* g, const float* scalar_dev, float mul, float* out, long long n, hipStream_t stream);
int avec_scale_by_scalar_multi(int n_tensors, const float* const* g, float* const* out, const long long* numel, const float* mul, const float* scalar_dev, hipStream_t stream);
int avec_softmax_ce(const float* logits, const long long* targets, long long ignore_index, float* loss, float* mean_out, float* grad, long long M, int V, hipStream_t stream);
int avec_len_affine(const long long* in, long long* out, int n, long long sub, long long div, long long add, hipStream_t stream);
int avec_argmax_rows(const float* x, long long* out, long long M, int V, hipStream_t stream);

typedef struct avec_ngram {
  int order;
  int V;
  const float* unigram;
  long long ctx_cap;
  const unsigned long long* ctx_key;
  const float* ctx_bo;
  const int* ctx_off;
  const int* ctx_cnt;
  const int* cont_tok;
  const float* cont_lp;
} avec_ngram_t;
long long avec_ctc_beam_workspace_bytes(int B, int T, int W);
int avec_ctc_beam_search(const float* logits, const long long* lengths, int B, int T, int V, int W, float inv_tmp, const avec_ngram_t* lm, float alpha, float beta,
                         float oov_logprob, void* workspace, long long workspace_bytes, int* tokens, int* out_len, float* score, float* ctc_logp, hipStream_t stream);
long long avec_ctc_beam_state_bytes(int B, int W);
int avec_ctc_beam_stream(const float* logits, const long long* chunk_len, const unsigned char* reset, int B, int Tc, int V, int W, int Tcap, float inv_tmp,
                         const avec_ngram_t* lm, float alpha, float beta, float oov_logprob, void* state, long long state_bytes, void* backptr, long long backptr_bytes,
                         int* tokens, int* out_len, float* score, float* ctc_logp, int* stable_len, int emit, hipStream_t stream);
int avec_ngram_rows(const avec_ngram_t* lm, const int* ctx, const int* ctx_len, int n, int max_len, float oov_logprob, float* rows, hipStream_t stream);
long long avec_ctc_align_workspace_bytes(int B, int T, int Lmax);
int avec_ctc_align_fits_lds(int T, int Lmax);
int avec_ctc_align(const float* logits, const long long* in_lens, const long long* targets, const long long* tgt_lens,
                   int B, int T, int V, int Lmax, int blank, int tier ,
                   void* workspace, long long workspace_bytes,
                   int* path, int* spans, float* score, float* token_logp, hipStream_t stream);
int avec_embed_pos(int dtype, const long long* ids, const float* E, const float* P, void* out, int out_f32, long long N, int L, int V, int D, hipStream_t stream);
int avec_causal_attention_supported(int d);
int avec_causal_attention(int dtype, const void* qkv, long long ld, const long long* lens, void* o, long long ldo, int N, int H, int L, int d, float scale, hipStream_t stream);
long long avec_lm_head_nll_workspace_bytes(long long R, int V, int D);
int avec_lm_head_nll(int dtype, const void* h, long long ldh, const void* W, long long ldw, const float* bias, const long long* tgt, float* nll, long long R, int V, int D,
                     void* workspace, long long workspace_bytes, hipStream_t stream);
int avec_lm_segment_sum(const float* nll, const long long* lens, long long S, int L, float* out, hipStream_t stream);
int avec_lm_rescore_select(const float* neural, const long long* lens, const float* beam_score, float alpha, float beta, int B, int K, float* total, long long* best,
                           hipStream_t stream);
int avec_ctc_tta_pick(const int* tokens, const int* out_len, const float* score, const long long* best_slot, int B, int n, int W, int T, long long* best_aug,
                      long long* best_beam, long long* ids, long long* ids_len, float* best_score, hipStream_t stream);
int avec_adam_step(float* params, float* grads, float* exp_avg, float* exp_avg_sq, const float* state_dev, float beta1, float beta2, float eps,
                   float weight_decay, float grad_scale, int zero_grad, long long n, hipStream_t stream);
int avec_adam_step_guarded(float* params, float* grads, float* exp_avg, float* exp_avg_sq, const float* state_dev, float beta1, float beta2, float eps,
                           float weight_decay, float grad_scale, int zero_grad, long long n, const int* skip_flag, hipStream_t stream);
long long avec_grad_norm_workspace_bytes(long long n);
int avec_grad_norm_blocks(long long n);
int avec_grad_norm(const float* g, long long n, float grad_scale, float max_norm, int skip_nonfinite, const int* skip_in, void* workspace, long long workspace_bytes,
                   float* stats, int* flag, hipStream_t stream);
int avec_adam_step_clipped(float* params, float* grads, float* exp_avg, float* exp_avg_sq, const float* state_dev, float beta1, float beta2, float eps,
                           float weight_decay, float grad_scale, int zero_grad, long long n, const int* skip_flag, const float* clip_dev, hipStream_t stream);
int avec_weight_average(float* avg, const float* p, int mode, float wa, float wp, long long n, hipStream_t stream);
int avec_shadow_refresh(int dtype, const float* master, void* shadow, const long long* table_dev, int n_entries, long long total_blocks, hipStream_t stream);
int avec_shadow_refresh_range(int dtype, const float* master, void* shadow, const long long* table_dev, int n_entries, long long first_block, long long n_blocks, hipStream_t stream);

#ifdef __cplusplus
}
#endif
#endif
```

Before: 1907.

## Fuse relpos attention backward into one per-head MFMA kernel with windowed dE GEMM

Adds a single-block-per-(batch,head) backward kernel for bf16 relative-position attention with T<=128 and d<=64. It computes dQ, dK and dV in one launch by keeping P and dS transposed in LDS, which removes the P/dS scratch round-trip and the separate GEMM launches for dK and dV. The dE gradient comes from a new windowed TN GEMM that reads the skewed dS rows directly and zero-clips entries outside the window. In exchange, only B*H blocks launch, each with a large LDS footprint, which can limit occupancy.

```diff
diff --git a/avec_amd/csrc/attention.h b/avec_amd/csrc/attention.h
--- a/avec_amd/csrc/attention.h
+++ b/avec_amd/csrc/attention.h
@@ -30,3 +30,5 @@
 
 int attn_mfma_fwd(const AttnArgs& a, hipStream_t st);
 int attn_mfma_bwd_rows(const AttnArgs& a, hipStream_t st);
+bool attn_mfma_bwd_fused_ok(const AttnArgs& a);
+int attn_mfma_bwd_fused(const AttnArgs& a, hipStream_t st);
diff --git a/avec_amd/csrc/attention.hip b/avec_amd/csrc/attention.hip
--- a/avec_amd/csrc/attention.hip
+++ b/avec_amd/csrc/attention.hip
@@ -270,6 +270,27 @@
   AttnArgs a; AVEC_CHECK_ARG(p, "attention_bwd: null args"); if (int r = fill_args(a, p)) return r;
   AVEC_CHECK_ARG(a.dout && a.dq && a.pbuf && a.dsbuf && a.ldt >= a.Tk && (a.dsrel ? a.ldr >= a.Tk + a.T - 1 : (a.Tk != a.T || (a.dk && a.dv && a.de))), "attention_bwd: null gradient / scratch pointer");
   int r = (dtype == AVEC_BF16) ? launch_bwd<bf16>(a, st) : launch_bwd<float>(a, st);
+  if (r) return r;
+  AVEC_LAUNCH_CHECK(); return 0;
+}
+
+static int fused_args(AttnArgs& a, int dtype, const avec_attn_t* p) {
+  AVEC_CHECK_ARG(p, "attention_bwd_fused: null args"); if (int r = fill_args(a, p)) return r;
+  AVEC_CHECK_ARG(dtype == AVEC_BF16, "attention_bwd_fused: bf16 only (dtype %d)", dtype);
+  AVEC_CHECK_ARG(!a.mask && a.Tk == a.T && a.T <= 128 && a.d <= 64 && a.d % 2 == 0, "attention_bwd_fused: serves no dense mask, Tk == T <= 128 and an even d <= 64 (T=%d Tk=%d d=%d mask=%d)",
+                 a.T, a.Tk, a.d, a.mask ? 1 : 0);
+  return 0;
+}
+extern "C" int avec_relpos_attention_bwd_fused_ok(int dtype, const avec_attn_t* p) {
+  AttnArgs a; if (!p || dtype != AVEC_BF16 || p->B <= 0 || p->H <= 0 || p->T <= 0 || p->d <= 0) return 0;
+  a.mask = p->mask; a.T = p->T; a.Tk = p->Tk > 0 ? p->Tk : p->T; a.d = p->d; a.ld = p->ld; a.lde = p->lde; a.ldo = p->ldo;
+  return attn_mfma_bwd_fused_ok(a) ? 1 : 0;
+}
+extern "C" int avec_relpos_attention_bwd_fused(int dtype, const avec_attn_t* p, hipStream_t st) {
+  AttnArgs a; if (int r = fused_args(a, dtype, p)) return r;
+  AVEC_CHECK_ARG(a.dout && a.dq && a.dk && a.dv && a.dsrel && a.ldr >= 2 * a.T - 1, "attention_bwd_fused: null gradient / staging pointer (dout, dq, dk, dv, dsrel with ldr >= 2T-1)");
+  const int r = attn_mfma_bwd_fused(a, st);
+  if (r == 1) { avec_set_error("attention_bwd_fused: rows shorter than a head's 16-channel padding (or AVEC_NO_MFMA_ATTN set): not served"); return -1; }
   if (r) return r;
   AVEC_LAUNCH_CHECK(); return 0;
 }
diff --git a/avec_amd/csrc/attention_mfma.hip b/avec_amd/csrc/attention_mfma.hip
--- a/avec_amd/csrc/attention_mfma.hip
+++ b/avec_amd/csrc/attention_mfma.hip
@@ -132,7 +132,7 @@
 
 template <int PITCH, int NTM, int DKS>
 __device__ __forceinline__ float scores(f32x16 (&S)[NTM], const char* Ks, const char* Es, const char* qrow, float* ring, const MfmaGeom& G, float scale,
-                                        int w, int il, int hf, int Tn, int klen, bool row_masked) {
+                                        int ewin, int il, int hf, int Tn, int klen, bool row_masked) {
   const int dks = DKS ? DKS : G.DKS;
   const int swr = aswz<PITCH>(il);
 #pragma unroll
@@ -143,7 +143,7 @@
     f32x16 R;
 #pragma unroll
     for (int r = 0; r < 16; ++r) R[r] = 0.f;
-    const char* erow = Es + (32 * et + 32 * (1 - w) + il) * PITCH;
+    const char* erow = Es + (32 * et + ewin + il) * PITCH;
 #pragma unroll
     for (int kk = 0; kk < dks; ++kk) {
       const chunk16 fa = *(const chunk16*)(erow + (((2 * kk + hf) ^ swr) << 4));
@@ -268,7 +268,7 @@
   const bool row_masked = i >= a.q_full;
 
   f32x16 S[NTM];
-  float mx = scores<PITCH, NTM, DKS>(S, Ks, Es, qrow, ring, G, a.scale, w, il, hf, Tn, klen, row_masked);
+  float mx = scores<PITCH, NTM, DKS>(S, Ks, Es, qrow, ring, G, a.scale, 32 * (1 - w), il, hf, Tn, klen, row_masked);
   mx = fmaxf(mx, __shfl_xor(mx, 32, 64));
   float lsum = 0.f;
 #pragma unroll
@@ -363,7 +363,7 @@
   delta += __shfl_xor(delta, 32, 64);
 
   f32x16 S[NTM];
-  scores<PITCH, NTM, DKS>(S, Ks, Es, qrow, ring, G, a.scale, w, il, hf, Tn, klen, row_masked);
+  scores<PITCH, NTM, DKS>(S, Ks, Es, qrow, ring, G, a.scale, 32 * (1 - w), il, hf, Tn, klen, row_masked);
 #if AVEC_ATTN_ABL == 2
   if (S[0][0] + S[1][3] + delta == 1234.5f) a.lse[0] = 1.f;
   return;
@@ -474,6 +474,204 @@
   }
   bf16* dqp = (bf16*)a.dq + ((long long)b * Tn + i0 + 32 * w) * a.lddq + h * d;
   store_rows_T(DQ, 1.f, ring, G, dqp, a.lddq, min(32, Tn - (i0 + 32 * w)), d, lane);
+}
+
+static constexpr int FNT = 4;
+__device__ __forceinline__ int pt_off(int j, int i) { return j * 256 + ((((i >> 2) ^ j) & 31) << 3) + (i & 3) * 2; }
+
+template <int DKS>
+__global__ __launch_bounds__(256) void attn_mfma_bwd_fused_kernel(AttnArgs a, MfmaGeom G) {
+  constexpr int PITCH = 128, NTM = FNT, NWS = 4;
+  extern __shared__ __attribute__((aligned(16))) char sm[];
+  char* Ks = sm + G.offK; char* Vs = sm + G.offV; char* Es = sm + G.offE; char* Qs = sm + G.offQ; char* Gs = Qs + G.Tp * PITCH;
+  const int tid = threadIdx.x, lane = tid & 63, w = tid >> 6, hf = lane >> 5, il = lane & 31;
+  float* ring = (float*)(sm + G.offS + w * 8192);
+  const int bh = blockIdx.x, b = bh / a.H, h = bh - b * a.H;
+  const int Tn = a.T, d = a.d;
+  const bf16* qp = (const bf16*)a.q + (long long)b * Tn * a.ld + h * d;
+  const bf16* kp = (const bf16*)a.k + (long long)b * Tn * a.ld + h * d;
+  const bf16* vp = (const bf16*)a.v + (long long)b * Tn * a.ld + h * d;
+  const bf16* ep = (const bf16*)a.e + h * d;
+  const bf16* gp = (const bf16*)a.dout + (long long)b * Tn * a.ldo + h * d;
+  {
+    typedef __attribute__((address_space(3))) void* lptr_t;
+    const unsigned lds0 = (unsigned)(uintptr_t)(lptr_t)sm;
+    const int wv = __builtin_amdgcn_readfirstlane(w);
+    const long long lastq = (long long)(a.B - 1 - b) * Tn + Tn - 1;
+    const int rb = (a.H - h) * d * 2;
+    stage_rows_dma<PITCH, NWS>(lds0 + (unsigned)G.offK, Ks, kp, a.ld, 0, G.Tp, Tn, d, G.dpad, lastq, rb, wv, lane);
+    stage_rows_dma<PITCH, NWS>(lds0 + (unsigned)G.offV, Vs, vp, a.ld, 0, G.Tp, Tn, d, G.dpad, lastq, rb, wv, lane);
+    stage_rows_dma<PITCH, NWS>(lds0 + (unsigned)G.offQ, Qs, qp, a.ld, 0, G.Tp, Tn, d, G.dpad, lastq, rb, wv, lane);
+    stage_rows_dma<PITCH, NWS>(lds0 + (unsigned)G.offQ + G.Tp * PITCH, Gs, gp, a.ldo, 0, G.Tp, Tn, d, G.dpad, lastq, rb, wv, lane);
+    stage_rows_dma<PITCH, NWS>(lds0 + (unsigned)G.offE, Es, ep, a.lde, (Tn - 1) - (G.Tp - 1), G.NE, 2 * Tn - 1, d, G.dpad, 2 * Tn - 2, rb, wv, lane);
+    asm volatile("s_waitcnt vmcnt(0)" ::: "memory");
+    zero_pad_channels<PITCH, NWS>(Qs, G.Tp, d, G.dpad, wv, lane);
+    zero_pad_channels<PITCH, NWS>(Gs, G.Tp, d, G.dpad, wv, lane);
+  }
+  __syncthreads();
+
+  const bool act = w < G.NT;
+  const int ewin = 32 * (G.NT - 1 - w);
+  const int i = 32 * w + il;
+  const int swr = aswz<PITCH>(il);
+  int offt[CTMAX][2]; tr_offsets<PITCH>(offt, lane);
+  f32x16 S[NTM]; uint32_t Pk[NTM][8];
+  if (act) {
+    const char* qrow = Qs + (32 * w + il) * PITCH; const char* grow = Gs + (32 * w + il) * PITCH;
+    const int klen = a.lens ? (int)(a.lens[b] / a.len_div) : Tn;
+    const bool row_masked = i >= a.q_full, iv = i < Tn;
+    float delta = 0.f, m_i = 0.f, il_i = 0.f;
+    if (iv) {
+      const bf16* orow = (const bf16*)a.o + ((long long)b * Tn + i) * a.ldo + h * d;
+      const int c0 = hf * ((d + 1) >> 1), c1 = hf ? d : ((d + 1) >> 1);
+      for (int c = c0; c < c1; ++c) {
+        const int ch = c >> 3; const bf16* gq = (const bf16*)(grow + ((ch ^ swr) << 4)) + (c & 7);
+        delta += bf16_to_f32(gq->v) * bf16_to_f32(orow[c].v);
+      }
+      m_i = a.lse[((long long)bh * Tn + i) * 2]; il_i = 1.f / a.lse[((long long)bh * Tn + i) * 2 + 1];
+    }
+    delta += __shfl_xor(delta, 32, 64);
+
+    scores<PITCH, NTM, DKS>(S, Ks, Es, qrow, ring, G, a.scale, ewin, il, hf, Tn, klen, row_masked);
+    bf16* rrow = (bf16*)a.dsrel + ((long long)h * a.B * Tn + (long long)b * Tn + i) * a.ldr + (Tn - 1 - i);
+#pragma unroll
+    for (int jt = 0; jt < NTM; ++jt) {
+      if (jt < G.NT) {
+        f32x16 dP;
+#pragma unroll
+        for (int r = 0; r < 16; ++r) dP[r] = 0.f;
+        const char* vrow = Vs + (32 * jt + il) * PITCH;
+#pragma unroll
+        for (int kk = 0; kk < (DKS ? DKS : G.DKS); ++kk) {
+          const chunk16 fa = *(const chunk16*)(vrow + (((2 * kk + hf) ^ swr) << 4));
+          const chunk16 fb = *(const chunk16*)(grow + (((2 * kk + hf) ^ swr) << 4));
+          dP = mma(fa, fb, dP);
+        }
+#pragma unroll
+        for (int q = 0; q < 4; ++q) {
+          const int j0 = 32 * jt + 8 * q + 4 * hf;
+          float pv[4], dv[4];
+#pragma unroll
+          for (int e = 0; e < 4; ++e) {
+            const int r = 4 * q + e; const bool ok = iv && (j0 + e) < Tn;
+            const float p = ok ? __expf(S[jt][r] - m_i) * il_i : 0.f;
+            pv[e] = p; dv[e] = p * (dP[r] - delta) * a.scale; S[jt][r] = dv[e];
+          }
+          Pk[jt][2 * q] = pack2(pv[0], pv[1]); Pk[jt][2 * q + 1] = pack2(pv[2], pv[3]);
+          if (iv && j0 < Tn) {
+            typedef uint2 __attribute__((aligned(2))) u64_u;
+            if (j0 + 3 < Tn) { uint2 ud; ud.x = pack2(dv[0], dv[1]); ud.y = pack2(dv[2], dv[3]); *(u64_u*)(rrow + j0) = ud; }
+            else {
+#pragma unroll
+              for (int e = 0; e < 4; ++e) if (j0 + e < Tn) rrow[j0 + e].v = f32_to_bf16(dv[e]);
+            }
+          }
+        }
+      }
+    }
+    f32x16 DQ[CTMAX];
+#pragma unroll
+    for (int ct = 0; ct < CTMAX; ++ct)
+#pragma unroll
+      for (int r = 0; r < 16; ++r) DQ[ct][r] = 0.f;
+#pragma unroll
+    for (int jt = 0; jt < NTM; ++jt) {
+      if (jt < G.NT) {
+#pragma unroll
+        for (int s = 0; s < 2; ++s) {
+          chunk16 pb;
+#pragma unroll
+          for (int e = 0; e < 4; ++e) pb.w[e] = pack2(S[jt][8 * s + 2 * e], S[jt][8 * s + 2 * e + 1]);
+          const char* kb = Ks + (32 * jt + 16 * s) * PITCH;
+#pragma unroll
+          for (int ct = 0; ct < CTMAX; ++ct) if (ct < G.CT) DQ[ct] = mma(tr8(kb + offt[ct][0], kb + offt[ct][1]), pb, DQ[ct]);
+        }
+      }
+    }
+    asm volatile("s_waitcnt lgkmcnt(0)" ::: "memory");
+#pragma unroll
+    for (int r = 0; r < 16; ++r) ring[1024 + ((r & 3) + 8 * (r >> 2) + 4 * hf) * 32 + il] = 0.f;
+#pragma unroll
+    for (int et = 0; et <= NTM; ++et) {
+      if (et <= G.NT) {
+        float* slot = ring + (et & 1) * 1024;
+#pragma unroll
+        for (int r = 0; r < 16; ++r) {
+          float v = 0.f;
+          if (et < NTM) v = (et < G.NT) ? S[et < NTM ? et : 0][r] : 0.f;
+          slot[((r & 3) + 8 * (r >> 2) + 4 * hf) * 32 + il] = v;
+        }
+        asm volatile("s_waitcnt lgkmcnt(0)" ::: "memory");
+        float rs[16];
+#pragma unroll
+        for (int r = 0; r < 16; ++r) {
+          const int j = 32 * et + (r & 3) + 8 * (r >> 2) + 4 * hf - 31 + il;
+          rs[r] = ring[(j & 63) * 32 + il];
+        }
+        asm volatile("" ::: "memory");
+#pragma unroll
+        for (int s = 0; s < 2; ++s) {
+          chunk16 pb;
+#pragma unroll
+          for (int e = 0; e < 4; ++e) pb.w[e] = pack2(rs[8 * s + 2 * e], rs[8 * s + 2 * e + 1]);
+          const char* eb = Es + (32 * et + ewin + 16 * s) * PITCH;
+#pragma unroll
+          for (int ct = 0; ct < CTMAX; ++ct) if (ct < G.CT) DQ[ct] = mma(tr8(eb + offt[ct][0], eb + offt[ct][1]), pb, DQ[ct]);
+        }
+      }
+    }
+    bf16* dqp = (bf16*)a.dq + ((long long)b * Tn + 32 * w) * a.lddq + h * d;
+    store_rows_T(DQ, 1.f, ring, G, dqp, a.lddq, min(32, Tn - 32 * w), d, lane);
+  }
+  __syncthreads();
+  char* PT = sm + G.offK; char* ST = sm + G.offE;
+  if (act) {
+#pragma unroll
+    for (int jt = 0; jt < NTM; ++jt) {
+      if (jt < G.NT) {
+#pragma unroll
+        for (int r = 0; r < 16; r += 2) {
+          const uint32_t pp = Pk[jt][r >> 1], ds = pack2(S[jt][r], S[jt][r + 1]);
+          const int j = 32 * jt + (r & 3) + 8 * (r >> 2) + 4 * hf;
+          *(unsigned short*)(PT + pt_off(j, i)) = (unsigned short)(pp & 0xffffu); *(unsigned short*)(PT + pt_off(j + 1, i)) = (unsigned short)(pp >> 16);
+          *(unsigned short*)(ST + pt_off(j, i)) = (unsigned short)(ds & 0xffffu); *(unsigned short*)(ST + pt_off(j + 1, i)) = (unsigned short)(ds >> 16);
+        }
+      }
+    }
+  }
+  __syncthreads();
+  if (!act) return;
+  f32x16 DK[CTMAX], DV[CTMAX];
+#pragma unroll
+  for (int ct = 0; ct < CTMAX; ++ct)
+#pragma unroll
+    for (int r = 0; r < 16; ++r) { DK[ct][r] = 0.f; DV[ct][r] = 0.f; }
+  const char* ptrow = PT + (32 * w + il) * 256; const char* strow = ST + (32 * w + il) * 256;
+#pragma unroll
+  for (int it = 0; it < NTM; ++it) {
+    if (it < G.NT) {
+#pragma unroll
+      for (int s = 0; s < 2; ++s) {
+        const int g0 = 8 * it + 4 * s + hf;
+        const uint2 p0 = *(const uint2*)(ptrow + ((g0 ^ il) << 3)), p1 = *(const uint2*)(ptrow + (((g0 + 2) ^ il) << 3));
+        const uint2 s0 = *(const uint2*)(strow + ((g0 ^ il) << 3)), s1 = *(const uint2*)(strow + (((g0 + 2) ^ il) << 3));
+        chunk16 pb, sb; pb.w[0] = p0.x; pb.w[1] = p0.y; pb.w[2] = p1.x; pb.w[3] = p1.y; sb.w[0] = s0.x; sb.w[1] = s0.y; sb.w[2] = s1.x; sb.w[3] = s1.y;
+        const char* gb = Gs + (32 * it + 16 * s) * PITCH; const char* qb = Qs + (32 * it + 16 * s) * PITCH;
+#pragma unroll
+        for (int ct = 0; ct < CTMAX; ++ct) {
+          if (ct < G.CT) {
+            DV[ct] = mma(tr8(gb + offt[ct][0], gb + offt[ct][1]), pb, DV[ct]);
+            DK[ct] = mma(tr8(qb + offt[ct][0], qb + offt[ct][1]), sb, DK[ct]);
+          }
+        }
+      }
+    }
+  }
+  const int nrow = min(32, Tn - 32 * w);
+  bf16* dkp = (bf16*)a.dk + ((long long)b * Tn + 32 * w) * a.ldd + h * d;
+  bf16* dvp = (bf16*)a.dv + ((long long)b * Tn + 32 * w) * a.ldd + h * d;
+  store_rows_T(DK, 1.f, ring, G, dkp, a.ldd, nrow, d, lane);
+  store_rows_T(DV, 1.f, ring, G, dvp, a.ldd, nrow, d, lane);
 }
 
 static const bool g_mfma_off = getenv("AVEC_NO_MFMA_ATTN") != nullptr;
@@ -511,3 +709,24 @@
 #undef AVEC_LAUNCH_ATTN
   AVEC_LAUNCH_CHECK(); return 0;
 }
+
+static MfmaGeom fused_geom(int T, int d) {
+  MfmaGeom g; g.Tp = (T + 31) / 32 * 32; g.NT = g.Tp / 32; g.NE = 2 * g.Tp; g.dpad = (d + 15) / 16 * 16; g.DKS = g.dpad / 16; g.CT = (d + 31) / 32; g.alias = 0;
+  g.offK = 0; g.offV = (size_t)g.Tp * 128; g.offE = g.offV + (size_t)g.Tp * 128; g.offQ = g.offE + (size_t)g.NE * 128; g.offS = g.offQ + (size_t)2 * g.Tp * 128;
+  g.total = g.offS + (size_t)4 * 8192;
+  return g;
+}
+bool attn_mfma_bwd_fused_ok(const AttnArgs& a) {
+  return !g_mfma_off && !a.mask && a.Tk == a.T && a.T <= 32 * FNT && a.d <= 64 && (a.d & 1) == 0 && !rows_too_short(a.ld, a.d) && !rows_too_short(a.lde, a.d) && !rows_too_short(a.ldo, a.d);
+}
+int attn_mfma_bwd_fused(const AttnArgs& a, hipStream_t st) {
+  if (!attn_mfma_bwd_fused_ok(a)) return 1;
+  const MfmaGeom G = fused_geom(a.T, a.d);
+  if (G.total > 160 * 1024) return 1;
+  const dim3 grid(a.B * a.H);
+#define AVEC_LAUNCH_FUSED(K) do { avec_note_kernel("attn_mfma_bwd_fused<%d>", K); if (int r = avec_lds_optin(attn_mfma_bwd_fused_kernel<K>, G.total)) return r; \
+    hipLaunchKernelGGL((attn_mfma_bwd_fused_kernel<K>), grid, dim3(256), G.total, st, a, G); } while (0)
+  if (G.DKS == 4) AVEC_LAUNCH_FUSED(4); else if (G.DKS == 3) AVEC_LAUNCH_FUSED(3); else AVEC_LAUNCH_FUSED(0);
+#undef AVEC_LAUNCH_FUSED
+  AVEC_LAUNCH_CHECK(); return 0;
+}
diff --git a/avec_amd/csrc/gemm.hip b/avec_amd/csrc/gemm.hip
--- a/avec_amd/csrc/gemm.hip
+++ b/avec_amd/csrc/gemm.hip
@@ -854,8 +854,23 @@
   }
 }
 
-template <typename T, int BI, int BJ, int MODE, bool Q_F32, bool A16>
-__device__ __forceinline__ void gemm_tn_body(TnArgs g, const int bx, const int by, const int bz) {
+template <typename T>
+__device__ __forceinline__ void tn_win_clip(chunk16& c, int i, int col, int winT) {
+  const int lo = winT - 1 - i - col, hi = lo + winT - 1;
+  if (sizeof(T) == 4) {
+#pragma unroll
+    for (int e = 0; e < 4; ++e) c.w[e] = (e >= lo && e <= hi) ? c.w[e] : 0u;
+  } else {
+#pragma unroll
+    for (int e = 0; e < 4; ++e) {
+      const uint32_t w = c.w[e];
+      c.w[e] = ((2 * e >= lo && 2 * e <= hi) ? (w & 0xffffu) : 0u) | ((2 * e + 1 >= lo && 2 * e + 1 <= hi) ? (w & 0xffff0000u) : 0u);
+    }
+  }
+}
+
+template <typename T, int BI, int BJ, int MODE, bool Q_F32, bool A16, bool WIN = false>
+__device__ __forceinline__ void gemm_tn_body(TnArgs g, const int bx, const int by, const int bz, const int winT = 0) {
   constexpr int VEC = Elt<T>::VEC;
   constexpr int RPT = sizeof(T) == 2 ? 2 : 1;
   constexpr int KE = 32 * RPT;
@@ -899,7 +914,9 @@
     }
   }
   Pend pp[NTI][RPT], pq[NTJ][RPT];
+  long long pend_m = 0;
   auto issue = [&](long long mt0) {
+    pend_m = mt0;
 #pragma unroll
     for (int u = 0; u < NTI; ++u) {
       const int col = i0 + task_c(u) * VEC;
@@ -929,7 +946,15 @@
   auto stage = [&](int buf) {
     char* Ps = smem + buf * TILE; char* Qs = Ps + BI * LDS_ROW;
 #pragma unroll
-    for (int u = 0; u < NTI; ++u) store_transposed<T>(Ps, task_c(u) * VEC, task_p(u), finish_load<T, false>(pp[u][0]), finish_load<T, false>(pp[u][RPT - 1]));
+    for (int u = 0; u < NTI; ++u) {
+      chunk16 c0 = finish_load<T, false>(pp[u][0]), c1 = finish_load<T, false>(pp[u][RPT - 1]);
+      if (WIN) {
+        const int col = i0 + task_c(u) * VEC;
+        const int wi = (int)((unsigned)(pend_m + task_p(u) * RPT) % (unsigned)winT), wi1 = RPT == 1 ? wi : (wi + 1 == winT ? 0 : wi + 1);
+        tn_win_clip<T>(c0, wi, col, winT); tn_win_clip<T>(c1, wi1, col, winT);
+      }
+      store_transposed<T>(Ps, task_c(u) * VEC, task_p(u), c0, c1);
+    }
 #pragma unroll
     for (int u = 0; u < NTJ; ++u) store_transposed<T>(Qs, task_c(u) * VEC, task_p(u), finish_load<T, Q_F32 && !Q_CONV>(pq[u][0]), finish_load<T, Q_F32 && !Q_CONV>(pq[u][RPT - 1]));
   };
@@ -963,6 +988,8 @@
 template <typename T, int BI, int BJ, int MODE, bool Q_F32, bool A16>
 __global__ __launch_bounds__(256, 2) void gemm_tn_kernel(TnArgs g) { gemm_tn_body<T, BI, BJ, MODE, Q_F32, A16>(g, blockIdx.x, blockIdx.y, blockIdx.z); }
 
+__global__ __launch_bounds__(256, 2) void gemm_tn_win_kernel(TnArgs g, int winT) { gemm_tn_body<bf16, 64, 64, MODE_PLAIN, false, false, true>(g, blockIdx.x, blockIdx.y, blockIdx.z, winT); }
+
 #define AVEC_TN_MULTI_MAX 3
 struct TnMulti { TnArgs g[AVEC_TN_MULTI_MAX]; int first[AVEC_TN_MULTI_MAX + 1], gx[AVEC_TN_MULTI_MAX], gy[AVEC_TN_MULTI_MAX], n; };
 __global__ __launch_bounds__(256, 2) void gemm_tn_multi_kernel(TnMulti m) {
@@ -971,7 +998,6 @@
   int l = w - m.first[p]; const int bx = l % m.gx[p]; l /= m.gx[p];
   gemm_tn_body<bf16, 64, 64, MODE_PLAIN, false, false>(m.g[p], bx, l % m.gy[p], l / m.gy[p]);
 }
-
 typedef short v4s_t __attribute__((ext_vector_type(4)));
 __device__ __forceinline__ chunk16 tr_read8(const char* p0, const char* p1) {
   typedef __attribute__((address_space(3))) v4s_t* lp_t;
@@ -1408,6 +1434,7 @@
 }
 
 static thread_local TnMulti* tn_collect = nullptr;
+static thread_local int tn_win_T = 0;
 template <typename T, int BI, int BJ, int MODE, bool F32SRC, bool A16>
 static int launch_tn_generic(const TnArgs& g, dim3 grid, hipStream_t st) {
   return avec_launch(gemm_tn_kernel<T, BI, BJ, MODE, F32SRC, A16>, grid, dim3(256), (size_t)2 * (BI + BJ) * LDS_ROW, st, {g},
@@ -1442,6 +1469,11 @@
   const bool f32src = q_f32 && sizeof(T) == 2;
   const bool a16 = nbatch == 1 && avec_aligned16(g.P) && avec_aligned16(g.q.ptr) && g.Iq % VEC == 0 && g.Jq % VEC == 0 && g.ldp % VEC == 0 &&
                    (mode != MODE_PLAIN || (g.q.ld % (f32src ? 4 : VEC) == 0));
+  if (tn_win_T) {
+    if constexpr (sizeof(T) == 2 && BI == 64 && BJ == 64) {
+      return avec_launch(gemm_tn_win_kernel, grid, dim3(256), (size_t)2 * (BI + BJ) * LDS_ROW, st, {g, tn_win_T}, "gemm_tn_win_kernel<%d>", tn_win_T);
+    } else { avec_set_error("gemm_tn_batched_window: bf16 products in 64 x 64 tiles only"); return -1; }
+  }
   if (sizeof(T) == 2 && a16 && !f32src && !g.Oact && (mode == MODE_PLAIN || g.q_mg != 0)) {
     static const int kt_env = getenv("AVEC_TN_KT") ? atoi(getenv("AVEC_TN_KT")) : 32;
     return kt_env == 64 ? launch_tn_tr_mode<BI, BJ, 64>(g, mode, grid, st) : launch_tn_tr_mode<BI, BJ, 32>(g, mode, grid, st);
@@ -1489,9 +1521,9 @@
   g.sOo = strides ? strides[4] : 0; g.sOi = strides ? strides[5] : 0;
   if (dtype == AVEC_BF16 && strides) for (int i = 0; i < 2; ++i) AVEC_CHECK_ARG(strides[i] % 2 == 0, "gemm_tn: bf16 batch strides of P must be even");
   const int nbatch = nb_outer * nb_inner;
-  bool big = (I >= 128 && J >= 128) && ((long long)((I + 127) / 128) * ((J + 127) / 128) * nbatch >= 48 || M >= 32768);
+  bool big = !tn_win_T && (I >= 128 && J >= 128) && ((long long)((I + 127) / 128) * ((J + 127) / 128) * nbatch >= 48 || M >= 32768);
   int r;
-  const bool wide = !big && I <= 64 && J >= 128 && M >= 32768 && dtype == AVEC_BF16 && !q_f32 && nbatch == 1 && avec_aligned16(P) && avec_aligned16(Q) && Iq % 8 == 0 && Jq % 8 == 0 &&
+  const bool wide = !big && !tn_win_T && I <= 64 && J >= 128 && M >= 32768 && dtype == AVEC_BF16 && !q_f32 && nbatch == 1 && avec_aligned16(P) && avec_aligned16(Q) && Iq % 8 == 0 && Jq % 8 == 0 &&
                     ldp % 8 == 0 && (q_mode != MODE_PLAIN || q_rows->ld % 8 == 0);
   if (dtype == AVEC_BF16) r = big ? launch_tn_tile<bf16, 128, 128>(g, q_mode, q_f32, nbatch, stream) : wide ? launch_tn_tile<bf16, 64, 128>(g, q_mode, q_f32, nbatch, stream)
                                                                                                     : launch_tn_tile<bf16, 64, 64>(g, q_mode, q_f32, nbatch, stream);
@@ -1522,6 +1554,18 @@
   avec_rows_t rows = {}; rows.ld = ldq;
   AVEC_CHECK_ARG(strides6 && O_act, "gemm_tn_batched_store: null pointer");
   return gemm_tn_impl(dtype, P, ldp, Q, &rows, MODE_PLAIN, 0, nullptr, O_act, ldo, M, I, J, nb_outer, nb_inner, strides6, nullptr, stream);
+}
+
+extern "C" int avec_gemm_tn_batched_window(int dtype, const void* P, long long ldp, const void* Q, long long ldq, float* O, long long ldo, long long M, int I, int J,
+                                           int nb_outer, int nb_inner, const long long* strides6, int T, hipStream_t stream) {
+  avec_rows_t rows = {}; rows.ld = ldq;
+  AVEC_CHECK_ARG(dtype == AVEC_BF16, "gemm_tn_batched_window: bf16 only (dtype %d)", dtype);
+  AVEC_CHECK_ARG(strides6 && O, "gemm_tn_batched_window: null pointer");
+  AVEC_CHECK_ARG(T > 0 && I == 2 * T - 1 && M > 0 && M % T == 0 && M < (1ll << 31), "gemm_tn_batched_window: P is [n * T][2T - 1] (T=%d I=%d M=%lld)", T, I, M);
+  tn_win_T = T;
+  const int rc = gemm_tn_impl(dtype, P, ldp, Q, &rows, MODE_PLAIN, 0, O, nullptr, ldo, M, I, J, nb_outer, nb_inner, strides6, nullptr, stream);
+  tn_win_T = 0;
+  return rc;
 }
 
 extern "C" int avec_gemm_tn_batched_multi(int dtype, const avec_tn_batched_t* items, int n, hipStream_t stream) {
diff --git a/avec_amd/ops.py b/avec_amd/ops.py
--- a/avec_amd/ops.py
+++ b/avec_amd/ops.py
@@ -129,6 +129,13 @@
 
 TN_MULTI = True
 ATTN_ODD_VALU = False
+ATTN_BWD_FUSED = True
+
+
+def attn_bwd_path(a, adt):
+    if ATTN_BWD_FUSED and adt == torch.bfloat16 and lib.raw("avec_relpos_attention_bwd_fused_ok")(rt.dt(), _byref(a)) == 1:
+        return "fused"
+    return "pair"
 
 
 def _chunk_readable(t, ld, width, rows):
@@ -811,9 +818,18 @@
         a.dk, a.dv, a.ldd = dqkv.data_ptr() + D * esz, dqkv.data_ptr() + 2 * D * esz, 3 * D
         a.de, a.ldde = de.data_ptr(), de.stride(0)
         Tld, Rld = (Tp + 7) // 8 * 8, (2 * Tp - 1 + 7) // 8 * 8
-        scratch = empty((2, B * H, Tp, Tld), adt, dy)
-        a.pbuf, a.dsbuf, a.ldt = scratch.data_ptr(), scratch.data_ptr() + scratch[0].numel() * esz, Tld
-        use_mfma = d % 2 == 0 or not ATTN_ODD_VALU
+        fused = attn_bwd_path(a, adt) == "fused"
+        if fused:
+            dsrel = empty((H, B * Tp, Rld), adt, dy)
+            a.dsrel, a.ldr = dsrel.data_ptr(), Rld
+            lib.relpos_attention_bwd_fused(rt.dt(), _byref(a), rt.stream())
+            L6 = ctypes.c_longlong * 6
+            lib.gemm_tn_batched_window(rt.dt(), dsrel.data_ptr(), Rld, qkv.data_ptr(), 3 * D, de.data_ptr(), de.stride(0), B * Tp, 2 * Tp - 1, d, 1, H,
+                                       L6(0, B * Tp * Rld, 0, d, 0, d), Tp, rt.stream())
+        else:
+            scratch = empty((2, B * H, Tp, Tld), adt, dy)
+            a.pbuf, a.dsbuf, a.ldt = scratch.data_ptr(), scratch.data_ptr() + scratch[0].numel() * esz, Tld
+        use_mfma = (d % 2 == 0 or not ATTN_ODD_VALU) and not fused
         if use_mfma:
             n_rel = H * B * Tp * Rld
             if adt == torch.bfloat16:
@@ -821,7 +837,8 @@
             else:
                 dsrel = rt.zeros_scratch(n_rel, dy.device).view(H, B * Tp, Rld)
             a.dsrel, a.ldr = dsrel.data_ptr(), Rld
-        lib.relpos_attention_bwd(rt.dt(), _byref(a), rt.stream())
+        if not fused:
+            lib.relpos_attention_bwd(rt.dt(), _byref(a), rt.stream())
         if use_mfma:
             L6 = ctypes.c_longlong * 6
             sK, sV, sE = L6(H * Tp * Tld, Tp * Tld, Tp * 3 * D, d, Tp * 3 * D, d), L6(H * Tp * Tld, Tp * Tld, Tp * D, d, Tp * 3 * D, d), L6(0, B * Tp * Rld, 0, d, 0, d)
diff --git a/include/avec_hip.h b/include/avec_hip.h
--- a/include/avec_hip.h
+++ b/include/avec_hip.h
@@ -82,6 +82,8 @@
   const long long* strides6;
 } avec_tn_batched_t;
 int avec_gemm_tn_batched_multi(int dtype, const avec_tn_batched_t* items, int n, hipStream_t stream);
+int avec_gemm_tn_batched_window(int dtype, const void* P, long long ldp, const void* Q, long long ldq, float* O, long long ldo, long long M, int I, int J,
+                                int nb_outer, int nb_inner, const long long* strides6, int T, hipStream_t stream);
 
 #define AVEC_PEER_MAX_WORLD 8
 int avec_peer_exchange_sum(const float* in, float* out, int n, void* const* pages, long long page_stride_granules, int rank, int world,
@@ -180,6 +182,8 @@
 } avec_attn_t;
 int avec_relpos_attention_fwd(int dtype, const avec_attn_t* args, hipStream_t stream);
 int avec_relpos_attention_bwd(int dtype, const avec_attn_t* args, hipStream_t stream);
+int avec_relpos_attention_bwd_fused_ok(int dtype, const avec_attn_t* args);
+int avec_relpos_attention_bwd_fused(int dtype, const avec_attn_t* args, hipStream_t stream);
 
 long long avec_glu_dwconv_stream_state_bytes(int dtype, int B, int C, int K);
 int avec_glu_dwconv_stream(int dtype, const void* u, const float* w, const float* bias, const float* ss, void* out, void* state, long long state_bytes,
```

New measurement: 1915, median of 6. Within noise of the previous version (+0.4%).
